# dnvtmf/SK_GS

Measured on AMD Instinct MI355X. Metric: train iters/sec (deform + rasterize fwd+bwd + L1/SSIM loss + Adam; ms/render fwd+bwd beside it), 100k Gaussians @800x800, higher is better.
Workload: dtype f32

## Files before the change

### include/skgs.h

```cpp
#ifndef SKGS_H_
#define SKGS_H_

#include <stddef.h>
#include <stdint.h>

#ifdef __cplusplus
extern "C" {
#endif

#define SKGS_VERSION 1
#define SKGS_TILE 16
#define SKGS_MAX_RENDER_EXTRA 4
#define SKGS_FUSED_LBS_MAX_BONES 60
#define SKGS_FUSED_LBS_MAX_K 8

typedef void* skgs_stream_t;

typedef struct skgs_knn_deform_job {
  int32_t M, K;
  const float* points;
  const float* joints;
  const float* sp_W;
  const float* bone_T;
  const float* bone_drot;
// ... 90 lines not shown
int skgs_rasterize_forward_stage2(const skgs_raster_inputs* in, const skgs_raster_buffers* buf, float* out_color,
    float* out_opacity, float* out_extra, skgs_stream_t stream);
int skgs_rasterize_forward(const skgs_raster_inputs* in, const skgs_raster_buffers* buf, int32_t* radii,
    float* out_color, float* out_opacity, float* out_extra, int32_t* host_num_rendered, skgs_stream_t stream);
int skgs_read_status(const skgs_raster_buffers* buf, skgs_status* host_status, skgs_stream_t stream);

typedef struct skgs_raster_grads {
  const float* dL_dout_color;
  const float* dL_dout_opacity;
  const float* dL_dout_extra;
  const float* grad_means2D_in;
  const float* grad_conic_in;
  const float* grad_opacity_in;
  float* dL_dmeans2D;
  float* dL_dconic;
  float* dL_dcolors;
  float* dL_dopacity;
  float* dL_dmeans3D;
  float* dL_dcov3D;
  float* dL_dsh;
  float* dL_dscales;
  float* dL_drotations;
  float* dL_dextras;
  float* dL_dsh_rest;
  float* workspace; size_t workspace_bytes;
  int32_t workspace_is_zero;
  float* dL_dsh_factors;
  float* stat_xyz_gradient_accum;
  float* stat_denom;
  float* stat_max_radii2D;
  float stat_grad_multiplier;
  const struct skgs_deform_backward_job* deform_backward_job;
  const struct skgs_sp_skinning_job* sp_skinning_job;
  const skgs_offset_deform_job* offset_job;
} skgs_raster_grads;
size_t skgs_backward_workspace_bytes(int32_t P);

int skgs_rasterize_backward(const skgs_raster_inputs* in, const skgs_raster_buffers* buf, const int32_t* radii,
    const float* out_opacity, const skgs_raster_grads* g, skgs_stream_t stream);

int skgs_rasterize_extra_forward(int32_t W, int32_t H, int32_t P, int32_t E, const float* extra,
    const skgs_raster_buffers* buf, float* pixel_extra, skgs_stream_t stream);
int skgs_rasterize_extra_backward(int32_t W, int32_t H, int32_t P, int32_t E, const float* extra,
    const float* out_opacity, const float* grad_pixel_extra, const skgs_raster_buffers* buf, float* grad_means2D,
    float* grad_conic, float* grad_opacity, float* dL_dextra, skgs_stream_t stream);
int skgs_topk_weights(int32_t topk, int32_t W, int32_t H, int32_t P, const skgs_raster_buffers* buf,
    int32_t* top_indices, float* top_weights, skgs_stream_t stream);
int skgs_render_census(int32_t W, int32_t H, const skgs_raster_buffers* buf, float* out_color, float* out_opacity,
    uint32_t* census, skgs_stream_t stream);
int skgs_mark_visible(int32_t P, const float* means3D, const float* viewmatrix, int32_t colmap, uint8_t* present,
    skgs_stream_t stream);

int skgs_sh_grad_from_factors(int32_t P, int32_t n_views, int32_t sh_degree, int32_t sh_coeffs, const float* factors,
    float* dL_dsh, float* dL_dsh_rest, skgs_stream_t stream);

typedef struct skgs_deform_inputs {
  int32_t P, K, M;
  const float* points;
  const float* weights;
  const int64_t* indices;
  const float* bone_T;
  const float* bone_drot;
  const float* bone_dscale;
  const float* xyz;
  const float* log_scale;
  const float* rot;
  const float* opacity_logit;
  const int32_t* live_count;
  int32_t largest;
} skgs_deform_inputs;
typedef struct skgs_deform_backward_job {
  const skgs_deform_inputs* in;
  float* g_bone_T;
  float* g_bone_drot;
  float* g_bone_dscale;
  float* g_xyz;
  float* g_log_scale;
  float* g_rot;
  float* g_opacity_logit;
  float* g_sp_W;
  float* g_logits;
  void* workspace;
  size_t workspace_bytes;
} skgs_deform_backward_job;
int skgs_lbs_deform_forward(const skgs_deform_inputs* in, float* means, float* scales, float* rotations,
    float* opacity, float* d_xyz, float* d_rot, float* d_scale, skgs_stream_t stream);
size_t skgs_lbs_deform_backward_workspace_bytes(int32_t P, int32_t M);
int skgs_lbs_deform_backward(const skgs_deform_inputs* in, const float* g_means, const float* g_scales,
    const float* g_rotations, const float* g_opacity, float* g_weights, float* g_bone_T, float* g_bone_drot,
    float* g_bone_dscale, float* g_xyz, float* g_log_scale, float* g_rot, float* g_opacity_logit, void* workspace,
    size_t workspace_bytes, skgs_stream_t stream);
int skgs_lbs_deform_backward_logits(const skgs_deform_inputs* in, const float* g_means, const float* g_scales,
    const float* g_rotations, const float* g_opacity, float* g_weights, float* g_bone_T, float* g_bone_drot,
    float* g_bone_dscale, float* g_xyz, float* g_log_scale, float* g_rot, float* g_opacity_logit, float* g_sp_W,
    float* g_logits, void* workspace, size_t workspace_bytes, skgs_stream_t stream);
int skgs_knn_bones(int32_t P, int32_t M, int32_t K, int32_t dim, const float* points, const float* joints,
    float* out_dist, int64_t* out_idx, skgs_stream_t stream);
int skgs_knn_dist_weights_forward(int32_t P, int32_t M, int32_t K, int32_t dim, const float* points, const float* joints,
    const float* kernel_radius, const float* kernel_weight, float temperature, int32_t raw_parameters, int64_t* out_idx,
    float* out_weights, float* out_dist, skgs_stream_t stream);
size_t skgs_knn_dist_weights_workspace_bytes(int32_t P, int32_t M, int32_t dim);
int skgs_knn_dist_weights_backward(int32_t P, int32_t M, int32_t K, int32_t dim, const float* points, const float* joints,
    const float* kernel_radius, const float* kernel_weight, float temperature, int32_t raw_parameters,
    int32_t accumulate_joints, const float* weights, const int64_t* indices, const float* nn_dist, const float* g_weights,
    float* g_points, float* g_joints, float* g_kernel_radius, float* g_kernel_weight, void* workspace, size_t workspace_bytes,
    skgs_stream_t stream);
int skgs_lbs_weights_forward(int32_t P, int32_t M, int32_t K, const float* sp_W, const int64_t* indices, float* weights,
    skgs_stream_t stream);
int skgs_lbs_weights_backward_compact(int32_t P, int32_t K, const float* weights, const float* g_weights, float* g_logits,
    skgs_stream_t stream);
int skgs_lbs_logits_scatter(int32_t P, int32_t M, int32_t K, const int64_t* indices, const float* g_logits, float* g_sp_W,
    skgs_stream_t stream);
int skgs_knn_lbs_weights(int32_t P, int32_t M, int32_t K, const float* points, const float* joints, const float* sp_W,
    int64_t* out_idx, float* out_weights, skgs_stream_t stream);
int skgs_lbs_weights_backward(int32_t P, int32_t M, int32_t K, const float* weights, const int64_t* indices,
    const float* g_weights, float* g_sp_W, skgs_stream_t stream);
int skgs_knn_lbs_deform_forward(int32_t P, int32_t M, int32_t K, const float* points, const float* joints, const float* sp_W,
    const float* bone_T, const float* bone_drot, const float* bone_dscale, const float* xyz, const float* log_scale,
    const float* rot, const float* opacity_logit, int64_t* out_idx, float* out_weights, float* means, float* scales,
    float* rotations, float* opacity, const int32_t* live_count ,
    skgs_stream_t stream);

int skgs_se3_blend_forward(int32_t P, int32_t K, int32_t M, const float* T, const int64_t* indices, const float* points,
    const float* weights, float* out, skgs_stream_t stream);
size_t skgs_se3_blend_backward_workspace_bytes(int32_t P, int32_t M);
int skgs_se3_blend_backward(int32_t P, int32_t K, int32_t M, const float* T, const int64_t* indices, const float* points,
    const float* weights, const float* g_out, float* g_T, float* g_weights, float* g_points, void* workspace,
    size_t workspace_bytes, skgs_stream_t stream);

size_t skgs_index_add_rows_workspace_bytes(int64_t R, int32_t C, int32_t M);
int skgs_index_add_rows(int64_t R, int32_t C, int32_t M, const int64_t* indices, const float* rows, float* out, void* workspace,
    size_t workspace_bytes, skgs_stream_t stream);

int skgs_lie_forward(int32_t group, int32_t op, int64_t B, const float* X, const float* Y, float* out, skgs_stream_t stream);
int skgs_lie_backward(int32_t group, int32_t op, int64_t B, const float* grad, const float* X, const float* Y, float* dX, float* dY,
    skgs_stream_t stream);

int skgs_bone_chain_forward(int32_t M, int32_t root, const int32_t* parents, const int32_t* level_nodes,
    const int32_t* level_start, int32_t num_levels, const float* sk_r_raw, const float* joints, const float* global_T,
    float* bone_T, float* chain_A, const int32_t* frame_index, skgs_stream_t stream);
int skgs_bone_chain_backward(int32_t M, int32_t root, const int32_t* parents, const int32_t* level_nodes,
    const int32_t* level_start, int32_t num_levels, const float* sk_r_raw, const float* joints, const float* global_T,
    const float* chain_A, const float* g_bone_T, float* g_sk_r_raw, float* g_joints, float* g_global_T,
    const int32_t* frame_index, skgs_stream_t stream);

size_t skgs_image_loss_workspace_bytes(int32_t C, int32_t H, int32_t W);
int skgs_image_loss_forward(int32_t C, int32_t H, int32_t W, const float* pred, const float* gt, const int32_t* gt_index,
    float lambda_l1, float lambda_ssim, float* loss3 , void* workspace,
    size_t workspace_bytes, skgs_stream_t stream);
int skgs_image_loss_backward(int32_t C, int32_t H, int32_t W, const float* pred, const float* gt, const int32_t* gt_index,
    float lambda_l1, float lambda_ssim, const float* grad_loss, const void* workspace, size_t workspace_bytes,
    float* dL_dpred, float* loss3, skgs_stream_t stream);
int skgs_image_loss_backward_terms(int32_t C, int32_t H, int32_t W, const float* pred, const float* gt,
    const int32_t* gt_index, const float* grad_l1, const float* grad_ssim, const void* workspace, size_t workspace_bytes,
    float* dL_dpred, skgs_stream_t stream);

int32_t skgs_weight_reg_partials(void);
int skgs_weight_sparsity(int64_t n, const float* weights, float eps, float* grad, float* partials, skgs_stream_t stream);
int skgs_weight_smooth(int32_t P, int32_t K, int32_t G, const float* weights, const int64_t* neighbours, const int32_t* inverse_offsets,
    const int32_t* inverse_sources, float* grad, float* partials, skgs_stream_t stream);

int32_t skgs_joint_loss_partials(int32_t M);
int skgs_joint_loss_forward(int32_t M, int32_t inverse_branch, const float* spT, const float* joint_pos, const float* cost_in, float momentum,
    float one_minus_momentum, float* cost_out, float* jd, float* partials, skgs_stream_t stream);
int skgs_joint_loss_reduce(int32_t M, int32_t edges, const int32_t* parent, const float* jd, const float* partials, float* out,
    skgs_stream_t stream);
size_t skgs_joint_loss_backward_workspace_bytes(int32_t M);
// ... 17 lines not shown
size_t skgs_adam_state_bytes(void);
int64_t skgs_adam_chunk_elems(void);
int skgs_adam_step(int32_t n_tensors, const void* tensors, int64_t total_chunks, double beta1, double beta2, double eps,
    float* step_state, float* zero_after ,
    int64_t zero_n, skgs_stream_t stream);
int skgs_adam_step_range(int32_t n_tensors, const void* tensors, int64_t chunk_begin, int64_t chunk_end, double beta1,
    double beta2, double eps, float* step_state, int32_t advance, float* zero_after, int64_t zero_n, skgs_stream_t stream);
int skgs_adam_logit_rows(int32_t P, int32_t M, int32_t K, const float* weights, const int64_t* indices, const float* g_weights,
    const void* tensor, uint32_t* tile_mask, double beta1, double beta2, double eps, const float* step_state, int32_t after_advance,
    skgs_stream_t stream);
int skgs_adam_masked_rows(int32_t P, int32_t M, int32_t K, const int64_t* indices, int32_t scan_gradient, const void* tensor,
    uint32_t* tile_mask, double beta1, double beta2, double eps, const float* step_state, int32_t after_advance, skgs_stream_t stream);
int skgs_adam_logit_mask_rebuild(int32_t P, int32_t M, const float* exp_avg, const float* exp_avg_sq, uint32_t* tile_mask,
    skgs_stream_t stream);
typedef struct skgs_view_advance {
  const void* table;
  const int32_t* order;
  int32_t* cursor;
  void* slot;
  int32_t n_order, words;
} skgs_view_advance;
int skgs_adam_step_tail(int32_t n_tensors, const void* tensors, int64_t chunk_begin, int64_t chunk_end, double beta1,
    double beta2, double eps, float* step_state, float* zero_after, int64_t zero_n, int64_t freq_chunk, int32_t freq_B,
    int32_t freq_D, int32_t freq_degree, const float* freq_grad_out, const float* freq_out, int32_t freq_ld_out,
    float* freq_grad_x, int32_t freq_accumulate, const skgs_view_advance* next_view, skgs_stream_t stream);

int skgs_freq_encode_forward(int32_t B, int32_t D, int32_t degree, const float* x, int32_t ld_x , float* out, int32_t ld_out, skgs_stream_t stream);
int skgs_freq_encode_backward(int32_t B, int32_t D, int32_t degree, const float* grad_out, const float* out, int32_t ld_out,
    float* grad_x, int32_t accumulate , skgs_stream_t stream);
int skgs_linear_forward(int32_t B, int32_t in1, int32_t in2, int32_t out, const float* X1, int32_t ldx1, const float* X2,
    int32_t ldx2, const float* W, const float* bias, float* Y, int32_t ldy, int32_t relu, skgs_stream_t stream);
int skgs_linear_backward(int32_t B, int32_t in1, int32_t in2, int32_t out, const float* X1, int32_t ldx1, const float* X2,
    int32_t ldx2, const float* W, const float* Y, const float* gY, int32_t ldy, int32_t relu, float* gW, float* gb,
    float* gX1, int32_t ldg1, float* gX2, int32_t ldg2, int32_t accumulate_gx, skgs_stream_t stream);

#define SKGS_MLP_MAX_LAYERS 12
typedef struct skgs_mlp_layer {
  const float* W;
  const float* bias;
  float* gW;
  float* gb;
  int32_t in_hidden, in_x0, out, relu;
} skgs_mlp_layer;
typedef struct skgs_mlp_desc {
  int32_t B;
  int32_t p_dim, p_degree, t_dim, t_degree;
  int32_t hidden, n_layers;
  skgs_mlp_layer layer[SKGS_MLP_MAX_LAYERS];
  int32_t n_heads, head_dim[4];
  float* head_out[4];
  const float* head_gout[4];
} skgs_mlp_desc;
size_t skgs_deform_mlp_workspace_bytes(const skgs_mlp_desc* d);
int skgs_deform_mlp_workspace_init(void* workspace, size_t workspace_bytes, skgs_stream_t stream);
int32_t skgs_deform_mlp_xcd_mode(int32_t mode);
int skgs_deform_mlp_forward(const skgs_mlp_desc* d, const float* points, const float* t, float* x0, float* acts, float* out,
    void* workspace, size_t workspace_bytes, skgs_stream_t stream);
int skgs_deform_mlp_backward(const skgs_mlp_desc* d, const float* points, const float* t, const float* x0, const float* acts,
    const float* g_out, float* g_x0, void* workspace, size_t workspace_bytes, skgs_stream_t stream);
typedef struct skgs_adam_range {
  int32_t n_tensors;
  const void* tensors;
  int64_t chunk_begin, chunk_end;
  double beta1, beta2, eps;
  const float* step_count;
  int32_t after_advance;
} skgs_adam_range;
int skgs_deform_mlp_backward_adam(const skgs_mlp_desc* d, const float* points, const float* t, const float* x0,
    const float* acts, const float* g_out, float* g_x0, void* workspace, size_t workspace_bytes, const skgs_adam_range* side,
    skgs_stream_t stream);
typedef struct skgs_bone_chain_desc {
  int32_t M, root, num_levels;
  const int32_t *parents, *level_nodes, *level_start;
  const float* joints;
  const float* global_T;
  const int32_t* frame_index;
  float* bone_T;
  float* chain_A;
  const float* sk_r_raw;
  const float* g_bone_T;
  float* g_joints;
  float* g_global_T;
  float* sk_cache;
} skgs_bone_chain_desc;
int skgs_skeleton_forward(const skgs_mlp_desc* d, const skgs_bone_chain_desc* bones, const float* points, const float* t,
    float* x0, float* acts, void* workspace, size_t workspace_bytes, const skgs_adam_range* side ,
    skgs_stream_t stream);
int skgs_skeleton_backward(const skgs_mlp_desc* d, const skgs_bone_chain_desc* bones, const float* points, const float* t,
    const float* x0, const float* acts, float* g_x0, void* workspace, size_t workspace_bytes, const skgs_adam_range* side,
    skgs_stream_t stream);
int skgs_deform_mlp_status(const void* workspace, uint32_t* host_words4, skgs_stream_t stream);

int skgs_sp_lbs_weights_forward(int32_t P, int32_t M, int32_t K, int32_t F, const float* points, const float* feature,
    const float* sp_points, const float* sp_feature, const float* sp_radius_raw, const float* sp_weight_raw, float temperature,
    const float* sp_W, const int32_t* sp_order , const int32_t* sp_rank , int64_t* out_idx,
    float* out_weights, float* out_dist, void* pairs , size_t pairs_bytes, int32_t params_activated,
    int32_t pairs_prepared ,
    skgs_stream_t stream);
size_t skgs_sp_lbs_weights_workspace_bytes(int32_t P, int32_t M, int32_t F);
int skgs_sp_lbs_weights_backward(int32_t P, int32_t M, int32_t K, int32_t F, const float* feature, const float* sp_feature,
    const float* sp_radius_raw, const float* sp_weight_raw, float temperature, const float* weights, const int64_t* indices,
    const float* nn_dist, const float* g_weights, float* g_feature, float* g_sp_feature, float* g_sp_radius, float* g_sp_weight,
    void* workspace, size_t workspace_bytes, int32_t params_activated, skgs_stream_t stream);

size_t skgs_sp_pairs_bytes(int32_t P, int32_t M, int32_t K);
size_t skgs_sp_skinning_backward_workspace_bytes(int32_t P, int32_t M, int32_t K);
typedef struct skgs_sp_skinning_job {
  const skgs_deform_inputs* in;
  int32_t F;
  const float *feature, *sp_feature, *sp_radius_raw, *sp_weight_raw;
  float temperature;
  int32_t logit_weighting;
  const float* nn_dist;
  float *g_weights, *g_xyz, *g_log_scale, *g_rot, *g_opacity_logit, *g_feature, *g_bone_T, *g_bone_drot, *g_bone_dscale, *g_sp_feature,
      *g_sp_radius, *g_sp_weight;
  void* pairs;
  size_t pairs_bytes;
  void* workspace;
  size_t workspace_bytes;
  const float* g_weights_extra;
  int32_t image_to_deform_off;
} skgs_sp_skinning_job;
int skgs_sp_skinning_backward(const skgs_deform_inputs* in, int32_t F, const float* feature, const float* sp_feature,
    const float* sp_radius_raw, const float* sp_weight_raw, float temperature, int32_t logit_weighting, const float* nn_dist,
    const float* g_means, const float* g_scales, const float* g_rotations, const float* g_opacity, float* g_weights, float* g_xyz,
    float* g_log_scale, float* g_rot, float* g_opacity_logit, float* g_feature, float* g_bone_T, float* g_bone_drot,
    float* g_bone_dscale, float* g_sp_feature, float* g_sp_radius, float* g_sp_weight, void* pairs, size_t pairs_bytes,
    void* workspace, size_t workspace_bytes, skgs_stream_t stream);
int skgs_sp_skinning_backward_job(const skgs_sp_skinning_job* job, const float* g_means, const float* g_scales, const float* g_rotations,
    const float* g_opacity, skgs_stream_t stream);

#define SKGS_SP_NET_LBS_C 1
#define SKGS_SP_NET_RAW_TIME_FLAG 2
#define SKGS_SP_NET_RAW_TIME SKGS_SP_NET_RAW_TIME_FLAG
#define SKGS_SP_NET_RAW_TIME_DEGREE(degree) (SKGS_SP_NET_RAW_TIME_FLAG | ((degree) << 8))
typedef struct skgs_sp_net {
  int32_t M, flags;
  const float* points;
  const float* time;
  const float *time_w1, *time_b1, *time_w2, *time_b2;
  const float* W[8];
  const float* b[8];
  const float *warp_w, *warp_b, *scaling_w, *scaling_b, *rotation_w, *rotation_b;
  const float *local_w, *local_b;
} skgs_sp_net;
size_t skgs_sp_net_saved_bytes(int32_t M);
size_t skgs_sp_net_workspace_bytes(int32_t M);
typedef struct skgs_sp_prepare {
  int32_t P, M, K, F;
  const float* sp_points;
  const float* sp_feature;
  const int32_t* sp_order;
  void* pairs;
  size_t pairs_bytes;
} skgs_sp_prepare;
int skgs_sp_net_forward(const skgs_sp_net* net, float* raw , float* bone_T, float* d_rot, float* d_scale,
    void* saved, size_t saved_bytes, const skgs_sp_prepare* prepare, skgs_stream_t stream);
int skgs_sp_net_backward(const skgs_sp_net* net, const skgs_sp_net* grads, const float* g_bone_T, const float* g_d_rot,
    const float* g_d_scale, const float* g_raw, const void* saved, size_t saved_bytes, void* workspace, size_t workspace_bytes,
    const skgs_adam_range* side, skgs_stream_t stream);

size_t skgs_sp_net_rows_saved_bytes(int32_t P);
size_t skgs_sp_net_rows_workspace_bytes(int32_t P);
int skgs_sp_net_rows_forward(const skgs_sp_net* net, float* raw, void* saved , size_t saved_bytes, skgs_stream_t stream);
int skgs_sp_net_rows_backward(const skgs_sp_net* net, const skgs_sp_net* grads, const float* g_raw, const void* saved,
    size_t saved_bytes, void* workspace, size_t workspace_bytes, skgs_stream_t stream);
// ... 42 lines not shown
```

### sk_gs_amd/_C.py

```python
from __future__ import annotations

import contextlib
import ctypes as C
import os
import threading
from typing import Optional, Tuple

import torch
from torch import Tensor

_HERE = os.path.dirname(os.path.abspath(__file__))
_LIB_PATH = os.environ.get('SKGS_HIP_LIB') or os.path.join(_HERE, 'libskgs_hip.so')
_lib = None
_lock = threading.Lock()


class SkgsError(RuntimeError):
    pass


class _KnnDeformJob(C.Structure):
    _fields_ = [('M', C.c_int32), ('K', C.c_int32)] + [(n, C.c_void_p) for n in (
        'points', 'joints', 'sp_W', 'bone_T', 'bone_drot', 'bone_dscale', 'xyz', 'log_scale', 'rot', 'opacity_logit', 'out_idx',
        'out_weights', 'means', 'scales', 'rotations', 'opacity')] + [('largest', C.c_int32)]


class _OffsetDeformJob(C.Structure):
    _fields_ = [('scale_mode', C.c_int32), ('d_xyz_stride', C.c_int32)] + [(n, C.c_void_p) for n in (
        'xyz', 'd_xyz', 'log_scale', 'rot', 'opacity_logit', 'scale_mean', 'means', 'scales', 'rotations', 'opacity', 'g_xyz', 'g_d_xyz',
        'g_log_scale', 'g_rot', 'g_opacity_logit', 'workspace')] + [('workspace_bytes', C.c_size_t)]


class _RasterInputs(C.Structure):
    _fields_ = [
        ('P', C.c_int32), ('sh_degree', C.c_int32), ('sh_coeffs', C.c_int32), ('E', C.c_int32),
        ('image_height', C.c_int32), ('image_width', C.c_int32),
        ('tanfovx', C.c_float), ('tanfovy', C.c_float), ('scale_modifier', C.c_float),
        ('prefiltered', C.c_int32), ('debug', C.c_int32), ('colmap', C.c_int32),
        ('viewmatrix', C.c_void_p), ('projmatrix', C.c_void_p), ('campos', C.c_void_p),
        ('means3D', C.c_void_p), ('opacity', C.c_void_p), ('sh', C.c_void_p), ('scales', C.c_void_p),
        ('rotations', C.c_void_p), ('extras', C.c_void_p), ('colors_precomp', C.c_void_p),
        ('cov3D_precomp', C.c_void_p), ('sh_rest', C.c_void_p), ('background', C.c_void_p),
        ('tile_bucket_capacity', C.c_int32), ('tanfov_device', C.c_void_p),
        ('host_status_words', C.c_int32), ('longest_list_hint', C.c_int32), ('live_count', C.c_void_p),
        ('deform_job', C.POINTER(_KnnDeformJob)), ('tiles_per_gaussian_hint', C.c_int32), ('offset_job', C.c_void_p),
    ]


class _RasterBuffers(C.Structure):
    _fields_ = [('geom', C.c_void_p), ('geom_bytes', C.c_size_t), ('binning', C.c_void_p),
                ('binning_bytes', C.c_size_t), ('img', C.c_void_p), ('img_bytes', C.c_size_t)]


class _Status(C.Structure):
    _fields_ = [('num_rendered', C.c_int32), ('overflow', C.c_int32), ('max_tile_count', C.c_int32),
                ('overflow_events', C.c_int32)]


class _RasterGrads(C.Structure):
    _fields_ = [
        ('dL_dout_color', C.c_void_p), ('dL_dout_opacity', C.c_void_p), ('dL_dout_extra', C.c_void_p),
        ('grad_means2D_in', C.c_void_p), ('grad_conic_in', C.c_void_p), ('grad_opacity_in', C.c_void_p),
        ('dL_dmeans2D', C.c_void_p), ('dL_dconic', C.c_void_p), ('dL_dcolors', C.c_void_p),
        ('dL_dopacity', C.c_void_p), ('dL_dmeans3D', C.c_void_p), ('dL_dcov3D', C.c_void_p), ('dL_dsh', C.c_void_p),
        ('dL_dscales', C.c_void_p), ('dL_drotations', C.c_void_p), ('dL_dextras', C.c_void_p),
        ('dL_dsh_rest', C.c_void_p), ('workspace', C.c_void_p), ('workspace_bytes', C.c_size_t),
        ('workspace_is_zero', C.c_int32), ('dL_dsh_factors', C.c_void_p),
        ('stat_xyz_gradient_accum', C.c_void_p), ('stat_denom', C.c_void_p), ('stat_max_radii2D', C.c_void_p),
        ('stat_grad_multiplier', C.c_float), ('deform_backward_job', C.c_void_p), ('sp_skinning_job', C.c_void_p),
        ('offset_job', C.c_void_p),
    ]


class _DeformInputs(C.Structure):
    _fields_ = [
        ('P', C.c_int32), ('K', C.c_int32), ('M', C.c_int32),
        ('points', C.c_void_p), ('weights', C.c_void_p), ('indices', C.c_void_p), ('bone_T', C.c_void_p),
        ('bone_drot', C.c_void_p), ('bone_dscale', C.c_void_p), ('xyz', C.c_void_p), ('log_scale', C.c_void_p),
        ('rot', C.c_void_p), ('opacity_logit', C.c_void_p), ('live_count', C.c_void_p), ('largest', C.c_int32),
    ]


class _DeformBackwardJob(C.Structure):
    _fields_ = [('in_', C.POINTER(_DeformInputs))] + [(n, C.c_void_p) for n in (
        'g_bone_T', 'g_bone_drot', 'g_bone_dscale', 'g_xyz', 'g_log_scale', 'g_rot', 'g_opacity_logit', 'g_sp_W', 'g_logits',
        'workspace')] + [('workspace_bytes', C.c_size_t)]


class _SpSkinningJob(C.Structure):
    _fields_ = ([('in_', C.POINTER(_DeformInputs)), ('F', C.c_int32)] +
                [(n, C.c_void_p) for n in ('feature', 'sp_feature', 'sp_radius_raw', 'sp_weight_raw')] +
                [('temperature', C.c_float), ('logit_weighting', C.c_int32), ('nn_dist', C.c_void_p)] +
                [(n, C.c_void_p) for n in ('g_weights', 'g_xyz', 'g_log_scale', 'g_rot', 'g_opacity_logit', 'g_feature', 'g_bone_T',
                                           'g_bone_drot', 'g_bone_dscale', 'g_sp_feature', 'g_sp_radius', 'g_sp_weight', 'pairs')] +
                [('pairs_bytes', C.c_size_t), ('workspace', C.c_void_p), ('workspace_bytes', C.c_size_t), ('g_weights_extra', C.c_void_p),
                 ('image_to_deform_off', C.c_int32)])


EXPORTED_SYMBOLS = [
    'skgs_geom_buffer_bytes', 'skgs_img_buffer_bytes', 'skgs_binning_buffer_bytes', 'skgs_binning_capacity',
    'skgs_rasterize_forward_stage1', 'skgs_rasterize_forward_stage2', 'skgs_rasterize_forward', 'skgs_read_status',
    'skgs_backward_workspace_bytes', 'skgs_rasterize_backward', 'skgs_rasterize_extra_forward',
    'skgs_rasterize_extra_backward', 'skgs_topk_weights', 'skgs_render_census', 'skgs_set_tile_order', 'skgs_knn_dist_weights_forward', 'skgs_knn_dist_weights_backward',
    'skgs_knn_dist_weights_workspace_bytes', 'skgs_mark_visible', 'skgs_lbs_deform_forward',
    'skgs_lbs_deform_backward', 'skgs_lbs_deform_backward_workspace_bytes', 'skgs_knn_bones',
    'skgs_lbs_weights_forward', 'skgs_lbs_weights_backward', 'skgs_last_error', 'skgs_version',
    'skgs_joint_loss_partials', 'skgs_joint_loss_forward', 'skgs_joint_loss_reduce', 'skgs_joint_loss_backward_workspace_bytes',
    'skgs_joint_loss_backward', 'skgs_point_knn_workspace_bytes', 'skgs_point_knn',
]


def lib_path() -> str:
    return _LIB_PATH


def load_library():
    global _lib
    if _lib is not None:
        return _lib
    with _lock:
        if _lib is not None:
            return _lib
        if not os.path.exists(_LIB_PATH):
            raise SkgsError(
                f'{_LIB_PATH} not found: the HIP extension is not built. Run `python -c "import __graft_entry__ as g; '
                f'g.build()"` or `make -C sk_gs_amd/csrc`. There is no CPU / PyTorch fallback for this path.')
        lib = C.CDLL(_LIB_PATH)
        for name in ('skgs_geom_buffer_bytes', 'skgs_img_buffer_bytes', 'skgs_binning_buffer_bytes',
                     'skgs_backward_workspace_bytes', 'skgs_lbs_deform_backward_workspace_bytes',
                     'skgs_image_loss_workspace_bytes', 'skgs_offset_deform_workspace_bytes'):
            getattr(lib, name).restype = C.c_size_t
        lib.skgs_binning_capacity.restype = C.c_int64
        lib.skgs_binning_capacity.argtypes = [C.c_size_t]
        lib.skgs_binning_buffer_bytes.argtypes = [C.c_int64]
        lib.skgs_last_error.restype = C.c_char_p
        if os.environ.get('SKGS_TILE_ORDER') is not None:
            lib.skgs_set_tile_order(C.c_int(int(os.environ['SKGS_TILE_ORDER'])))
        _lib = lib
    return _lib


_ops = None


def _torch_ops():
    global _ops
    if _ops is None:
        _ops = False
        if os.environ.get('SKGS_TORCH_OPS', '1') != '0' and not os.environ.get('SKGS_HIP_LIB'):
            load_library()
            try:
                from sk_gs_amd import _skgs_torch
                _ops = _skgs_torch
            except ImportError:
                pass
    return _ops or None


def _check(rc: int):
    if rc != 0:
        raise SkgsError(load_library().skgs_last_error().decode())


def _ptr(t: Optional[Tensor]):
    if t is None or t.numel() == 0:
        return None
    return t.data_ptr()


# ... 773 lines not shown
```

### sk_gs_amd/csrc/api.hip

```cpp
#include <stdarg.h>
#include <stdio.h>

#include <algorithm>

#include "skgs_common.h"

namespace skgs {
static thread_local char g_err[512] = "";
int set_error(const char* fmt, ...) {
  va_list ap;
  va_start(ap, fmt);
  vsnprintf(g_err, sizeof(g_err), fmt, ap);
  va_end(ap);
  return 1;
}

__global__ void fill_u32_kernel(uint32_t* __restrict__ p, uint32_t v, size_t n) {
  const size_t stride = (size_t) gridDim.x * blockDim.x;
  for (size_t i = (size_t) blockIdx.x * blockDim.x + threadIdx.x; i < n; i += stride) p[i] = v;
}
int fill_u32(void* p, uint32_t v, size_t n_words, hipStream_t s) {
  if (n_words == 0) return 0;
  const int blocks = (int) std::min<size_t>((n_words + 255) / 256, 2048);
  hipLaunchKernelGGL(fill_u32_kernel, dim3(blocks), dim3(256), 0, s, reinterpret_cast<uint32_t*>(p), v, n_words);
// ... 186 lines not shown
    if (launch_preprocess_forward(*in, g, im, radii, s)) return 1;
    if (launch_scatter_sort(*in, g, im, b, s)) return 1;
    return launch_render_forward(*in, g, im, b, out_color, out_opacity, out_extra, s);
  }
  if (skgs_rasterize_forward_stage1(in, buf, radii, host_num_rendered, stream)) return 1;
  return skgs_rasterize_forward_stage2(in, buf, out_color, out_opacity, out_extra, stream);
}

int skgs_read_status(const skgs_raster_buffers* buf, skgs_status* host_status, skgs_stream_t stream) {
  SKGS_REQUIRE(buf && buf->geom && host_status, "read_status: NULL argument");
  SKGS_CHECK_HIP(hipMemcpyAsync(host_status, buf->geom, sizeof(skgs_status), hipMemcpyDeviceToHost, (hipStream_t) stream));
  return 0;
}

static int check_deform(const skgs_deform_inputs* in);

int skgs_rasterize_backward(const skgs_raster_inputs* in, const skgs_raster_buffers* buf, const int32_t* radii,
    const float* out_opacity, const skgs_raster_grads* gr, skgs_stream_t stream) {
  if (check_inputs(in) || check_buffers(in, buf, true)) return 1;
  SKGS_REQUIRE(gr != nullptr, "grads struct is NULL");
  const skgs_offset_deform_job* oj = gr->offset_job;
  if (oj) {
    SKGS_REQUIRE(!gr->deform_backward_job && !gr->sp_skinning_job, "offset_job: not together with deform_backward_job / sp_skinning_job");
    if (offset_job_check(*in, *oj, true)) return 1;
  }
  if (in->P == 0) {
    if (const skgs_deform_backward_job* dj0 = gr->deform_backward_job) {
      SKGS_REQUIRE(dj0->in && dj0->g_bone_T && dj0->g_bone_drot && dj0->g_bone_dscale, "deform_backward_job: NULL argument");
      hipStream_t s0 = (hipStream_t) stream;
      if (fill_u32(dj0->g_bone_T, 0u, (size_t) dj0->in->M * 7, s0) || fill_u32(dj0->g_bone_drot, 0u, (size_t) dj0->in->M * 4, s0) ||
          fill_u32(dj0->g_bone_dscale, 0u, (size_t) dj0->in->M * 3, s0))
        return 1;
    }
    if (const skgs_sp_skinning_job* sj0 = gr->sp_skinning_job)
      return sp_skinning_check(*sj0) || (!sp_fix_job(*sj0) && launch_sp_skinning_rest(*sj0, (hipStream_t) stream));
    return 0;
  }
  SKGS_REQUIRE(radii && out_opacity, "radii / out_opacity are required");
  SKGS_REQUIRE(gr->dL_dout_color, "dL_dout_color is required");
  SKGS_REQUIRE(gr->dL_dmeans2D && ((gr->deform_backward_job || gr->sp_skinning_job || oj) ||
                                      (gr->dL_dcolors && gr->dL_dopacity && gr->dL_dmeans3D && gr->dL_dcov3D && gr->dL_dscales &&
                                          gr->dL_drotations)),
      "gradient outputs are required");
  SKGS_REQUIRE(!(in->sh && in->sh_coeffs > 0) || gr->dL_dsh || gr->dL_dsh_factors,
      "dL_dsh (or dL_dsh_factors) is required when sh is given");
  SKGS_REQUIRE(gr->dL_dsh_factors || (in->sh_rest != nullptr) == (gr->dL_dsh_rest != nullptr),
      "dL_dsh_rest goes with sh_rest (split SH storage)");
  SKGS_REQUIRE(!gr->dL_dsh_factors || (!gr->dL_dsh && !gr->dL_dsh_rest), "dL_dsh_factors replaces dL_dsh / dL_dsh_rest");
  SKGS_REQUIRE(gr->workspace && gr->workspace_bytes >= skgs_backward_workspace_bytes(in->P), "workspace too small");
  hipStream_t s = (hipStream_t) stream;
  GeomView g    = geom_view(buf->geom);
  ImgView im    = img_view(buf->img, in->image_width, in->image_height);
  BinView b     = bin_view(buf->binning, buf->binning_bytes);
  const skgs_deform_backward_job* dj = gr->deform_backward_job;
  if (dj) {
    SKGS_REQUIRE(dj->in != nullptr, "deform_backward_job: in is NULL");
    if (check_deform(dj->in)) return 1;
    SKGS_REQUIRE(dj->in->P == in->P && dj->in->live_count == in->live_count, "deform_backward_job: P / live_count differ from the rasterizer's");
    SKGS_REQUIRE(!dj->in->largest, "deform_backward_job: warp_method `largest` is served by the sp_skinning_job only");
    SKGS_REQUIRE(dj->in->M <= deform_backward_job_max_bones() && dj->in->K <= deform_backward_job_max_k(),
        "deform_backward_job: needs M <= %d, K <= %d (got %d, %d)", deform_backward_job_max_bones(), deform_backward_job_max_k(),
        dj->in->M, dj->in->K);
    SKGS_REQUIRE(dj->g_bone_T && dj->g_bone_drot && dj->g_bone_dscale, "deform_backward_job: bone gradient outputs are required");
    SKGS_REQUIRE(dj->g_xyz && dj->g_log_scale && dj->g_rot && dj->g_opacity_logit, "deform_backward_job: gradient outputs are required");
    SKGS_REQUIRE(dj->g_sp_W || dj->g_logits, "deform_backward_job: one of g_sp_W / g_logits is required");
    SKGS_REQUIRE(dj->workspace && dj->workspace_bytes >= deform_backward_workspace_bytes(in->P, dj->in->M),
        "deform_backward_job: workspace too small (skgs_lbs_deform_backward_workspace_bytes)");
    SKGS_REQUIRE(in->scales && in->rotations, "deform_backward_job: not with cov3D_precomp");
  }
  const skgs_sp_skinning_job* sj = gr->sp_skinning_job;
  if (sj) {
    SKGS_REQUIRE(!dj, "sp_skinning_job: not together with deform_backward_job");
    if (sp_skinning_check(*sj)) return 1;
    SKGS_REQUIRE(sj->in->P == in->P && in->live_count == nullptr, "sp_skinning_job: P differs from the rasterizer's / no row capacity");
    SKGS_REQUIRE(in->scales && in->rotations, "sp_skinning_job: not with cov3D_precomp");
  }
  if (!gr->workspace_is_zero && fill_u32(gr->workspace, 0u, (size_t) in->P * GRAD_ROW, s)) return 1;
  if (launch_render_backward(*in, g, im, b, out_opacity, gr->dL_dout_color, gr->dL_dout_opacity, gr->dL_dout_extra,
          gr->workspace, s))
    return 1;
  if (launch_preprocess_backward(*in, g, radii, *gr, s)) return 1;
  if (sj) return sp_fix_job(*sj) ? 0 : launch_sp_skinning_rest(*sj, s);
  if (oj) return launch_offset_scale_grad_finalize(in->P, *oj, s);
  return dj ? launch_deform_backward_finalize(*dj->in, dj->workspace, dj->g_bone_T, dj->g_bone_drot, dj->g_bone_dscale, s) : 0;
}

int skgs_rasterize_extra_forward(int32_t W, int32_t H, int32_t P, int32_t E, const float* extra,
    const skgs_raster_buffers* buf, float* pixel_extra, skgs_stream_t stream) {
  SKGS_REQUIRE(buf && buf->geom && buf->img, "buffers are required");
  SKGS_REQUIRE(E > 0 && extra && pixel_extra, "Error shape for extras");
  if (P == 0) return 0;
  GeomView g = geom_view(buf->geom);
  ImgView im = img_view(buf->img, W, H);
  BinView b  = bin_view(buf->binning, buf->binning_bytes);
  return launch_extra_forward(W, H, P, E, extra, g, im, b, pixel_extra, (hipStream_t) stream);
}

int skgs_rasterize_extra_backward(int32_t W, int32_t H, int32_t P, int32_t E, const float* extra, const float* out_opacity,
    const float* grad_pixel_extra, const skgs_raster_buffers* buf, float* grad_means2D, float* grad_conic,
    float* grad_opacity, float* dL_dextra, skgs_stream_t stream) {
  SKGS_REQUIRE(buf && buf->geom && buf->img, "buffers are required");
  SKGS_REQUIRE(E > 0 && extra && grad_pixel_extra && out_opacity, "Error shape for extras");
  SKGS_REQUIRE(grad_means2D && grad_conic && grad_opacity && dL_dextra, "gradient outputs are required");
  if (P == 0) return 0;
  hipStream_t s = (hipStream_t) stream;
  GeomView g = geom_view(buf->geom);
  ImgView im = img_view(buf->img, W, H);
  BinView b  = bin_view(buf->binning, buf->binning_bytes);
  if (fill_u32(dL_dextra, 0u, (size_t) P * E, s)) return 1;
  return launch_extra_backward(W, H, P, E, extra, out_opacity, grad_pixel_extra, g, im, b, grad_means2D, grad_conic,
      grad_opacity, dL_dextra, s);
}

int skgs_topk_weights(int32_t topk, int32_t W, int32_t H, int32_t P, const skgs_raster_buffers* buf, int32_t* top_indices,
    float* top_weights, skgs_stream_t stream) {
  SKGS_REQUIRE(buf && buf->geom && buf->img, "buffers are required");
  SKGS_REQUIRE(topk > 0 && top_indices && top_weights, "topk outputs are required");
  hipStream_t s = (hipStream_t) stream;
  if (P == 0) {
    if (fill_u32(top_indices, 0xffffffffu, (size_t) W * H * topk, s)) return 1;
    if (fill_u32(top_weights, 0u, (size_t) W * H * topk, s)) return 1;
    return 0;
  }
  GeomView g = geom_view(buf->geom);
  ImgView im = img_view(buf->img, W, H);
  BinView b  = bin_view(buf->binning, buf->binning_bytes);
  return launch_topk(topk, W, H, g, im, b, top_indices, top_weights, s);
}

int skgs_render_census(int32_t W, int32_t H, const skgs_raster_buffers* buf, float* out_color, float* out_opacity,
    uint32_t* census, skgs_stream_t stream) {
  SKGS_REQUIRE(buf && buf->geom && buf->img && buf->binning, "buffers of a finished forward are required");
  SKGS_REQUIRE(out_color && out_opacity && census, "census outputs are required");
  GeomView g = geom_view(buf->geom);
  ImgView im = img_view(buf->img, W, H);
  BinView b  = bin_view(buf->binning, buf->binning_bytes);
  return launch_render_census(W, H, g, im, b, out_color, out_opacity, census, (hipStream_t) stream);
}

int skgs_mark_visible(int32_t P, const float* means3D, const float* viewmatrix, int32_t colmap, uint8_t* present,
    skgs_stream_t stream) {
  SKGS_REQUIRE(P == 0 || (means3D && viewmatrix && present), "mark_visible: NULL argument");
  return launch_mark_visible(P, means3D, viewmatrix, colmap, present, (hipStream_t) stream);
}

static int check_deform(const skgs_deform_inputs* in) {
  SKGS_REQUIRE(in != nullptr, "deform inputs struct is NULL");
  SKGS_REQUIRE(in->P >= 0 && in->K >= 1 && in->M >= 1, "deform: need P >= 0, K >= 1, M >= 1");
  if (in->P == 0) return 0;
  SKGS_REQUIRE(in->points && in->weights && in->indices && in->bone_T && in->bone_drot && in->bone_dscale,
      "deform: points / weights / indices / bone tensors are required");
  SKGS_REQUIRE(in->log_scale && in->rot && in->opacity_logit, "deform: Gaussian parameter tensors are required");
  return 0;
}

int skgs_lbs_deform_forward(const skgs_deform_inputs* in, float* means, float* scales, float* rotations, float* opacity,
    float* d_xyz, float* d_rot, float* d_scale, skgs_stream_t stream) {
  if (check_deform(in)) return 1;
  SKGS_REQUIRE(in->P == 0 || (in->xyz && means && scales && rotations && opacity), "deform: outputs are required");
  return launch_deform_forward(*in, means, scales, rotations, opacity, d_xyz, d_rot, d_scale, (hipStream_t) stream);
}

size_t skgs_lbs_deform_backward_workspace_bytes(int32_t P, int32_t M) {
  return deform_backward_workspace_bytes(P < 0 ? 0 : P, M < 0 ? 0 : M);
}

int skgs_lbs_deform_backward(const skgs_deform_inputs* in, const float* g_means, const float* g_scales,
// ... 120 lines not shown
```

### sk_gs_amd/csrc/deform.hip

```cpp
#include <algorithm>

#include "skgs_common.h"
#include "deform_lane.h"

#pragma clang fp contract(off)

namespace skgs {
namespace {

constexpr int DEFORM_THREADS = 256;
constexpr int MAX_LDS_BONES  = 1024;

template <bool LDS_BONES>
__global__ void __launch_bounds__(DEFORM_THREADS) deform_forward_kernel(int P, int K, int M, const float* __restrict__ points,
    const float* __restrict__ weights, const int64_t* __restrict__ indices, const float* __restrict__ bone_T,
    const float* __restrict__ bone_drot, const float* __restrict__ bone_dscale, const float* __restrict__ xyz,
    const float* __restrict__ log_scale, const float* __restrict__ rot, const float* __restrict__ opacity_logit,
    float* __restrict__ means, float* __restrict__ scales, float* __restrict__ rotations, float* __restrict__ opacity,
    float* __restrict__ d_xyz, float* __restrict__ d_rot, float* __restrict__ d_scale, int largest) {
  extern __shared__ float s_bones[];
  if (LDS_BONES) {
    for (int j = threadIdx.x; j < M; j += DEFORM_THREADS) load_bone(bone_T, bone_drot, bone_dscale, j, s_bones + j * BONE_F);
    __syncthreads();
  }
  const int n = blockIdx.x * DEFORM_THREADS + threadIdx.x;
  if (n >= P) return;
  const float p[3] = {points[3 * n], points[3 * n + 1], points[3 * n + 2]};
  float sx[3] = {0, 0, 0}, sr[4] = {0, 0, 0, 0}, ss[3] = {0, 0, 0};
  const int kmax = largest ? argmax_slot(weights + (size_t) n * K, K) : -1;
  for (int k = 0; k < K; ++k) {
    const int j   = (int) indices[(size_t) n * K + k];
    const float w = weights[(size_t) n * K + k];
    float bl[BONE_F];
    const float* b;
    if (LDS_BONES) {
      b = s_bones + j * BONE_F;
    } else {
      load_bone(bone_T, bone_drot, bone_dscale, j, bl);
      b = bl;
    }
    float y[3];
    se3_act(b, p, y);
    const float wx = kmax < 0 ? w : (k == kmax ? 1.f : 0.f);
    sx[0] += y[0] * wx, sx[1] += y[1] * wx, sx[2] += y[2] * wx;
    sr[0] += b[7] * w, sr[1] += b[8] * w, sr[2] += b[9] * w, sr[3] += b[10] * w;
    ss[0] += b[11] * w, ss[1] += b[12] * w, ss[2] += b[13] * w;
  }
  float v[4];
#pragma unroll
  for (int c = 0; c < 3; ++c) {
    const float dx = sx[c] - p[c];
    if (d_xyz) d_xyz[3 * n + c] = dx;
    means[3 * n + c]  = xyz[3 * n + c] + dx;
    scales[3 * n + c] = expf(log_scale[3 * n + c]) + ss[c];
    if (d_scale) d_scale[3 * n + c] = ss[c];
  }
  const float4 r4 = reinterpret_cast<const float4*>(rot)[n];
  v[0] = r4.x + sr[0], v[1] = r4.y + sr[1], v[2] = r4.z + sr[2], v[3] = r4.w + sr[3];
  if (d_rot) reinterpret_cast<float4*>(d_rot)[n] = make_float4(sr[0], sr[1], sr[2], sr[3]);
  float nv = sqrtf(v[0] * v[0] + v[1] * v[1] + v[2] * v[2] + v[3] * v[3]);
  nv       = fmaxf(nv, 1e-12f);
  reinterpret_cast<float4*>(rotations)[n] = make_float4(v[0] / nv, v[1] / nv, v[2] / nv, v[3] / nv);
  opacity[n] = 1.0f / (1.0f + expf(-opacity_logit[n]));
}

template <bool LDS_BONES>
__global__ void __launch_bounds__(DEFORM_THREADS) deform_backward_kernel(int P, int K, int M, const float* __restrict__ points,
    const float* __restrict__ weights, const int64_t* __restrict__ indices, const float* __restrict__ bone_T,
    const float* __restrict__ bone_drot, const float* __restrict__ bone_dscale, const float* __restrict__ log_scale,
    const float* __restrict__ rot, const float* __restrict__ opacity_logit, const float* __restrict__ g_means,
    const float* __restrict__ g_scales, const float* __restrict__ g_rotations, const float* __restrict__ g_opacity,
    float* __restrict__ g_weights, float* __restrict__ g_bone_T, float* __restrict__ g_bone_drot,
    float* __restrict__ g_bone_dscale, float* __restrict__ g_xyz, float* __restrict__ g_log_scale,
    float* __restrict__ g_rot, float* __restrict__ g_opacity_logit, int ncopy, float* __restrict__ partials) {
  extern __shared__ float s_mem[];
  float* s_bones = s_mem;
  float* s_grad  = s_mem + (LDS_BONES ? M * BONE_F : 0);
  float* s_my = s_grad + (size_t) (threadIdx.x & (ncopy - 1)) * M * BONE_F;
  if (LDS_BONES) {
    for (int j = threadIdx.x; j < M; j += DEFORM_THREADS) load_bone(bone_T, bone_drot, bone_dscale, j, s_bones + j * BONE_F);
    for (int i = threadIdx.x; i < ncopy * M * BONE_F; i += DEFORM_THREADS) s_grad[i] = 0.f;
    __syncthreads();
  }
  for (int base = blockIdx.x * DEFORM_THREADS; base < P; base += gridDim.x * DEFORM_THREADS) {
    const bool live = base + (int) threadIdx.x < P;
    const int n     = live ? base + (int) threadIdx.x : P - 1;
// ... 93 lines not shown
          for (int c = 0; c < BONE_F; ++c) atomicAdd(&s_my[j * BONE_F + c], out[c]);
        }
      } else if (live) {
#pragma unroll
        for (int c = 0; c < 7; ++c) atomicAdd(&g_bone_T[7 * j + c], out[c]);
#pragma unroll
        for (int c = 0; c < 4; ++c) atomicAdd(&g_bone_drot[4 * j + c], out[7 + c]);
#pragma unroll
        for (int c = 0; c < 3; ++c) atomicAdd(&g_bone_dscale[3 * j + c], out[11 + c]);
      }
    };
#pragma unroll
    for (int k = 0; k < PREF_K; ++k)
      if (k < K) bone_body(k, jj[k], ww[k]);
    for (int k = PREF_K; k < K; ++k) bone_body(k, (int) indices[(size_t) n * K + k], weights[(size_t) n * K + k]);
  }
  if (LDS_BONES) {
    __syncthreads();
    for (int i = threadIdx.x; i < M * BONE_F; i += DEFORM_THREADS) {
      float val = 0.f;
      for (int cpy = 0; cpy < ncopy; ++cpy) val += s_grad[(size_t) cpy * M * BONE_F + i];
      if (partials) {
        partials[(size_t) blockIdx.x * M * BONE_F + i] = val;
      } else if (val != 0.f) {
        const int j = i / BONE_F, c = i % BONE_F;
        if (c < 7)
          atomicAdd(&g_bone_T[7 * j + c], val);
        else if (c < 11)
          atomicAdd(&g_bone_drot[4 * j + c - 7], val);
        else
          atomicAdd(&g_bone_dscale[3 * j + c - 11], val);
      }
    }
  }
}

__global__ void __launch_bounds__(256) deform_backward_wide_finalize_kernel(int M, int nblk, const float* __restrict__ partials,
    float* __restrict__ g_bone_T, float* __restrict__ g_bone_drot, float* __restrict__ g_bone_dscale) {
  const int i = blockIdx.x * 256 + threadIdx.x;
  if (i >= M * BONE_F) return;
  float sum = 0.f;
  for (int b0 = 0; b0 < nblk; b0 += 16) {
    float v[16];
#pragma unroll
    for (int u = 0; u < 16; ++u) v[u] = partials[(size_t) min(b0 + u, nblk - 1) * M * BONE_F + i];
#pragma unroll
    for (int u = 0; u < 16; ++u)
      if (b0 + u < nblk) sum += v[u];
  }
  const int j = i / BONE_F, c = i % BONE_F;
  if (c < 7)
    g_bone_T[7 * j + c] = sum;
  else if (c < 11)
    g_bone_drot[4 * j + c - 7] = sum;
  else
    g_bone_dscale[3 * j + c - 11] = sum;
}

__global__ void __launch_bounds__(DEFORM_BWD_THREADS) deform_backward_moments_kernel(int P, DeformBwdArgs a,
    const float* __restrict__ g_means, const float* __restrict__ g_scales, const float* __restrict__ g_rotations,
    const float* __restrict__ g_opacity, const int32_t* __restrict__ live_count ) {
  if (live_count) P = min(P, live_count[0]);
  if ((int) (blockIdx.x * DEFORM_BWD_THREADS) >= P) {
    deform_bwd_zero_partials(a);
    return;
  }
  extern __shared__ float s_mem[];
  const int n = blockIdx.x * DEFORM_BWD_THREADS + threadIdx.x;
  DeformBwdLane L;
  deform_bwd_prefetch(a, n, n < P, L);
  float g_dx[3] = {0, 0, 0}, g_ds[3] = {0, 0, 0}, go = 0.f;
  float4 gr4 = make_float4(0.f, 0.f, 0.f, 0.f);
  if (n < P) {
#pragma unroll
    for (int c = 0; c < 3; ++c) g_dx[c] = g_means[3 * n + c], g_ds[c] = g_scales[3 * n + c];
    gr4 = reinterpret_cast<const float4*>(g_rotations)[n], go = g_opacity[n];
  }
  deform_bwd_moments(a, P, s_mem, L, g_dx, g_ds, gr4, go);
}

__global__ void __launch_bounds__(256) deform_backward_finalize_kernel(int M, int nblk, const float* __restrict__ partials,
    const float* __restrict__ bone_T, float* __restrict__ g_bone_T, float* __restrict__ g_bone_drot,
    float* __restrict__ g_bone_dscale) {
  __shared__ float s_red[256][MOM_F + 1];
  const int b = blockIdx.x, t = threadIdx.x;
  float acc[MOM_F];
#pragma unroll
  for (int c = 0; c < MOM_F; ++c) acc[c] = 0.f;
  for (int w = t; w < nblk; w += 256) {
    const float* row = partials + ((size_t) w * M + b) * MOM_F;
#pragma unroll
    for (int c = 0; c < MOM_F; ++c) acc[c] += row[c];
  }
#pragma unroll
  for (int c = 0; c < MOM_F; ++c) s_red[t][c] = acc[c];
  __syncthreads();
  for (int d = 128; d > 0; d >>= 1) {
    if (t < d) {
#pragma unroll
      for (int c = 0; c < MOM_F; ++c) s_red[t][c] += s_red[t + d][c];
    }
    __syncthreads();
  }
  if (t != 0) return;
  float m[MOM_F];
  for (int i = 0; i < MOM_F; ++i) m[i] = s_red[0][i];
  const float q0 = bone_T[7 * b + 3], q1 = bone_T[7 * b + 4], q2 = bone_T[7 * b + 5], q3 = bone_T[7 * b + 6];
  const float qn = sqrtf(q0 * q0 + q1 * q1 + q2 * q2 + q3 * q3);
  const float vq[4] = {q0 / qn, q1 / qn, q2 / qn, q3 / qn};
  const float* S = m + 3;
#define SM(a, c) S[3 * (a) + (c)]
  const float pxg[3] = {SM(2, 1) - SM(1, 2), SM(0, 2) - SM(2, 0), SM(1, 0) - SM(0, 1)};
  const float tr     = SM(0, 0) + SM(1, 1) + SM(2, 2);
  float gqh[4];
  for (int i = 0; i < 3; ++i) {
    const float vdp_g = vq[0] * SM(i, 0) + vq[1] * SM(i, 1) + vq[2] * SM(i, 2);
    const float gdv_p = vq[0] * SM(0, i) + vq[1] * SM(1, i) + vq[2] * SM(2, i);
    gqh[i] = 2.0f * vq[3] * pxg[i] + 2.0f * (vdp_g + gdv_p - 2.0f * tr * vq[i]);
  }
  gqh[3] = 2.0f * ((vq[1] * SM(0, 2) - vq[2] * SM(0, 1)) + (vq[2] * SM(1, 0) - vq[0] * SM(1, 2)) +
                   (vq[0] * SM(2, 1) - vq[1] * SM(2, 0)));
#undef SM
  const float dotq = vq[0] * gqh[0] + vq[1] * gqh[1] + vq[2] * gqh[2] + vq[3] * gqh[3];
  g_bone_T[7 * b] = m[0], g_bone_T[7 * b + 1] = m[1], g_bone_T[7 * b + 2] = m[2];
  for (int i = 0; i < 4; ++i) g_bone_T[7 * b + 3 + i] = (gqh[i] - vq[i] * dotq) / qn;
  for (int i = 0; i < 4; ++i) g_bone_drot[4 * b + i] = m[12 + i];
  for (int i = 0; i < 3; ++i) g_bone_dscale[3 * b + i] = m[16 + i];
}

constexpr int KNN_MAXK = 16;
template <int KCAP>
__global__ void __launch_bounds__(256) knn_bones_kernel(int P, int M, int K, int dim, const float* __restrict__ points,
    const float* __restrict__ joints, float* __restrict__ out_dist, int64_t* __restrict__ out_idx, int lds_joints) {
  extern __shared__ float s_j[];
  if (lds_joints) {
    for (int i = threadIdx.x; i < M * dim; i += blockDim.x) s_j[i] = joints[i];
    __syncthreads();
  }
  const float* jt = lds_joints ? s_j : joints;
  const int n = blockIdx.x * blockDim.x + threadIdx.x;
  if (n >= P) return;
  float bd[KCAP];
  int bi[KCAP];
#pragma unroll
  for (int k = 0; k < KCAP; ++k) bd[k] = __builtin_inff(), bi[k] = -1;
  const float* pn = points + (size_t) n * dim;
  const float p0 = pn[0], p1 = dim > 1 ? pn[1] : 0.f, p2 = dim > 2 ? pn[2] : 0.f;
  for (int j = 0; j < M; ++j) {
    float d = 0.f;
    if (dim == 3) {
      const float d0 = p0 - jt[3 * j], d1 = p1 - jt[3 * j + 1], d2 = p2 - jt[3 * j + 2];
      d += d0 * d0;
      d += d1 * d1;
      d += d2 * d2;
    } else {
      for (int c = 0; c < dim; ++c) {
        const float df = pn[c] - jt[(size_t) j * dim + c];
        d += df * df;
      }
    }
    float cd = d;
    int ci   = j;
    topk_insert<KCAP>(bd, bi, cd, ci);
  }
#pragma unroll
  for (int k = 0; k < KCAP; ++k)
    if (k < K) {
      out_dist[(size_t) n * K + k] = bi[k] >= 0 ? bd[k] : 0.f;
      out_idx[(size_t) n * K + k]  = bi[k];
    }
}

__global__ void __launch_bounds__(256) lbs_weights_forward_kernel(int P, int M, int K, const float* __restrict__ sp_W,
    const int64_t* __restrict__ indices, float* __restrict__ weights) {
  const int p = blockIdx.x * 256 + threadIdx.x;
  if (p >= P) return;
  float l[KNN_MAXK];
  float mx = -INFINITY;
  for (int k = 0; k < K; ++k) {
    l[k] = sp_W[(size_t) p * M + (int) indices[(size_t) p * K + k]];
    mx   = fmaxf(mx, l[k]);
  }
  float sum = 0.f;
  for (int k = 0; k < K; ++k) {
    l[k] = expf(l[k] - mx);
    sum += l[k];
  }
  for (int k = 0; k < K; ++k) weights[(size_t) p * K + k] = l[k] / sum;
}

__global__ void __launch_bounds__(256) lbs_weights_backward_kernel(int P, int M, int K, const float* __restrict__ weights,
    const int64_t* __restrict__ indices, const float* __restrict__ g_weights, float* __restrict__ g_sp_W) {
  extern __shared__ float s_rows[];
  const int p0 = blockIdx.x * 256, p = p0 + threadIdx.x;
  float* row = s_rows + (size_t) threadIdx.x * M;
  for (int m = 0; m < M; ++m) row[m] = 0.f;
  if (p < P) {
    float dot = 0.f;
    for (int k = 0; k < K; ++k) dot += weights[(size_t) p * K + k] * g_weights[(size_t) p * K + k];
    for (int k = 0; k < K; ++k) {
      const float w = weights[(size_t) p * K + k];
      row[(int) indices[(size_t) p * K + k]] += w * (g_weights[(size_t) p * K + k] - dot);
    }
  }
  __syncthreads();
  const size_t n = (size_t) min(256, P - p0) * M;
  float* dst     = g_sp_W + (size_t) p0 * M;
  for (size_t i = threadIdx.x; i < n; i += 256) dst[i] = s_rows[i];
}

// ... 315 lines not shown
  if (in.M <= MAX_LDS_BONES)
    hipLaunchKernelGGL(deform_forward_kernel<true>, grid, block, (size_t) in.M * BONE_F * 4, s, in.P, in.K, in.M, in.points,
        in.weights, in.indices, in.bone_T, in.bone_drot, in.bone_dscale, in.xyz, in.log_scale, in.rot, in.opacity_logit,
        means, scales, rotations, opacity, d_xyz, d_rot, d_scale, in.largest ? 1 : 0);
  else
    hipLaunchKernelGGL(deform_forward_kernel<false>, grid, block, 0, s, in.P, in.K, in.M, in.points, in.weights,
        in.indices, in.bone_T, in.bone_drot, in.bone_dscale, in.xyz, in.log_scale, in.rot, in.opacity_logit, means, scales,
        rotations, opacity, d_xyz, d_rot, d_scale, in.largest ? 1 : 0);
  SKGS_CHECK_HIP(hipGetLastError());
  return 0;
}

constexpr int WIDE_MAX_BLOCKS = 512;
static int wide_blocks(int P) { return std::max(1, std::min((P + DEFORM_THREADS - 1) / DEFORM_THREADS, WIDE_MAX_BLOCKS)); }
size_t deform_backward_workspace_bytes(int P, int M) {
  if (M > MOM_MAX_BONES) return M <= MAX_LDS_BONES / 2 ? align256((size_t) wide_blocks(P) * M * BONE_F * 4) + 256 : 256;
  const size_t nblk = (size_t) (P + DEFORM_THREADS - 1) / DEFORM_THREADS;
  return align256(nblk * (size_t) M * MOM_F * 4) + 256;
}

int launch_deform_backward(const skgs_deform_inputs& in, const float* g_means, const float* g_scales,
    const float* g_rotations, const float* g_opacity, float* g_weights, float* g_bone_T, float* g_bone_drot,
    float* g_bone_dscale, float* g_xyz, float* g_log_scale, float* g_rot, float* g_opacity_logit, void* workspace,
    hipStream_t s, float* g_sp_W, float* g_logits) {
  if ((g_sp_W || g_logits) && (in.M > MOM_MAX_BONES || in.K > PREF_K))
    return set_error("deform backward with the logit gradient folded in needs M <= %d and K <= %d (got %d, %d)",
        MOM_MAX_BONES, PREF_K, in.M, in.K);
  if (in.P == 0) {
    if (fill_u32(g_bone_T, 0u, (size_t) in.M * 7, s) || fill_u32(g_bone_drot, 0u, (size_t) in.M * 4, s) ||
        fill_u32(g_bone_dscale, 0u, (size_t) in.M * 3, s))
      return 1;
    return 0;
  }
  dim3 grid((in.P + DEFORM_THREADS - 1) / DEFORM_THREADS), block(DEFORM_THREADS);
  if (in.M <= MOM_MAX_BONES) {
    const size_t lds = deform_bwd_lds_bytes(in.M);
    float* partials  = reinterpret_cast<float*>(workspace);
    DeformBwdArgs a{in.K, in.M, in.points, in.weights, in.indices, in.bone_T, in.bone_drot, in.bone_dscale, in.log_scale, in.rot,
        in.opacity_logit, g_weights, g_xyz, g_log_scale, g_rot, g_opacity_logit, partials, g_sp_W, g_logits};
    {
      ProfScope prof(K_DEFORM_BWD, s);
      hipLaunchKernelGGL(deform_backward_moments_kernel, grid, block, lds, s, in.P, a, g_means, g_scales, g_rotations, g_opacity,
          in.live_count);
    }
    SKGS_CHECK_HIP(hipGetLastError());
    hipLaunchKernelGGL(deform_backward_finalize_kernel, dim3(in.M), dim3(256), 0, s, in.M, (int) grid.x, partials, in.bone_T,
        g_bone_T, g_bone_drot, g_bone_dscale);
    SKGS_CHECK_HIP(hipGetLastError());
    return 0;
  }
  if (in.M <= MAX_LDS_BONES / 2) {
    const size_t table = (size_t) in.M * BONE_F * 4;
    int ncopy = 1;
    while (ncopy < 16 && table * (1 + 2 * ncopy) <= 56 * 1024) ncopy *= 2;
    const int nblk  = wide_blocks(in.P);
    float* partials = reinterpret_cast<float*>(workspace);
    {
      ProfScope prof(K_DEFORM_BWD, s);
      hipLaunchKernelGGL(deform_backward_kernel<true>, dim3(nblk), block, table * (1 + ncopy), s, in.P, in.K, in.M, in.points,
          in.weights, in.indices, in.bone_T, in.bone_drot, in.bone_dscale, in.log_scale, in.rot, in.opacity_logit, g_means,
          g_scales, g_rotations, g_opacity, g_weights, g_bone_T, g_bone_drot, g_bone_dscale, g_xyz, g_log_scale, g_rot,
          g_opacity_logit, ncopy, partials);
    }
    SKGS_CHECK_HIP(hipGetLastError());
    hipLaunchKernelGGL(deform_backward_wide_finalize_kernel, dim3((in.M * BONE_F + 255) / 256), dim3(256), 0, s, in.M, nblk,
        partials, g_bone_T, g_bone_drot, g_bone_dscale);
    SKGS_CHECK_HIP(hipGetLastError());
    return 0;
  }
  if (fill_u32(g_bone_T, 0u, (size_t) in.M * 7, s) || fill_u32(g_bone_drot, 0u, (size_t) in.M * 4, s) ||
      fill_u32(g_bone_dscale, 0u, (size_t) in.M * 3, s))
    return 1;
  ProfScope prof(K_DEFORM_BWD, s);
  hipLaunchKernelGGL(deform_backward_kernel<false>, grid, block, 0, s, in.P, in.K, in.M, in.points, in.weights,
      in.indices, in.bone_T, in.bone_drot, in.bone_dscale, in.log_scale, in.rot, in.opacity_logit, g_means, g_scales,
      g_rotations, g_opacity, g_weights, g_bone_T, g_bone_drot, g_bone_dscale, g_xyz, g_log_scale, g_rot,
      g_opacity_logit, 1, (float*) nullptr);
  SKGS_CHECK_HIP(hipGetLastError());
  return 0;
}

int launch_deform_backward_finalize(const skgs_deform_inputs& in, void* workspace, float* g_bone_T, float* g_bone_drot,
    float* g_bone_dscale, hipStream_t s) {
  const int nblk = (in.P + DEFORM_BWD_THREADS - 1) / DEFORM_BWD_THREADS;
  hipLaunchKernelGGL(deform_backward_finalize_kernel, dim3(in.M), dim3(256), 0, s, in.M, nblk, reinterpret_cast<float*>(workspace),
      in.bone_T, g_bone_T, g_bone_drot, g_bone_dscale);
  SKGS_CHECK_HIP(hipGetLastError());
  return 0;
}
int deform_backward_job_max_bones() { return MOM_MAX_BONES; }
int deform_backward_job_max_k() { return PREF_K; }

int launch_knn_bones(int P, int M, int K, int dim, const float* points, const float* joints, float* out_dist,
    int64_t* out_idx, hipStream_t s) {
  if (P == 0) return 0;
  if (K > KNN_MAXK || K < 1) return set_error("knn_bones: K must be in [1,%d] (got %d)", KNN_MAXK, K);
  const size_t lds = (size_t) M * dim * 4;
  const int use_lds = lds <= 48 * 1024;
  ProfScope prof(K_KNN, s);
#define SKGS_KNN(KCAP_)                                                                                                  \
  hipLaunchKernelGGL(knn_bones_kernel<KCAP_>, dim3((P + 255) / 256), dim3(256), use_lds ? lds : 0, s, P, M, K, dim, points, \
      joints, out_dist, out_idx, use_lds)
  if (K <= 4)
    SKGS_KNN(4);
  else if (K <= 8)
    SKGS_KNN(8);
  else
    SKGS_KNN(KNN_MAXK);
#undef SKGS_KNN
  SKGS_CHECK_HIP(hipGetLastError());
  return 0;
}

int launch_lbs_weights_forward(int P, int M, int K, const float* sp_W, const int64_t* indices, float* weights, hipStream_t s) {
  if (P == 0) return 0;
  if (K > KNN_MAXK || K < 1) return set_error("lbs_weights: K must be in [1,%d] (got %d)", KNN_MAXK, K);
  hipLaunchKernelGGL(lbs_weights_forward_kernel, dim3((P + 255) / 256), dim3(256), 0, s, P, M, K, sp_W, indices, weights);
  SKGS_CHECK_HIP(hipGetLastError());
  return 0;
}

int launch_lbs_weights_backward(int P, int M, int K, const float* weights, const int64_t* indices, const float* g_weights,
    float* g_sp_W, hipStream_t s) {
  if (P == 0 || M == 0) return 0;
  if (M > SKGS_FUSED_LBS_MAX_BONES) {
    const long long n = (long long) P * ((M + 3) / 4);
    hipLaunchKernelGGL(lbs_logits_dense_wide_kernel<true>, dim3((unsigned) ((n + 255) / 256)), dim3(256), 0, s, P, M, K, weights,
        indices, g_weights, g_sp_W);
    SKGS_CHECK_HIP(hipGetLastError());
    return 0;
  }
  hipLaunchKernelGGL(lbs_weights_backward_kernel, dim3((P + 255) / 256), dim3(256), (size_t) M * 256 * 4, s, P, M, K, weights,
      indices, g_weights, g_sp_W);
  SKGS_CHECK_HIP(hipGetLastError());
  return 0;
}

int launch_knn_lbs_weights(int P, int M, int K, const float* points, const float* joints, const float* sp_W, int64_t* out_idx,
    float* out_weights, hipStream_t s) {
  if (P == 0) return 0;
  if (K > KNN_MAXK || K < 1 || K > M) return set_error("knn_lbs_weights: K must be in [1,min(%d,M)] (got %d)", KNN_MAXK, K);
  const size_t lds = ((size_t) ((M * 3 + 3) & ~3) + ((256 * K + 3) & ~3)) * 4 + (size_t) 256 * K * 8;
  if (lds > 60 * 1024) return set_error("knn_lbs_weights: M = %d too large for the LDS joint table", M);
  ProfScope prof(K_KNN, s);
#define SKGS_KNNW(KCAP_)                                                                                            \
  hipLaunchKernelGGL(knn_weights_kernel<KCAP_>, dim3((P + 255) / 256), dim3(256), lds, s, P, M, K, points, joints, sp_W, \
      out_idx, out_weights)
  if (K <= 4)
    SKGS_KNNW(4);
  else if (K <= 5)
    SKGS_KNNW(5);
  else if (K <= 8)
    SKGS_KNNW(8);
  else
    SKGS_KNNW(KNN_MAXK);
#undef SKGS_KNNW
  SKGS_CHECK_HIP(hipGetLastError());
  return 0;
}

int launch_knn_dist_weights_forward(int P, int M, int K, int dim, const float* points, const float* joints, const float* radius,
    const float* kweight, float temperature, int activate, int64_t* out_idx, float* out_weights, float* out_dist, hipStream_t s) {
  if (P == 0) return 0;
  if (K > KNN_MAXK || K < 1 || K > M) return set_error("knn_dist_weights: K must be in [1,min(%d,M)] (got %d)", KNN_MAXK, K);
  if (dim < 1 || dim > 16) return set_error("knn_dist_weights: dim must be in [1,16] (got %d)", dim);
  const size_t lds = (size_t) M * dim * 4;
  const int use_lds = lds <= 48 * 1024;
  ProfScope prof(K_KNN, s);
#define SKGS_KNND(KCAP_)                                                                                                     \
  hipLaunchKernelGGL(knn_dist_weights_kernel<KCAP_>, dim3((P + 255) / 256), dim3(256), use_lds ? lds : 0, s, P, M, K, dim, points, \
      joints, radius, kweight, temperature, out_idx, out_weights, out_dist, use_lds, activate)
  if (K <= 4)
// ... 89 lines not shown
```

### sk_gs_amd/csrc/mlp_fused.hip

```cpp
#include <algorithm>
#include <cstdlib>

#include "adam_update.h"
#include "bone_chain.inl"
#include "skgs_common.h"

namespace skgs {
namespace {

constexpr int MAXL = SKGS_MLP_MAX_LAYERS;
constexpr unsigned SENTINEL = 0xffffffffu;
constexpr int H = 256, INP = 128, KL = 10;
constexpr int NT = 512, NW = NT / 64, NC = 8;
constexpr int G_NET = H / NC;
constexpr int HP = H + 4;

using gu32 = __attribute__((address_space(1))) unsigned int;
typedef float f4 __attribute__((ext_vector_type(4)));

struct FusedLayer {
  const float* W;
  const float* bias;
  float* gW;
  float* gb;
  int in_h, in_x, out, relu;
};
struct FusedArgs {
  int B, p_dim, p_deg, t_dim, t_deg, IN, n_layers, lds_floats;
  const float* points;
  const float* t;
  float* x0;
  float* acts;
  float* out;
  const float* g_out;
  float* g_x0;
  unsigned* hdr;
  float* exch;
  int n_heads, head_dim[4];
  float* head_out[4];
  const float* head_gout[4];
  const float* W[KL];
  const float* bias[KL];
  float* gW[KL];
  float* gb[KL];
  unsigned xmask, relu_mask;
  int out_last;
  const AdamTensor* adam_tensors;
  int adam_n;
  long long adam_c0, adam_c1;
  double adam_beta1, adam_beta2;
  float adam_eps;
  const AdamState* adam_step;
  int adam_after_advance;
  int has_chain;
  chain::ChainArgs chain;
  float* sk_cache;
  int xcd_mode;
  int side_delay;
  unsigned* census;
};

__device__ __forceinline__ FusedLayer get_layer(const FusedArgs& a, int l) {
  return FusedLayer{a.W[l], a.bias[l], a.gW[l], a.gb[l], l ? H : 0, ((a.xmask >> l) & 1u) ? a.IN : 0,
      l == a.n_layers - 1 ? a.out_last : H, (int) ((a.relu_mask >> l) & 1u)};
}

__device__ __host__ __forceinline__ int pad32(int x) { return (x + 31) & ~31; }

__device__ __forceinline__ float* head_elem(const FusedArgs& a, float* const* heads, float* single, int row, int col, int out) {
  if (a.n_heads == 0) return single + (size_t) row * out + col;
  int j = 0, off = 0;
  while (j < a.n_heads - 1 && col >= off + a.head_dim[j]) off += a.head_dim[j++];
  return heads[j] + (size_t) row * a.head_dim[j] + (col - off);
}

__device__ __forceinline__ float row_sum_to_lane15(float v) {
  v += dpp_mov<0x111, 0xf, 0xf, true>(v);
  v += dpp_mov<0x112, 0xf, 0xf, true>(v);
  v += dpp_mov<0x114, 0xf, 0xf, true>(v);
  v += dpp_mov<0x118, 0xf, 0xf, true>(v);
  return v;
}


__device__ __forceinline__ void stamp(const FusedArgs& a, const unsigned* s_misc, int& si, unsigned long long t_entry = 0) {
  if (s_misc[2] && blockIdx.x == 0 && threadIdx.x == 0 && si < 20) {
    if (t_entry) a.hdr[16 + 46] = (unsigned) t_entry;
    a.hdr[16 + 2 * si]     = (unsigned) __builtin_amdgcn_s_memrealtime();
    a.hdr[16 + 2 * si + 1] = (unsigned) __builtin_amdgcn_s_memtime();
    ++si;
  }
}

__device__ __forceinline__ const float* head_elem_sel(const FusedArgs& a, const float* const* heads, const float* single, int row, int col,
    int out) {
  if (a.n_heads == 0) return single + (size_t) row * out + col;
  const int d0 = a.head_dim[0], d1 = a.head_dim[1], d2 = a.head_dim[2], d3 = a.head_dim[3];
  const float *h0 = heads[0], *h1 = heads[1], *h2 = heads[2], *h3 = heads[3];
  const int n = a.n_heads;
  const bool in0 = n == 1 || col < d0, in1 = n == 2 || col < d0 + d1, in2 = n == 3 || col < d0 + d1 + d2;
  const float* base = in0 ? h0 : in1 ? h1 : in2 ? h2 : h3;
  const int dim     = in0 ? d0 : in1 ? d1 : in2 ? d2 : d3;
  const int off     = in0 ? 0 : in1 ? d0 : in2 ? d0 + d1 : d0 + d1 + d2;
  return base + (size_t) row * dim + (col - off);
}

__device__ __forceinline__ bool stamps_on_all(const FusedArgs& a) { return a.hdr[2] != 0; }

__device__ __forceinline__ float not_sentinel(float v) { return f2u(v) == SENTINEL ? u2f(0x7fc00000u) : v; }

__device__ __forceinline__ void store16_sc1(float* p, float4 v) {
  const f4 q = {v.x, v.y, v.z, v.w};
  asm volatile("global_store_dwordx4 %0, %1, off sc1\n\ts_nop 1" ::"v"(p), "v"(q) : "memory");
}

__device__ __forceinline__ void store16_plain(float* p, float4 v) {
  const f4 q = {v.x, v.y, v.z, v.w};
  asm volatile("global_store_dwordx4 %0, %1, off\n\ts_nop 1" ::"v"(p), "v"(q) : "memory");
}
__device__ __forceinline__ void store16_exch(float* p, float4 v, bool plain) {
  if (plain) store16_plain(p, v);
  else store16_sc1(p, v);
}

template <int U>
__device__ __forceinline__ bool gather_slabs(const float* img, float* s_dst, int B, int Bp, int pitch, int n_units, const unsigned* census,
    unsigned& census_word) {
  constexpr int Q = NC / 4;
  const unsigned* cptr = census + 4 * (threadIdx.x & (G_NET - 1));
  f4 cv;
  const float* ptr[U];
  int dst[U];
  bool live[U];
#pragma unroll
  for (int j = 0; j < U; ++j) {
    int u   = j * NT + (int) threadIdx.x;
    live[j] = u < n_units;
    if (!live[j]) u = 0;
    const int g = u / (B * Q), rem = u - g * (B * Q), row = rem / Q, part = rem - row * Q;
    ptr[j] = img + ((size_t) g * Bp + row) * NC + 4 * part;
    dst[j] = row * pitch + g * NC + 4 * part;
  }
  f4 v[U];
  const unsigned long long t0 = __builtin_amdgcn_s_memrealtime();
  bool good = true;
  unsigned polls = 0;
  for (;;) {
    if constexpr (U == 4) {
      asm volatile(
          "global_load_dwordx4 %0, %5, off sc1\n\tglobal_load_dwordx4 %1, %6, off sc1\n\t"
          "global_load_dwordx4 %2, %7, off sc1\n\tglobal_load_dwordx4 %3, %8, off sc1\n\t"
          "global_load_dwordx4 %4, %9, off sc1\n\ts_waitcnt vmcnt(0)"
          : "=&v"(v[0]), "=&v"(v[1]), "=&v"(v[2]), "=&v"(v[3]), "=&v"(cv)
          : "v"(ptr[0]), "v"(ptr[1]), "v"(ptr[2]), "v"(ptr[3]), "v"(cptr)
          : "memory");
    } else {
      static_assert(U == 4 || U == 8, "gather_slabs: 4 or 8 units per thread");
      asm volatile(
          "global_load_dwordx4 %0, %9, off sc1\n\tglobal_load_dwordx4 %1, %10, off sc1\n\t"
          "global_load_dwordx4 %2, %11, off sc1\n\tglobal_load_dwordx4 %3, %12, off sc1\n\t"
          "global_load_dwordx4 %4, %13, off sc1\n\tglobal_load_dwordx4 %5, %14, off sc1\n\t"
          "global_load_dwordx4 %6, %15, off sc1\n\tglobal_load_dwordx4 %7, %16, off sc1\n\t"
          "global_load_dwordx4 %8, %17, off sc1\n\ts_waitcnt vmcnt(0)"
          : "=&v"(v[0]), "=&v"(v[1]), "=&v"(v[2]), "=&v"(v[3]), "=&v"(v[4 % U]), "=&v"(v[5 % U]), "=&v"(v[6 % U]), "=&v"(v[7 % U]), "=&v"(cv)
          : "v"(ptr[0]), "v"(ptr[1]), "v"(ptr[2]), "v"(ptr[3]), "v"(ptr[4 % U]), "v"(ptr[5 % U]), "v"(ptr[6 % U]), "v"(ptr[7 % U]), "v"(cptr)
          : "memory");
    }
    bool ok = f2u(cv.x) != SENTINEL;
#pragma unroll
// ... 44 lines not shown
    acc[rd][1] = __builtin_amdgcn_mfma_f32_4x4x1f32(xv.y, wv.y, acc[rd][1], 0, 0, 0);
    acc[rd][0] = __builtin_amdgcn_mfma_f32_4x4x1f32(xv.z, wv.z, acc[rd][0], 0, 0, 0);
    acc[rd][1] = __builtin_amdgcn_mfma_f32_4x4x1f32(xv.w, wv.w, acc[rd][1], 0, 0, 0);
  }
}
template <int ROUNDS, int NK4 = 0>
__device__ __forceinline__ void mfma_dot(f4 (&acc)[ROUNDS][2], const float* __restrict__ s_src, int pitch, const int (&rowc)[ROUNDS],
    const float* __restrict__ s_w, int wpitch, int colw, int k0, int nk4 = NK4) {
  const float* ws = s_w + colw * wpitch + k0;
  const float* xs = s_src + k0;
  if constexpr (NK4 > 0) {
#pragma unroll
    for (int q = 0; q < NK4; ++q) mfma_step<ROUNDS>(acc, xs + 4 * q, pitch, rowc, ws + 4 * q);
  } else {
#pragma unroll 1
    for (int q = 0; q < nk4; ++q) mfma_step<ROUNDS>(acc, xs + 4 * q, pitch, rowc, ws + 4 * q);
  }
}
template <int ROUNDS>
__device__ __forceinline__ void zero_acc(f4 (&acc)[ROUNDS][2]) {
#pragma unroll
  for (int rd = 0; rd < ROUNDS; ++rd) acc[rd][0] = acc[rd][1] = f4{0.f, 0.f, 0.f, 0.f};
}
template <int Bp>
__device__ __forceinline__ void load_act_column(float (&av)[Bp], const float* __restrict__ ap, int B) {
#pragma unroll
  for (int b4 = 0; b4 < Bp; b4 += 4) {
    if (b4 < B) {
#pragma unroll
      for (int u = 0; u < 4; ++u) av[b4 + u] = ap[min(b4 + u, B - 1) * H];
    }
  }
}
template <int ROUNDS>
__device__ __forceinline__ void write_partials(float* s_part, const f4 (&acc)[ROUNDS][2], const LaneMap& m, int wave, int Bp,
    int n_rg) {
#pragma unroll
  for (int rd = 0; rd < ROUNDS; ++rd) {
    const int rg = 8 * rd + m.rgl;
    if (rg < n_rg) {
      const f4 v = acc[rd][0] + acc[rd][1];
      float* d   = s_part + ((size_t) (wave * Bp + 4 * rg)) * NC + m.colw;
      d[0] = v[0], d[NC] = v[1], d[2 * NC] = v[2], d[3 * NC] = v[3];
    }
  }
}
__device__ __forceinline__ float4 sum_partials(const float* s_part, int Bp, int row, int part) {
  float4 y = *reinterpret_cast<const float4*>(s_part + (size_t) row * NC + 4 * part);
#pragma unroll
  for (int w = 1; w < NW; ++w) {
    const float4 p = *reinterpret_cast<const float4*>(s_part + ((size_t) (w * Bp + row)) * NC + 4 * part);
    y.x += p.x, y.y += p.y, y.z += p.z, y.w += p.w;
  }
  return y;
}

__device__ __forceinline__ void repoison(float* img_other, int nX, int G, int Bp, int g, unsigned* census_other) {
  const int slab4 = Bp * NC / 4;
  const float4 s  = make_float4(u2f(SENTINEL), u2f(SENTINEL), u2f(SENTINEL), u2f(SENTINEL));
  if (threadIdx.x == 0) reinterpret_cast<float4*>(census_other)[g] = s;
  for (int i = threadIdx.x; i < nX * slab4; i += NT) {
    const int l = i / slab4, q = i - l * slab4;
    reinterpret_cast<float4*>(img_other + ((size_t) l * G + g) * Bp * NC)[q] = s;
  }
}

inline int num_cus() {
  static int cached[64] = {0};
  int dev = 0;
  if (hipGetDevice(&dev) != hipSuccess || dev < 0 || dev >= 64) return 256;
  if (cached[dev] == 0) {
    int n = 0;
    if (hipDeviceGetAttribute(&n, hipDeviceAttributeMultiprocessorCount, dev) != hipSuccess || n <= 0) n = 256;
    cached[dev] = n;
  }
  return cached[dev];
}
struct Role {
  bool net;
  int g, wg, n_side;
};
__device__ __forceinline__ Role role_of(const FusedArgs& a) {
  const int b = (int) blockIdx.x, n_side = (int) gridDim.x - G_NET;
  if (!a.xcd_mode) return Role{b < G_NET, b, b - G_NET, n_side};
  const bool low = b < 8 * G_NET;
  const bool net = low && (b & 7) == 0;
  const int before = low ? (b >> 3) + 1 : G_NET;
  return Role{net, b >> 3, b - before, n_side};
}
__device__ __forceinline__ void adam_side_job(const FusedArgs& a, int wg, int n_side) {
  if (!a.adam_tensors || a.adam_c1 <= a.adam_c0) return;
  for (int i = 0; i < a.side_delay; ++i) __builtin_amdgcn_s_sleep(32);
  const int half = threadIdx.x >> 8, t256 = threadIdx.x & 255, lane = threadIdx.x & 63;
  const AdamCoef k = adam_coefficients(a.adam_beta1, a.adam_beta2, a.adam_eps, a.adam_step, a.adam_after_advance != 0);
  const AdamTensorLanes desc = adam_load_descriptors(a.adam_tensors, a.adam_n, lane);
  const int64_t first0 = lane < a.adam_n ? a.adam_tensors[lane].chunk0 : INT64_MAX;
  const int64_t n_chunks = a.adam_c1 - a.adam_c0;
  const int64_t begin = a.adam_c0 + n_chunks * wg / n_side, end = a.adam_c0 + n_chunks * (wg + 1) / n_side;
#if SKGS_SIDE_CHUNKS == 1
  for (int64_t chunk = begin + half; chunk < end; chunk += 2) {
    const int ti0 = adam_owner(a.adam_tensors, a.adam_n, first0, lane, chunk);
    const AdamTensor T0 = ti0 < 64 ? adam_descriptor_of(desc, ti0) : a.adam_tensors[ti0];
    adam_update_chunk(T0, (chunk - T0.chunk0) * ADAM_CHUNK, t256, k);
  }
  return;
#endif
  for (int64_t chunk = begin + 2 * half; chunk < end; chunk += 4) {
    const int ti0 = adam_owner(a.adam_tensors, a.adam_n, first0, lane, chunk);
    const AdamTensor T0 = ti0 < 64 ? adam_descriptor_of(desc, ti0) : a.adam_tensors[ti0];
    if (chunk + 1 < end) {
      const int ti1 = adam_owner(a.adam_tensors, a.adam_n, first0, lane, chunk + 1);
      const AdamTensor T1 = ti1 < 64 ? adam_descriptor_of(desc, ti1) : a.adam_tensors[ti1];
      adam_update_chunk2(T0, (chunk - T0.chunk0) * ADAM_CHUNK, T1, (chunk + 1 - T1.chunk0) * ADAM_CHUNK, t256, k);
    } else {
      adam_update_chunk(T0, (chunk - T0.chunk0) * ADAM_CHUNK, t256, k);
    }
  }
}

template <int PASSES>
__global__ void __launch_bounds__(NT) fused_mlp_forward_kernel(const FusedArgs a) {
  constexpr int Bp = 16 * PASSES, ROUNDS = (4 * PASSES + 7) / 8;
  constexpr int U = (Bp * 64 + NT - 1) / NT <= 4 ? 4 : 8;
  constexpr int EQ = (Bp * INP + NT - 1) / NT;
  static_assert((Bp * 64 + NT - 1) / NT <= 8, "gather_slabs covers at most 8 units per thread");
  extern __shared__ __attribute__((aligned(16))) float smem[];
  const Role role = role_of(a);
  if (!role.net) {
    adam_side_job(a, role.wg, role.n_side);
    return;
  }
  const unsigned long long t_entry = __builtin_amdgcn_s_memrealtime();
  const int tid = threadIdx.x, wave = tid >> 6;
  const int G = G_NET, g = role.g, col0 = g * NC;
  const int B = a.B, nL = a.n_layers, nX = nL - 1, IN = a.IN;
  const int XW = pad32(IN), XP = XW + 4;
  float* s_x0   = smem;
  float* s_act  = s_x0 + Bp * XP;
  float* s_part = s_act + Bp * HP;
  float* s_raw  = s_part + NW * Bp * NC;
  float* s_w    = s_raw + Bp * 4;
  unsigned* s_misc = reinterpret_cast<unsigned*>(smem + a.lds_floats - 4);
  float* s_bias    = smem + a.lds_floats - 4 - KL * NC;
  const LaneMap lm = lane_map();
  int rowc[ROUNDS];
#pragma unroll
  for (int rd = 0; rd < ROUNDS; ++rd) rowc[rd] = (8 * rd + lm.rgl < 4 * PASSES) ? 4 * (8 * rd + lm.rgl) + lm.j : lm.j;

  unsigned cnt = 0, stamps_on = 0;
  if (tid == 0) {
    const gu32* h = reinterpret_cast<const gu32*>((unsigned long long) a.hdr);
    cnt       = __hip_atomic_load(h, __ATOMIC_RELAXED, __HIP_MEMORY_SCOPE_AGENT);
    stamps_on = __hip_atomic_load(h + 2, __ATOMIC_RELAXED, __HIP_MEMORY_SCOPE_AGENT);
  }
  chain::Prefetch cpf;
  int frame_pf = 0;
  if (a.sk_cache && a.chain.frame_index && col0 < a.out_last) frame_pf = a.chain.frame_index[0];
  cpf.valid = false;
  if (a.has_chain && g == 0) cpf = chain::prefetch(a.chain, false, false);
  const int pe = a.p_dim * (1 + 2 * a.p_deg);
  const int ec = tid & (INP - 1), eb0 = tid >> 7;
  const bool e_live = ec < IN;
  const bool e_pt   = ec < pe;
  const int e_cc = e_pt ? ec : ec - pe, e_D = e_pt ? a.p_dim : a.t_dim;
  const int e_col = e_cc / e_D - 1, e_d = e_cc - (e_col + 1) * e_D;
  const float e_phase = (float) (e_col & 1) * (3.141592653589793f / 2);
  float xin[EQ];
#pragma unroll
  for (int q = 0; q < EQ; ++q) {
    const int b = eb0 + q * (NT / INP);
    xin[q] = 0.f;
    if (e_live && b < B) xin[q] = e_pt ? a.points[(size_t) b * a.p_dim + e_d] : a.t[e_d];
  }
  float bv[KL];
  float4 vh[KL], vx[KL];
  const int ch = tid >> 6, kh = 4 * (tid & 63);
  const int cx = tid >> 5, kx = 4 * (tid & 31);
  {
    const float* wp[KL];
    const float* bp[KL];
#pragma unroll
    for (int l = 0; l < KL; ++l) wp[l] = a.W[l], bp[l] = a.bias[l];
#pragma unroll
    for (int l = 0; l < KL; ++l) asm volatile("" : "+s"(wp[l]), "+s"(bp[l]));
#pragma unroll
    for (int l = 0; l < KL; ++l) {
      bv[l] = 0.f;
      vh[l] = vx[l] = make_float4(0.f, 0.f, 0.f, 0.f);
      if (l < nL) {
        FusedLayer L = get_layer(a, l);
        L.W = wp[l], L.bias = bp[l];
        const int K = L.in_h + L.in_x;
        if (tid < NC && L.bias && col0 + tid < L.out) bv[l] = L.bias[col0 + tid];
        if (l > 0 && col0 + ch < L.out) vh[l] = *reinterpret_cast<const float4*>(L.W + (size_t) (col0 + ch) * K + kh);
        if (L.in_x && tid < NT / 2 && col0 + cx < L.out && kx < L.in_x)
          vx[l] = *reinterpret_cast<const float4*>(L.W + (size_t) (col0 + cx) * K + L.in_h + kx);
      }
    }
  }
#pragma unroll
// ... 36 lines not shown
    if (l > 0) {
      const bool ok = gather_slabs<U>(img + (size_t) (l - 1) * G * Bp * NC, s_act, B, Bp, HP, B * H / 4, census, census_word);
      if (!ok) s_misc[1] = 1;
      __syncthreads();
      if (s_misc[1]) break;
      if (l == 1) plain = (a.xcd_mode == 1 || a.xcd_mode == 3) && census_one_xcd(census_word);
      stamp(a, s_misc, si);
    }
    if (last && col0 >= L.out) break;
    f4 acc[ROUNDS][2];
    zero_acc<ROUNDS>(acc);
    if (l > 0) mfma_dot<ROUNDS, H / NW / 4>(acc, s_act, HP, rowc, s_w + woff, WP, lm.colw, (H / NW) * wave);
    if (L.in_x) mfma_dot<ROUNDS>(acc, s_x0, XP, rowc, s_w + woff + hp, WP, lm.colw, (XW / NW) * wave, XW / NW / 4);
    write_partials<ROUNDS>(s_part, acc, lm, wave, Bp, 4 * PASSES);
    __syncthreads();
    if (tid < Bp * 2) {
      const int row = tid >> 1, part = tid & 1;
      float4 y = sum_partials(s_part, Bp, row, part);
      const float4 bz = *reinterpret_cast<const float4*>(s_bias + l * NC + 4 * part);
      y.x += bz.x, y.y += bz.y, y.z += bz.z, y.w += bz.w;
      if (L.relu) y.x = fmaxf(y.x, 0.f), y.y = fmaxf(y.y, 0.f), y.z = fmaxf(y.z, 0.f), y.w = fmaxf(y.w, 0.f);
      y.x = not_sentinel(y.x), y.y = not_sentinel(y.y), y.z = not_sentinel(y.z), y.w = not_sentinel(y.w);
      if (row < B) {
        if (last) {
          const int c = col0 + 4 * part;
          if (c == 0) *reinterpret_cast<float4*>(s_raw + 4 * row) = y;
          if (c < L.out) *const_cast<float*>(head_elem_sel(a, a.head_out, a.out, row, c, L.out)) = y.x;
          if (c + 1 < L.out) *const_cast<float*>(head_elem_sel(a, a.head_out, a.out, row, c + 1, L.out)) = y.y;
          if (c + 2 < L.out) *const_cast<float*>(head_elem_sel(a, a.head_out, a.out, row, c + 2, L.out)) = y.z;
          if (c + 3 < L.out) *const_cast<float*>(head_elem_sel(a, a.head_out, a.out, row, c + 3, L.out)) = y.w;
          if (a.sk_cache) {
            const int frame = frame_pf;
            float* cr = a.sk_cache + ((size_t) frame * B + row) * L.out;
            if (c == 0) {
              const chain::Q4 q = chain::qnormalize({y.x, y.y, y.z, y.w + 1.0f});
              cr[0] = q.x, cr[1] = q.y, cr[2] = q.z, cr[3] = q.w;
            } else {
              if (c < L.out) cr[c] = y.x;
              if (c + 1 < L.out) cr[c + 1] = y.y;
              if (c + 2 < L.out) cr[c + 2] = y.z;
              if (c + 3 < L.out) cr[c + 3] = y.w;
            }
          }
        } else {
          store16_exch(img + ((size_t) l * G + g) * Bp * NC + 4 * tid, y, plain);
          *reinterpret_cast<float4*>(a.acts + ((size_t) l * B + row) * H + col0 + 4 * part) = y;
        }
      }
    }
    woff += NC * WP;
    if (l == 0) {
      int woffs = w_after0;
#pragma unroll
      for (int l2 = 1; l2 < KL; ++l2)
        if (l2 < nL) woffs += store_layer(l2, woffs);
    }
    stamp(a, s_misc, si);
  }
  if (a.has_chain && g == 0 && !s_misc[1]) {
    __syncthreads();
    chain::ChainArgs c = a.chain;
    c.sk_r_raw = s_raw;
    chain::forward_body(s_part, c, cpf);
  }
  if (a.x0 && g == G - 1)
    for (int i = tid; i < B * IN; i += NT) a.x0[i] = s_x0[(i / IN) * XP + (i % IN)];
  if (g == 0 && tid == 0) {
    gu32* h = reinterpret_cast<gu32*>((unsigned long long) a.hdr);
    if (s_misc[1]) __hip_atomic_fetch_add(h + 1, 1u, __ATOMIC_RELAXED, __HIP_MEMORY_SCOPE_AGENT);
    if (plain) __hip_atomic_fetch_add(h + 4, 1u, __ATOMIC_RELAXED, __HIP_MEMORY_SCOPE_AGENT);
    __hip_atomic_fetch_or(h + 6, 1u << (xcc_id() & 7u), __ATOMIC_RELAXED, __HIP_MEMORY_SCOPE_AGENT);
    __hip_atomic_store(h, count + 1, __ATOMIC_RELAXED, __HIP_MEMORY_SCOPE_AGENT);
  }
}

template <int PASSES>
__global__ void __launch_bounds__(NT) fused_mlp_backward_kernel(const FusedArgs a) {
  constexpr int Bp = 16 * PASSES, ROUNDS = (4 * PASSES + 7) / 8;
  constexpr int U = (Bp * 64 + NT - 1) / NT <= 4 ? 4 : 8;
  static_assert((Bp * 64 + NT - 1) / NT <= 8, "gather_slabs covers at most 8 units per thread");
  extern __shared__ __attribute__((aligned(16))) float smem[];
  const Role role = role_of(a);
  if (!role.net) {
    adam_side_job(a, role.wg, role.n_side);
    return;
  }
  const int tid = threadIdx.x, wave = tid >> 6;
  const int G = G_NET, g = role.g, col0 = g * NC;
  const int B = a.B, nL = a.n_layers, IN = a.IN, nX = nL - 1;
  const bool want_gx = a.g_x0 != nullptr && col0 < IN;
  float* s_gz   = smem;
  float* s_x0   = s_gz;
  float* s_own  = s_gz + Bp * HP;
  float* s_part = s_own + nL * Bp * NC;
  float* s_graw = s_part + NW * Bp * NC;
  float* s_wT   = s_graw + Bp * 4;
  int t_total = 0;
  for (int l = 1; l < nL; ++l) t_total += NC * (pad32(get_layer(a, l).out) + 4);
  int x_total = 0;
  if (want_gx)
    for (int l = 0; l < nL; ++l)
      if (get_layer(a, l).in_x) x_total += NC * (pad32(get_layer(a, l).out) + 4);
  unsigned* s_misc = reinterpret_cast<unsigned*>(smem + a.lds_floats - 4);
  float** s_ptr = reinterpret_cast<float**>(smem + a.lds_floats - 4 - 4 * KL);
  static_assert(4 * (KL - 1) <= 64, "the ReLU masks of a thread's unit: four bits per layer in one 64-bit word");
  unsigned long long relu_bits = 0;
  const LaneMap lm = lane_map();
  int rowc[ROUNDS];
#pragma unroll
  for (int rd = 0; rd < ROUNDS; ++rd) rowc[rd] = (8 * rd + lm.rgl < 4 * PASSES) ? 4 * (8 * rd + lm.rgl) + lm.j : lm.j;

  const unsigned long long t_entry = __builtin_amdgcn_s_memrealtime();
  unsigned cnt = 0, stamps_on = 0;
  if (tid == 0) {
    const gu32* h = reinterpret_cast<const gu32*>((unsigned long long) a.hdr);
    cnt       = __hip_atomic_load(h + 3, __ATOMIC_RELAXED, __HIP_MEMORY_SCOPE_AGENT);
    stamps_on = __hip_atomic_load(h + 2, __ATOMIC_RELAXED, __HIP_MEMORY_SCOPE_AGENT);
  }
  auto pstamp = [&](int slot, unsigned long long t) {
    if (stamps_on && blockIdx.x == 0 && tid == 0) {
      a.hdr[16 + 2 * slot]     = (unsigned) (t ? t : __builtin_amdgcn_s_memrealtime());
      a.hdr[16 + 2 * slot + 1] = (unsigned) __builtin_amdgcn_s_memtime();
    }
  };
  chain::Prefetch cpf;
  cpf.valid = false;
  if (a.has_chain) cpf = chain::prefetch(a.chain, true, true);
  pstamp(18, t_entry);
  const int mrow = tid >> 1, mpart = tid & 1;
  const bool mlive = tid < Bp * 2 && mrow < B;
  float4 am[KL], vt[KL], vx[KL];
  constexpr int XQ = Bp * INP / NT;
  float xv[XQ];
  if (a.x0) {
#pragma unroll
    for (int q = 0; q < XQ; ++q) {
      const int i = tid + q * NT, b = i / INP, c = i - b * INP;
      xv[q] = a.x0[(size_t) min(b, B - 1) * IN + min(c, IN - 1)];
    }
  }
  const int wo = tid >> 1, wc4 = 4 * (tid & 1);
  {
    const float* wp[KL];
    float* gwp[KL];
    float* gbp[KL];
#pragma unroll
    for (int l = 0; l < KL; ++l) wp[l] = a.W[l], gwp[l] = a.gW[l], gbp[l] = a.gb[l];
#pragma unroll
    for (int l = 0; l < KL; ++l) asm volatile("" : "+s"(wp[l]), "+s"(gwp[l]), "+s"(gbp[l]));
    if (tid == 0) {
#pragma unroll
      for (int l = 0; l < KL; ++l) s_ptr[2 * l] = gwp[l], s_ptr[2 * l + 1] = gbp[l];
    }
#pragma unroll
    for (int l = 0; l < KL; ++l) {
      am[l] = make_float4(1.f, 1.f, 1.f, 1.f);
      vt[l] = vx[l] = make_float4(0.f, 0.f, 0.f, 0.f);
      if (l < nL) {
        FusedLayer L = get_layer(a, l);
        L.W = wp[l];
        const int K = L.in_h + L.in_x;
        if (l < nL - 1 && L.relu && mlive)
          am[l] = *reinterpret_cast<const float4*>(a.acts + ((size_t) l * B + mrow) * H + col0 + 4 * mpart);
        if (wo < L.out) {
          if (l >= 1) vt[l] = *reinterpret_cast<const float4*>(L.W + (size_t) wo * K + col0 + wc4);
          if (want_gx && L.in_x && col0 + wc4 < L.in_x) vx[l] = *reinterpret_cast<const float4*>(L.W + (size_t) wo * K + L.in_h + col0 + wc4);
        }
      }
    }
  }
  const int oL_pf = get_layer(a, nL - 1).out;
  constexpr int GZQ = Bp * 64 / NT;
  float hgz[GZQ], hown = 0.f;
  {
    const int c = tid & 63;
#pragma unroll
    for (int q = 0; q < GZQ; ++q) {
      const int b = (tid >> 6) + q * (NT / 64);
      hgz[q] = 0.f;
      if (b < B && c < oL_pf && !(a.has_chain && c < 4))
        hgz[q] = *head_elem_sel(a, a.head_gout, a.g_out, b, c, oL_pf);
    }
    const int bo = tid / NC, co = col0 + tid % NC;
    if (tid < Bp * NC && bo < B && co < oL_pf && !(a.has_chain && co < 4))
      hown = *head_elem_sel(a, a.head_gout, a.g_out, bo, co, oL_pf);
  }
  if (stamps_on_all(a)) {
    asm volatile("s_waitcnt vmcnt(0)" ::: "memory");
    pstamp(22, 0);
  }
  if (a.has_chain) {
    chain::backward_stage(s_part, a.chain, cpf);
    pstamp(19, 0);
    chain::backward_levels(s_part, a.chain, s_graw, g == 0);
    __syncthreads();
  }
  pstamp(21, 0);
  {
    int toff = 0, xoff = t_total;
#pragma unroll
    for (int l = 0; l < KL; ++l) {
      if (l < nL) {
        if (l < nL - 1)
          relu_bits |= (unsigned long long) ((am[l].x > 0.f ? 1u : 0u) | (am[l].y > 0.f ? 2u : 0u) | (am[l].z > 0.f ? 4u : 0u) | (am[l].w > 0.f ? 8u : 0u))
                       << (4 * l);
        const int op = pad32(get_layer(a, l).out), OP = op + 4;
        if (wo < op) {
          if (l >= 1) {
            float* d = s_wT + toff + wc4 * OP + wo;
            d[0] = vt[l].x, d[OP] = vt[l].y, d[2 * OP] = vt[l].z, d[3 * OP] = vt[l].w;
          }
          if (want_gx && get_layer(a, l).in_x) {
            float* d = s_wT + xoff + wc4 * OP + wo;
            d[0] = vx[l].x, d[OP] = vx[l].y, d[2 * OP] = vx[l].z, d[3 * OP] = vx[l].w;
          }
        }
        if (l >= 1) toff += NC * OP;
        if (want_gx && get_layer(a, l).in_x) xoff += NC * OP;
      }
    }
  }
  pstamp(20, 0);
  {
    const int oL = oL_pf;
    const int c = tid & 63;
#pragma unroll
    for (int q = 0; q < GZQ; ++q) {
      const int b = (tid >> 6) + q * (NT / 64);
      float v = hgz[q];
      if (a.has_chain && c < 4 && b < B) v = s_graw[4 * b + c];
      s_gz[b * HP + c] = (b < B && c < oL) ? v : 0.f;
    }
    if (tid < Bp * NC) {
      const int b = tid / NC, cc = col0 + tid % NC;
      float v = hown;
      if (a.has_chain && cc < 4 && b < B) v = s_graw[4 * b + cc];
      s_own[(nL - 1) * Bp * NC + tid] = (b < B && cc < oL) ? v : 0.f;
    }
  }
  if (tid == 0) s_misc[0] = cnt, s_misc[1] = 0, s_misc[2] = stamps_on;
  __syncthreads();
  const unsigned count = s_misc[0];
  const size_t img_floats = (size_t) nX * G * Bp * NC;
  float* img = a.exch + (count & 1u) * img_floats;
  repoison(a.exch + ((count & 1u) ^ 1u) * img_floats, nX, G, Bp, g, a.census + ((count & 1u) ^ 1u) * (G_NET * 4));
  census_publish(a, count & 1u, g);
  const unsigned* census = a.census + (count & 1u) * (G_NET * 4);
  bool plain = false;
  unsigned census_word = 0;
  int si = 12;
  stamp(a, s_misc, si);

  const int kcol = (H / NW) * wave + 4 * lm.rgl + lm.j;
  f4 gw = {0.f, 0.f, 0.f, 0.f};
  float* gw_dst = nullptr;
  int gw_ld = 0, gw_rows = 0;
  f4 accx[ROUNDS][2];
  zero_acc<ROUNDS>(accx);

  int tcur = t_total, xcur = t_total + x_total;
#pragma unroll 1
  for (int l = nL - 1; l >= 1; --l) {
    {
      const int L_out = l == nL - 1 ? a.out_last : H, L_in_x = ((a.xmask >> l) & 1u) ? a.IN : 0, L_in_h = H;
      float* const L_gW = s_ptr[2 * l];
      const int op = pad32(L_out), OP = op + 4;
      const bool publish = l - 1 >= 1 || a.g_x0 != nullptr;
      const bool do_x = want_gx && L_in_x;
      tcur -= NC * OP;
      if (do_x) xcur -= NC * OP;
      if (gw_dst) {
#pragma unroll
        for (int i = 0; i < 4; ++i)
          if (i < gw_rows) gw_dst[(size_t) i * gw_ld] = gw[i];
        gw_dst = nullptr;
      }
      const bool wg_rows = col0 < L_out;
      float av[Bp];
      if (wg_rows) load_act_column<Bp>(av, a.acts + (size_t) (l - 1) * B * H + kcol, B);
      f4 acc[ROUNDS][2];
      zero_acc<ROUNDS>(acc);
      if (op == H) {
        mfma_dot<ROUNDS, H / NW / 4>(acc, s_gz, HP, rowc, s_wT + tcur, OP, lm.colw, (H / NW) * wave);
        if (do_x) mfma_dot<ROUNDS, H / NW / 4>(accx, s_gz, HP, rowc, s_wT + xcur, OP, lm.colw, (H / NW) * wave);
      } else {
        mfma_dot<ROUNDS>(acc, s_gz, HP, rowc, s_wT + tcur, OP, lm.colw, (op / NW) * wave, op / NW / 4);
        if (do_x) mfma_dot<ROUNDS>(accx, s_gz, HP, rowc, s_wT + xcur, OP, lm.colw, (op / NW) * wave, op / NW / 4);
      }
      write_partials<ROUNDS>(s_part, acc, lm, wave, Bp, 4 * PASSES);
      __syncthreads();
      if (tid < Bp * 2) {
        float4 y = sum_partials(s_part, Bp, mrow, mpart);
        const unsigned m = (unsigned) (relu_bits >> (4 * (l - 1)));
        y.x = (mlive && (m & 1u)) ? not_sentinel(y.x) : 0.f, y.y = (mlive && (m & 2u)) ? not_sentinel(y.y) : 0.f;
        y.z = (mlive && (m & 4u)) ? not_sentinel(y.z) : 0.f, y.w = (mlive && (m & 8u)) ? not_sentinel(y.w) : 0.f;
        if (publish && mlive) store16_exch(img + ((size_t) (l - 1) * G + g) * Bp * NC + 4 * tid, y, plain);
        *reinterpret_cast<float4*>(s_own + (l - 1) * Bp * NC + 4 * tid) = y;
      }
      if (wg_rows) {
        const float* own = s_own + l * Bp * NC + lm.colw;
        gw = f4{0.f, 0.f, 0.f, 0.f};
#pragma unroll
        for (int b4 = 0; b4 < Bp; b4 += 4) {
          if (b4 < B) {
#pragma unroll
            for (int u = 0; u < 4; ++u) gw = __builtin_amdgcn_mfma_f32_4x4x1f32(own[(b4 + u) * NC], av[b4 + u], gw, 0, 0, 0);
          }
        }
        gw_dst = L_gW + (size_t) (col0 + 4 * lm.cg) * (L_in_h + L_in_x) + kcol;
        gw_ld = L_in_h + L_in_x, gw_rows = L_out - (col0 + 4 * lm.cg);
      }
      if (publish) {
        const bool ok = gather_slabs<U>(img + (size_t) (l - 1) * G * Bp * NC, s_gz, B, Bp, HP, B * H / 4, census, census_word);
        if (!ok) s_misc[1] = 1;
      }
      __syncthreads();
      if (s_misc[1]) break;
      if (publish && l == nL - 1) plain = (a.xcd_mode == 1 || a.xcd_mode == 3) && census_one_xcd(census_word);
    }
  }
  if (gw_dst) {
#pragma unroll
    for (int i = 0; i < 4; ++i)
      if (i < gw_rows) gw_dst[(size_t) i * gw_ld] = gw[i];
  }
  stamp(a, s_misc, si);
  if (want_gx && !s_misc[1]) {
    mfma_dot<ROUNDS, H / NW / 4>(accx, s_gz, HP, rowc, s_wT + t_total, H + 4, lm.colw, (H / NW) * wave);
    write_partials<ROUNDS>(s_part, accx, lm, wave, Bp, 4 * PASSES);
    __syncthreads();
    if (tid < Bp * 2 && mrow < B) {
      const float4 y = sum_partials(s_part, Bp, mrow, mpart);
      const int c = col0 + 4 * mpart;
      float* d = a.g_x0 + (size_t) mrow * IN + c;
      if (c < IN) d[0] = y.x;
      if (c + 1 < IN) d[1] = y.y;
      if (c + 2 < IN) d[2] = y.z;
      if (c + 3 < IN) d[3] = y.w;
    }
  }
  stamp(a, s_misc, si);
  if (!s_misc[1]) {
    __syncthreads();
    if (a.x0) {
#pragma unroll
      for (int q = 0; q < XQ; ++q) {
        const int i = tid + q * NT, b = i / INP, c = i - b * INP;
        s_x0[i] = (b < B && c < IN) ? xv[q] : 0.f;
      }
    } else {
      const int pe = a.p_dim * (1 + 2 * a.p_deg);
      for (int i = tid; i < Bp * INP; i += NT) {
        const int b = i / INP, c = i - b * INP;
        float v = 0.f;
        if (b < B && c < IN) {
          const int cc = c < pe ? c : c - pe, D = c < pe ? a.p_dim : a.t_dim;
          v = c < pe ? a.points[(size_t) b * a.p_dim + cc % D] : a.t[cc % D];
          if (cc >= D) {
            const int col = cc / D - 1;
            v = sinf(scalbnf(v, col / 2) + (float) (col % 2) * (3.141592653589793f / 2));
          }
        }
        s_x0[i] = v;
      }
    }
    __syncthreads();
    for (int l = nL - 1; l >= 0; --l) {
      struct { int out, in_x, in_h; float* gW; } L = {l == nL - 1 ? a.out_last : H, ((a.xmask >> l) & 1u) ? a.IN : 0, l ? H : 0, s_ptr[2 * l]};
      if (col0 >= L.out || !L.in_x) continue;
      const int K = L.in_h + L.in_x;
      const float* own = s_own + l * Bp * NC;
      for (int i = tid; i < L.in_x * (NC / 4); i += NT) {
        const int kx = i % L.in_x, q = i / L.in_x, k = L.in_h + kx;
        float gacc[4] = {0.f, 0.f, 0.f, 0.f};
#pragma unroll 4
        for (int b = 0; b < B; ++b) {
          const float av = s_x0[b * INP + kx];
          const float4 o = *reinterpret_cast<const float4*>(own + b * NC + 4 * q);
          gacc[0] += o.x * av, gacc[1] += o.y * av, gacc[2] += o.z * av, gacc[3] += o.w * av;
        }
#pragma unroll
        for (int c = 0; c < 4; ++c)
          if (col0 + 4 * q + c < L.out) L.gW[(size_t) (col0 + 4 * q + c) * K + k] = gacc[c];
      }
    }
    for (int i = tid; i < nL * NC; i += NT) {
      const int l = i / NC, c = i - l * NC;
      struct { int out; float* gb; } L = {l == nL - 1 ? a.out_last : H, s_ptr[2 * l + 1]};
      if (L.gb && col0 + c < L.out) {
        const float* own = s_own + l * Bp * NC + c;
        float sum = 0.f;
#pragma unroll 4
        for (int b = 0; b < B; ++b) sum += own[b * NC];
        L.gb[col0 + c] = sum;
      }
    }
  }
  stamp(a, s_misc, si);
  if (g == 0 && tid == 0) {
    gu32* h = reinterpret_cast<gu32*>((unsigned long long) a.hdr);
    if (s_misc[1]) __hip_atomic_fetch_add(h + 1, 1u, __ATOMIC_RELAXED, __HIP_MEMORY_SCOPE_AGENT);
    if (plain) __hip_atomic_fetch_add(h + 5, 1u, __ATOMIC_RELAXED, __HIP_MEMORY_SCOPE_AGENT);
    __hip_atomic_fetch_or(h + 7, 1u << (xcc_id() & 7u), __ATOMIC_RELAXED, __HIP_MEMORY_SCOPE_AGENT);
    __hip_atomic_store(h + 3, count + 1, __ATOMIC_RELAXED, __HIP_MEMORY_SCOPE_AGENT);
  }
}

constexpr int HDR_BYTES = 256;
constexpr int CENSUS_BYTES = 2 * G_NET * 16;

struct Plan {
  int Bp, passes, IN, INP, G, NC;
  size_t exch_bytes;
};
int make_plan(const skgs_mlp_desc* d, Plan* p) {
  SKGS_REQUIRE(d, "deform_mlp: NULL descriptor");
  SKGS_REQUIRE(d->B >= 1 && d->B <= 48, "deform_mlp: the fused kernels handle 1..48 rows (B = %d): use the per-layer path", d->B);
  SKGS_REQUIRE(d->hidden == H, "deform_mlp: the fused kernels are built for hidden width %d (got %d): use the per-layer path", H, d->hidden);
  SKGS_REQUIRE(d->n_layers >= 2 && d->n_layers <= KL, "deform_mlp: 2..%d layers (heads included)", KL);
  SKGS_REQUIRE(d->p_dim >= 1 && d->t_dim >= 0 && d->p_degree >= 0 && d->t_degree >= 0, "deform_mlp: bad encoder sizes");
  p->IN  = d->p_dim * (1 + 2 * d->p_degree) + d->t_dim * (1 + 2 * d->t_degree);
  p->INP = (p->IN + 63) & ~63;
  SKGS_REQUIRE(p->IN <= INP && p->IN % 4 == 0, "deform_mlp: encoded input must be a multiple of 4 and <= %d wide (%d)", INP, p->IN);
  for (int l = 0; l < d->n_layers; ++l) {
    const skgs_mlp_layer& L = d->layer[l];
    SKGS_REQUIRE(L.W && (reinterpret_cast<uintptr_t>(L.W) & 15) == 0, "deform_mlp: layer %d: weights missing or not 16-byte aligned", l);
    SKGS_REQUIRE(L.in_hidden == (l == 0 ? 0 : d->hidden), "deform_mlp: layer %d: in_hidden must be %d", l, l == 0 ? 0 : d->hidden);
    SKGS_REQUIRE(L.in_x0 == 0 || L.in_x0 == p->IN, "deform_mlp: layer %d: in_x0 must be 0 or the encoded width %d", l, p->IN);
    SKGS_REQUIRE(l > 0 || L.in_x0 == p->IN, "deform_mlp: the first layer reads the encoded input");
    SKGS_REQUIRE(l == d->n_layers - 1 ? (L.out >= 1 && L.out <= d->hidden) : L.out == d->hidden,
        "deform_mlp: layer %d: out = %d", l, L.out);
  }
  SKGS_REQUIRE(d->n_heads >= 0 && d->n_heads <= 4, "deform_mlp: 0..4 heads");
  if (d->n_heads) {
    int sum = 0;
    for (int j = 0; j < d->n_heads; ++j) sum += d->head_dim[j];
    SKGS_REQUIRE(sum == d->layer[d->n_layers - 1].out, "deform_mlp: the head widths must add up to the last layer's out");
  }
  p->passes = (d->B + 15) / 16;
  p->Bp     = p->passes * 16;
  p->NC     = NC;
  p->G      = d->hidden / NC;
  p->exch_bytes = (size_t) 2 * (d->n_layers - 1) * p->Bp * d->hidden * 4 + CENSUS_BYTES;
  return 0;
}

void fill_args(const skgs_mlp_desc* d, const Plan& p, FusedArgs* a) {
  a->B = d->B, a->p_dim = d->p_dim, a->p_deg = d->p_degree, a->t_dim = d->t_dim, a->t_deg = d->t_degree;
  a->IN = p.IN, a->n_layers = d->n_layers;
  a->xmask = a->relu_mask = 0;
  for (int l = 0; l < d->n_layers; ++l) {
    const skgs_mlp_layer& L = d->layer[l];
    a->W[l] = L.W, a->bias[l] = L.bias, a->gW[l] = L.gW, a->gb[l] = L.gb;
    if (L.in_x0) a->xmask |= 1u << l;
    if (L.relu) a->relu_mask |= 1u << l;
  }
  a->out_last = d->layer[d->n_layers - 1].out;
  a->n_heads = d->n_heads;
  for (int j = 0; j < 4; ++j) a->head_dim[j] = d->head_dim[j], a->head_out[j] = d->head_out[j], a->head_gout[j] = d->head_gout[j];
}

int fill_chain(const skgs_mlp_desc* d, const Plan& p, const skgs_bone_chain_desc* b, FusedArgs* a) {
  SKGS_REQUIRE(d->n_heads >= 1 && d->head_dim[0] == 4, "skeleton: the network's first head must be the [M,4] raw joint rotations");
  SKGS_REQUIRE(b->M == d->B, "skeleton: %d bones but %d network rows", b->M, d->B);
  SKGS_REQUIRE(b->root >= 0 && b->root < b->M && b->num_levels >= 1, "skeleton: bad skeleton sizes");
  SKGS_REQUIRE(b->parents && b->level_nodes && b->level_start && b->joints, "skeleton: NULL topology / joints");
  a->has_chain = 1;
  chain::ChainArgs& c = a->chain;
  c.M = b->M, c.root = b->root, c.num_levels = b->num_levels, c.parents = b->parents, c.level_nodes = b->level_nodes;
  c.level_start = b->level_start, c.joints = b->joints, c.global_T = b->global_T, c.frame_index = b->frame_index;
  c.bone_T = b->bone_T, c.chain_A = b->chain_A;
  c.global_T_row = reinterpret_cast<float*>(a->hdr + 8);
  a->sk_cache = b->sk_cache;
  return 0;
}
int fill_side(const skgs_adam_range* side, FusedArgs* a) {
  if (!side || side->n_tensors <= 0) return 0;
  SKGS_REQUIRE(side->tensors && side->step_count && side->chunk_begin >= 0 && side->chunk_end >= side->chunk_begin,
      "deform_mlp: bad side range");
  a->adam_tensors = reinterpret_cast<const AdamTensor*>(side->tensors), a->adam_n = side->n_tensors;
  a->adam_c0 = side->chunk_begin, a->adam_c1 = side->chunk_end;
  a->adam_beta1 = side->beta1, a->adam_beta2 = side->beta2, a->adam_eps = (float) side->eps;
  a->adam_step  = reinterpret_cast<const AdamState*>(side->step_count);
  a->adam_after_advance = side->after_advance ? 1 : 0;
  return 0;
}
int forward_impl(const skgs_mlp_desc* d, const skgs_bone_chain_desc* bones, const float* points, const float* t, float* x0,
    float* acts, float* out, void* workspace, size_t workspace_bytes, const skgs_adam_range* side, skgs_stream_t stream);
int backward_impl(const skgs_mlp_desc* d, const skgs_bone_chain_desc* bones, const float* points, const float* t,
    const float* x0, const float* acts, const float* g_out, float* g_x0, void* workspace, size_t workspace_bytes,
    const skgs_adam_range* side, skgs_stream_t stream);

int g_xcd_mode = -1;
inline int xcd_mode_wanted() {
  if (g_xcd_mode < 0) {
    const char* e = getenv("SKGS_MLP_XCD");
    const char* shared = getenv("SKGS_SHARE_GPU");
    g_xcd_mode = e ? std::max(0, std::min(3, atoi(e))) : ((shared && atoi(shared) != 0) ? 0 : 1);
  }
  return g_xcd_mode;
}
template <typename KernelT>
int launch(KernelT k, const Plan& p, const FusedArgs& a, size_t lds, hipStream_t s, int prof_id) {
  ProfScope prof(prof_id, s);
  if (lds > 64 * 1024)
    SKGS_CHECK_HIP(hipFuncSetAttribute(reinterpret_cast<const void*>(k), hipFuncAttributeMaxDynamicSharedMemorySize, 160 * 1024));
  int side = 0;
  if (a.adam_tensors && a.adam_c1 > a.adam_c0)
    side = (int) std::max<long long>(1, std::min<long long>((a.adam_c1 - a.adam_c0 + 1) / 2, num_cus() - p.G));
  FusedArgs b = a;
  int grid = p.G + side;
  {
    static const int delay = [] { const char* e = getenv("SKGS_SIDE_DELAY"); return e ? std::max(0, atoi(e)) : 0; }();
    b.side_delay = delay;
  }
  b.xcd_mode = xcd_mode_wanted();
  if (b.xcd_mode) {
    if (num_cus() != 256 || p.G != G_NET || (side > 0 && grid < 8 * p.G - 7)) b.xcd_mode = 0;
    else grid = std::max(grid, 8 * p.G - 7);
  }
  hipLaunchKernelGGL(k, dim3(grid), dim3(NT), lds, s, b);
  SKGS_CHECK_HIP(hipGetLastError());
  return 0;
}
#define SKGS_MLP_DISPATCH(KERNEL, PROF_ID)                                                    \
  if (p.passes == 1) return launch(KERNEL<1>, p, a, lds, (hipStream_t) stream, PROF_ID);      \
  if (p.passes == 2) return launch(KERNEL<2>, p, a, lds, (hipStream_t) stream, PROF_ID);      \
  return launch(KERNEL<3>, p, a, lds, (hipStream_t) stream, PROF_ID);

__global__ void init_workspace_kernel(uint32_t* w, size_t n_words) {
  const size_t stride = (size_t) gridDim.x * blockDim.x;
  for (size_t i = (size_t) blockIdx.x * blockDim.x + threadIdx.x; i < n_words; i += stride)
    w[i] = i < HDR_BYTES / 4 ? 0u : SENTINEL;
}

}
}

using namespace skgs;

extern "C" {

int32_t skgs_deform_mlp_xcd_mode(int32_t mode) {
  const int before = xcd_mode_wanted();
  if (mode >= 0) g_xcd_mode = std::min(3, (int) mode);
  return before;
}

size_t skgs_deform_mlp_workspace_bytes(const skgs_mlp_desc* d) {
  Plan p;
  if (make_plan(d, &p)) return 0;
  return HDR_BYTES + 2 * p.exch_bytes;
}

int skgs_deform_mlp_workspace_init(void* workspace, size_t workspace_bytes, skgs_stream_t stream) {
  SKGS_REQUIRE(workspace && workspace_bytes >= HDR_BYTES && (reinterpret_cast<uintptr_t>(workspace) & 255) == 0,
      "deform_mlp_workspace_init: NULL, short or unaligned workspace");
  const size_t n = workspace_bytes / 4;
  hipLaunchKernelGGL(init_workspace_kernel, dim3((unsigned) std::min<size_t>((n + 255) / 256, 1024)), dim3(256), 0,
      (hipStream_t) stream, reinterpret_cast<uint32_t*>(workspace), n);
  SKGS_CHECK_HIP(hipGetLastError());
  return 0;
}

int skgs_deform_mlp_forward(const skgs_mlp_desc* d, const float* points, const float* t, float* x0, float* acts, float* out,
    void* workspace, size_t workspace_bytes, skgs_stream_t stream) {
  return forward_impl(d, nullptr, points, t, x0, acts, out, workspace, workspace_bytes, nullptr, stream);
}

int skgs_skeleton_forward(const skgs_mlp_desc* d, const skgs_bone_chain_desc* bones, const float* points, const float* t,
    float* x0, float* acts, void* workspace, size_t workspace_bytes, const skgs_adam_range* side, skgs_stream_t stream) {
  SKGS_REQUIRE(bones, "skeleton_forward: NULL bone chain");
  return forward_impl(d, bones, points, t, x0, acts, nullptr, workspace, workspace_bytes, side, stream);
}

}

namespace skgs {
namespace {
int forward_impl(const skgs_mlp_desc* d, const skgs_bone_chain_desc* bones, const float* points, const float* t, float* x0,
    float* acts, float* out, void* workspace, size_t workspace_bytes, const skgs_adam_range* side, skgs_stream_t stream) {
  Plan p;
  if (make_plan(d, &p)) return 1;
  SKGS_REQUIRE(points && (t || d->t_dim == 0) && acts && workspace, "deform_mlp_forward: NULL argument");
  for (int j = 0; j < d->n_heads; ++j) SKGS_REQUIRE(d->head_out[j], "deform_mlp_forward: head_out[%d] is NULL", j);
  SKGS_REQUIRE(out || d->n_heads, "deform_mlp_forward: no output tensor");
  SKGS_REQUIRE(workspace_bytes >= HDR_BYTES + 2 * p.exch_bytes, "deform_mlp_forward: workspace too small");
  SKGS_REQUIRE((reinterpret_cast<uintptr_t>(acts) & 15) == 0 && (reinterpret_cast<uintptr_t>(workspace) & 255) == 0,
      "deform_mlp_forward: acts must be 16-byte, the workspace 256-byte aligned");
  FusedArgs a{};
  fill_args(d, p, &a);
  a.points = points, a.t = t, a.x0 = x0, a.acts = acts, a.out = out;
  a.hdr  = reinterpret_cast<unsigned*>(workspace);
  a.exch = reinterpret_cast<float*>(reinterpret_cast<char*>(workspace) + HDR_BYTES);
  a.census = reinterpret_cast<unsigned*>(reinterpret_cast<char*>(a.exch) + p.exch_bytes - CENSUS_BYTES);
  if (bones) {
    if (fill_chain(d, p, bones, &a)) return 1;
    SKGS_REQUIRE(bones->bone_T, "skeleton_forward: bone_T is NULL");
    SKGS_REQUIRE(chain::forward_scratch_floats(bones->M, bones->num_levels) <= (size_t) NW * p.Bp * NC,
        "skeleton_forward: %d tree levels do not fit the scratch", bones->num_levels);
  }
  if (fill_side(side, &a)) return 1;
  const int XW = pad32(p.IN);
  size_t fl = (size_t) p.Bp * (XW + 4) + (size_t) p.Bp * HP + (size_t) NW * p.Bp * NC + (size_t) p.Bp * 4 + (size_t) KL * NC + 4;
  for (int l = 0; l < d->n_layers; ++l) fl += (size_t) NC * ((l ? H : 0) + (d->layer[l].in_x0 ? XW : 0) + 4);
  a.lds_floats = (int) fl;
  const size_t lds = fl * 4;
  SKGS_REQUIRE(lds <= 160 * 1024, "deform_mlp_forward: %zu bytes of LDS needed", lds);
  SKGS_MLP_DISPATCH(fused_mlp_forward_kernel, K_SKELETON_FWD)
}
}
}

extern "C" {

int skgs_deform_mlp_backward(const skgs_mlp_desc* d, const float* points, const float* t, const float* x0, const float* acts,
    const float* g_out, float* g_x0, void* workspace, size_t workspace_bytes, skgs_stream_t stream) {
  return backward_impl(d, nullptr, points, t, x0, acts, g_out, g_x0, workspace, workspace_bytes, nullptr, stream);
}

int skgs_deform_mlp_backward_adam(const skgs_mlp_desc* d, const float* points, const float* t, const float* x0,
    const float* acts, const float* g_out, float* g_x0, void* workspace, size_t workspace_bytes, const skgs_adam_range* side,
    skgs_stream_t stream) {
  return backward_impl(d, nullptr, points, t, x0, acts, g_out, g_x0, workspace, workspace_bytes, side, stream);
}

int skgs_skeleton_backward(const skgs_mlp_desc* d, const skgs_bone_chain_desc* bones, const float* points, const float* t,
    const float* x0, const float* acts, float* g_x0, void* workspace, size_t workspace_bytes, const skgs_adam_range* side,
    skgs_stream_t stream) {
  SKGS_REQUIRE(bones, "skeleton_backward: NULL bone chain");
  return backward_impl(d, bones, points, t, x0, acts, nullptr, g_x0, workspace, workspace_bytes, side, stream);
}

}

namespace skgs {
namespace {
int backward_impl(const skgs_mlp_desc* d, const skgs_bone_chain_desc* bones, const float* points, const float* t,
    const float* x0, const float* acts, const float* g_out, float* g_x0, void* workspace, size_t workspace_bytes,
    const skgs_adam_range* side, skgs_stream_t stream) {
  Plan p;
  if (make_plan(d, &p)) return 1;
  SKGS_REQUIRE(points && (t || d->t_dim == 0) && acts && workspace, "deform_mlp_backward: NULL argument");
  for (int j = bones ? 1 : 0; j < d->n_heads; ++j)
    SKGS_REQUIRE(d->head_gout[j], "deform_mlp_backward: head_gout[%d] is NULL", j);
  SKGS_REQUIRE(g_out || d->n_heads, "deform_mlp_backward: no incoming gradient");
  SKGS_REQUIRE(workspace_bytes >= HDR_BYTES + 2 * p.exch_bytes, "deform_mlp_backward: workspace too small");
  SKGS_REQUIRE((reinterpret_cast<uintptr_t>(acts) & 15) == 0 && (reinterpret_cast<uintptr_t>(workspace) & 255) == 0,
      "deform_mlp_backward: acts must be 16-byte, the workspace 256-byte aligned");
  for (int l = 0; l < d->n_layers; ++l) SKGS_REQUIRE(d->layer[l].gW, "deform_mlp_backward: layer %d has no gW", l);
  SKGS_REQUIRE(!g_x0 || p.IN <= d->hidden, "deform_mlp_backward: the input gradient needs hidden >= encoded width (%d < %d)",
      d->hidden, p.IN);
  FusedArgs a{};
  fill_args(d, p, &a);
  a.points = points, a.t = t, a.x0 = const_cast<float*>(x0), a.acts = const_cast<float*>(acts), a.g_out = g_out, a.g_x0 = g_x0;
  a.hdr = reinterpret_cast<unsigned*>(workspace);
  if (bones) {
    if (fill_chain(d, p, bones, &a)) return 1;
    SKGS_REQUIRE(bones->sk_r_raw && bones->chain_A && bones->g_bone_T, "skeleton_backward: sk_r_raw / chain_A / g_bone_T is NULL");
    SKGS_REQUIRE(chain::backward_scratch_floats(bones->M, bones->num_levels) <= (size_t) NW * p.Bp * NC,
        "skeleton_backward: %d tree levels do not fit the scratch", bones->num_levels);
    a.chain.sk_r_raw = bones->sk_r_raw, a.chain.g_bone_T = bones->g_bone_T, a.chain.g_joints = bones->g_joints;
    a.chain.g_global_T = bones->g_global_T, a.chain.g_sk_r_raw = const_cast<float*>(d->head_gout[0]);
  }
  if (fill_side(side, &a)) return 1;
  a.hdr  = reinterpret_cast<unsigned*>(workspace);
  a.exch = reinterpret_cast<float*>(reinterpret_cast<char*>(workspace) + HDR_BYTES + p.exch_bytes);
  a.census = reinterpret_cast<unsigned*>(reinterpret_cast<char*>(a.exch) + p.exch_bytes - CENSUS_BYTES);
  size_t fl = (size_t) p.Bp * HP + (size_t) (d->n_layers + NW) * p.Bp * NC + (size_t) p.Bp * 4 + 4;
  fl += (size_t) 4 * KL;
  for (int l = 1; l < d->n_layers; ++l) fl += (size_t) NC * (pad32(d->layer[l].out) + 4);
  if (g_x0)
    for (int l = 0; l < d->n_layers; ++l)
      if (d->layer[l].in_x0) fl += (size_t) NC * (pad32(d->layer[l].out) + 4);
  a.lds_floats = (int) fl;
  const size_t lds = fl * 4;
  SKGS_REQUIRE(lds <= 160 * 1024, "deform_mlp_backward: %zu bytes of LDS needed", lds);
  SKGS_MLP_DISPATCH(fused_mlp_backward_kernel, K_SKELETON_BWD)
}
}
}

extern "C" {

int skgs_deform_mlp_status(const void* workspace, uint32_t* host_words4, skgs_stream_t stream) {
  SKGS_REQUIRE(workspace && host_words4, "deform_mlp_status: NULL argument");
  SKGS_CHECK_HIP(hipMemcpyAsync(host_words4, workspace, 16, hipMemcpyDeviceToHost, (hipStream_t) stream));
  return 0;
}

}
```

### sk_gs_amd/csrc/skgs_common.h

```cpp
#pragma once
#include <hip/hip_runtime.h>
#include <algorithm>
#include <stdint.h>

#include "../../include/skgs.h"

namespace skgs {

constexpr int TILE      = SKGS_TILE;
constexpr int WAVE      = 64;
constexpr int REC_F4    = 3;
constexpr int GRAD_ROW  = 16;

struct GeomHeader {
  int32_t num_rendered;
  int32_t overflow;
  int32_t max_tile_count;
  int32_t overflow_events;
  int32_t P;
  int32_t big_tiles;
  int32_t pad[58];
};
static_assert(sizeof(GeomHeader) == 256, "header");

// ... 287 lines not shown
};
#if defined(__HIPCC__)
__device__ __forceinline__ void sp_prepare_element(const SpPrepareJob& j, int i) {
  constexpr int ROW = 12;
  if (i < j.n_clear && i != 2) j.header_and_counts[i] = 0u;
  if (i >= j.M * ROW) return;
  const int r = i / ROW, c = i - r * ROW;
  const int id = j.sp_order ? j.sp_order[r] : r;
  float v = 0.f;
  if (c < 3)
    v = j.sp_points[3 * id + c];
  else if (c < 3 + j.F)
    v = j.sp_feature[(size_t) id * j.F + c - 3];
  else if (c == ROW - 1)
    v = __builtin_bit_cast(float, id);
  j.table[i] = v;
}
#endif
inline size_t sp_pairs_capacity(int P, int M, int K) {
  const size_t mean = ((size_t) P * K + M - 1) / M;
  return std::min<size_t>((size_t) std::max(P, 1), std::max<size_t>(4096, 16 * mean));
}
inline SpPairsView sp_pairs_view(void* base, int P, int M, int K) {
  SpPairsView v;
  v.header = reinterpret_cast<uint32_t*>(base);
  v.counts = reinterpret_cast<uint32_t*>(reinterpret_cast<char*>(base) + 256);
  v.lists  = reinterpret_cast<uint32_t*>(reinterpret_cast<char*>(base) + 256 + align256((size_t) M * 4));
  v.cap    = (int) sp_pairs_capacity(P, M, K);
  v.table  = reinterpret_cast<float*>(v.lists + (size_t) M * v.cap);
  return v;
}
size_t sp_pairs_bytes(int P, int M, int K);

int fill_u32(void* p, uint32_t v, size_t n_words, hipStream_t s);

int launch_preprocess_forward(const skgs_raster_inputs& in, GeomView g, ImgView im, int32_t* radii, hipStream_t s);
int launch_preprocess_backward(const skgs_raster_inputs& in, GeomView g, const int32_t* radii,
    const skgs_raster_grads& gr, hipStream_t s);
int launch_sh_grad_from_factors(int P, int n_views, int D, int M, const float* factors, float* dL_dsh, float* dL_dsh_rest,
    hipStream_t s);
int launch_mark_visible(int P, const float* means, const float* view, int colmap, uint8_t* present, hipStream_t s);
size_t offset_deform_workspace_bytes(int P);
int offset_job_check(const skgs_raster_inputs& in, const skgs_offset_deform_job& j, bool backward);
int launch_offset_scale_grad_finalize(int P, const skgs_offset_deform_job& j, hipStream_t s);
int launch_scan_tiles(GeomView g, ImgView im, int64_t P, hipStream_t s);
int launch_scatter_sort(const skgs_raster_inputs& in, GeomView g, ImgView im, BinView b, hipStream_t s);
bool gradacc_rows_hold_moments();
int launch_render_forward(const skgs_raster_inputs& in, GeomView g, ImgView im, BinView b, float* out_color,
    float* out_opacity, float* out_extra, hipStream_t s);
int launch_render_census(int W, int H, GeomView g, ImgView im, BinView b, float* out_color, float* out_opacity,
    uint32_t* census, hipStream_t s);
int launch_render_backward(const skgs_raster_inputs& in, GeomView g, ImgView im, BinView b, const float* out_opacity,
    const float* dL_dcolor, const float* dL_dopacity, const float* dL_dextra, float* gradacc, hipStream_t s);
int launch_extra_forward(int W, int H, int P, int E, const float* extra, GeomView g, ImgView im, BinView b,
    float* pixel_extra, hipStream_t s);
int launch_extra_backward(int W, int H, int P, int E, const float* extra, const float* out_opacity,
    const float* grad_pixel_extra, GeomView g, ImgView im, BinView b, float* grad_means2D, float* grad_conic,
    float* grad_opacity, float* dL_dextra, hipStream_t s);
int launch_topk(int topk, int W, int H, GeomView g, ImgView im, BinView b, int32_t* top_idx, float* top_w,
    hipStream_t s);
int launch_deform_forward(const skgs_deform_inputs& in, float* means, float* scales, float* rotations, float* opacity,
    float* d_xyz, float* d_rot, float* d_scale, hipStream_t s);
size_t deform_backward_workspace_bytes(int P, int M);
int launch_deform_backward(const skgs_deform_inputs& in, const float* g_means, const float* g_scales,
    const float* g_rotations, const float* g_opacity, float* g_weights, float* g_bone_T, float* g_bone_drot,
    float* g_bone_dscale, float* g_xyz, float* g_log_scale, float* g_rot, float* g_opacity_logit, void* workspace,
    hipStream_t s, float* g_sp_W = nullptr, float* g_logits = nullptr);
int launch_knn_bones(int P, int M, int K, int dim, const float* points, const float* joints, float* out_dist,
    int64_t* out_idx, hipStream_t s);
int launch_knn_dist_weights_forward(int P, int M, int K, int dim, const float* points, const float* joints, const float* radius,
    const float* kweight, float temperature, int activate, int64_t* out_idx, float* out_weights, float* out_dist, hipStream_t s);
size_t knn_dist_weights_workspace_bytes(int P, int M, int dim);
int launch_knn_dist_weights_backward(int P, int M, int K, int dim, const float* points, const float* joints, const float* radius,
    const float* kweight, float temperature, int activate, int accumulate_joints, const float* weights, const int64_t* indices,
    const float* nn_dist, const float* g_weights, float* g_points, float* g_joints, float* g_radius, float* g_kweight,
    void* workspace, size_t workspace_bytes, hipStream_t s);
int launch_knn_lbs_weights(int P, int M, int K, const float* points, const float* joints, const float* sp_W, int64_t* out_idx,
    float* out_weights, hipStream_t s);
int sp_skinning_check(const skgs_sp_skinning_job& j);
int launch_sp_skinning_rest(const skgs_sp_skinning_job& j, hipStream_t s);
inline bool sp_fix_job(const skgs_sp_skinning_job& j) { return j.image_to_deform_off != 0 && j.g_weights_extra == nullptr; }
int launch_deform_backward_finalize(const skgs_deform_inputs& in, void* workspace, float* g_bone_T, float* g_bone_drot,
    float* g_bone_dscale, hipStream_t s);
int deform_backward_job_max_bones();
int deform_backward_job_max_k();
int launch_knn_deform_forward(int P, int M, int K, const float* points, const float* joints, const float* sp_W,
    const float* bone_T, const float* bone_drot, const float* bone_dscale, const float* xyz, const float* log_scale,
    const float* rot, const float* opacity_logit, int64_t* out_idx, float* out_weights, float* means, float* scales,
    float* rotations, float* opacity, const int32_t* live_count, hipStream_t s);
int launch_lbs_weights_backward_compact(int P, int K, const float* weights, const float* g_weights, float* g_logits,
    hipStream_t s);
int launch_lbs_logits_scatter(int P, int M, int K, const int64_t* indices, const float* g_logits, float* g_sp_W,
    hipStream_t s);
int launch_lbs_weights_forward(int P, int M, int K, const float* sp_W, const int64_t* indices, float* weights, hipStream_t s);
int launch_lbs_weights_backward(int P, int M, int K, const float* weights, const int64_t* indices, const float* g_weights,
    float* g_sp_W, hipStream_t s);
}
```

### sk_gs_amd/deform_net.py

```python
import ctypes as C
import weakref
from typing import List, Optional, Sequence, Tuple

import torch
from torch import Tensor, nn
import torch.nn.functional as F

from sk_gs_amd import _C


def freq_encode_torch(x: Tensor, degree: int) -> Tensor:
    outs = [x]
    for f in range(degree):
        outs.append(torch.sin(x * (2.0 ** f)))
        outs.append(torch.sin(x * (2.0 ** f) + torch.pi / 2))
    return torch.cat(outs, dim=-1)


class _MLPWithSkips(nn.Module):

    def __init__(self, in_channels: int, dim_hidden: int, out_channels: Sequence[int], num_layers: int, skips: Sequence[int]):
        super().__init__()
        self.in_channels, self.dim_hidden, self.num_layers = in_channels, dim_hidden, num_layers
        self.out_channels, self.skips = tuple(out_channels), tuple(skips)
# ... 92 lines not shown
    def forward_hidden(self, x0: Tensor, acts: Tensor):
        net, lib = self.mlp.dynamic_net, self.lib
        B, IN, H = x0.shape[0], net.in_channels, net.dim_hidden
        dims = net.layer_dims()
        prev, ldp = x0.data_ptr(), IN
        for i, layer in enumerate(net.net):
            in1, in2 = dims[i]
            _lin_fwd(lib, B, in1, in2, H, prev, ldp, x0.data_ptr() if in2 else None, IN, layer.weight.data_ptr(),
                     layer.bias.data_ptr(), acts[i].data_ptr(), H, 1)
            prev, ldp = acts[i].data_ptr(), H

    def forward(self, x0: Tensor, acts: Tensor, out: Tensor):
        net, lib = self.mlp.dynamic_net, self.lib
        self.forward_hidden(x0, acts)
        in1, in2 = net.layer_dims()[-1]
        _lin_fwd(lib, x0.shape[0], in1, in2, out.shape[1], acts[-1].data_ptr(), net.dim_hidden,
                 x0.data_ptr() if in2 else None, net.in_channels, net.last_weight.data_ptr(), net.last_bias.data_ptr(),
                 out.data_ptr(), out.shape[1], 0)

    def backward_hidden(self, x0: Tensor, acts: Tensor, grads: List[Tensor], g_act: Tensor, g_x0: Optional[Tensor] = None,
                        g_x0_started: bool = False):
        net, lib = self.mlp.dynamic_net, self.lib
        B, IN, H, L = x0.shape[0], net.in_channels, net.dim_hidden, net.num_layers
        dims = net.layer_dims()
        x0p = x0.data_ptr()
        gx0p = None if g_x0 is None else g_x0.data_ptr()
        started = g_x0_started
        cur = 0
        for i in range(L - 1, -1, -1):
            in1, in2 = dims[i]
            layer = net.net[i]
            x1, ld1 = (acts[i - 1].data_ptr(), H) if i > 0 else (x0p, IN)
            if i > 0:
                gx1, ldg1, gx2 = g_act[1 - cur].data_ptr(), H, (gx0p if in2 else None)
                acc = 2 if (gx2 is not None and started) else 0
                started = started or gx2 is not None
            else:
                gx1, ldg1, gx2 = gx0p, IN, None
                acc = 1 if (gx1 is not None and started) else 0
            _lin_bwd(lib, B, in1, in2, H, x1, ld1, x0p if in2 else None, IN, layer.weight.data_ptr(), acts[i].data_ptr(),
                     g_act[cur].data_ptr(), H, 1, grads[2 * i].data_ptr(), grads[2 * i + 1].data_ptr(), gx1, ldg1, gx2, IN,
                     acc)
            cur = 1 - cur

    def backward(self, x0: Tensor, acts: Tensor, out: Tensor, g_out: Tensor, grads: List[Tensor], g_act: Tensor,
                 g_x0: Optional[Tensor] = None):
        net, lib = self.mlp.dynamic_net, self.lib
        B, IN, H, L = x0.shape[0], net.in_channels, net.dim_hidden, net.num_layers
        in1, in2 = net.layer_dims()[-1]
        gx2 = g_x0.data_ptr() if (g_x0 is not None and in2) else None
        _lin_bwd(lib, B, in1, in2, out.shape[1], acts[L - 1].data_ptr(), H, x0.data_ptr() if in2 else None, IN,
                 net.last_weight.data_ptr(), None, g_out.data_ptr(), out.shape[1], 0, grads[-2].data_ptr(),
                 grads[-1].data_ptr(), g_act[0].data_ptr(), H, gx2, IN, 0)
        self.backward_hidden(x0, acts, grads[:-2], g_act, g_x0, g_x0_started=gx2 is not None)

    def input_grad(self, g_x0: Tensor, x0: Tensor, g_points: Tensor, accumulate: bool = False):
        m = self.mlp
        _C._check(self.lib.skgs_freq_encode_backward(
            C.c_int32(x0.shape[0]), C.c_int32(m.p_in), C.c_int32(m.p_degree), C.c_void_p(g_x0.data_ptr()),
            C.c_void_p(x0.data_ptr()), C.c_int32(x0.shape[1]), C.c_void_p(g_points.data_ptr()), C.c_int32(int(accumulate)),
            _C._stream()))


class _MlpLayer(C.Structure):
    _fields_ = [('W', C.c_void_p), ('bias', C.c_void_p), ('gW', C.c_void_p), ('gb', C.c_void_p),
                ('in_hidden', C.c_int32), ('in_x0', C.c_int32), ('out', C.c_int32), ('relu', C.c_int32)]


MLP_MAX_LAYERS = 12


class _MlpDesc(C.Structure):
    _fields_ = [('B', C.c_int32), ('p_dim', C.c_int32), ('p_degree', C.c_int32), ('t_dim', C.c_int32),
                ('t_degree', C.c_int32), ('hidden', C.c_int32), ('n_layers', C.c_int32),
                ('layer', _MlpLayer * MLP_MAX_LAYERS), ('n_heads', C.c_int32), ('head_dim', C.c_int32 * 4),
                ('head_out', C.c_void_p * 4), ('head_gout', C.c_void_p * 4)]


class BoneChainDesc(C.Structure):
    _fields_ = [('M', C.c_int32), ('root', C.c_int32), ('num_levels', C.c_int32),
                ('parents', C.c_void_p), ('level_nodes', C.c_void_p), ('level_start', C.c_void_p),
                ('joints', C.c_void_p), ('global_T', C.c_void_p), ('frame_index', C.c_void_p),
                ('bone_T', C.c_void_p), ('chain_A', C.c_void_p), ('sk_r_raw', C.c_void_p), ('g_bone_T', C.c_void_p),
                ('g_joints', C.c_void_p), ('g_global_T', C.c_void_p), ('sk_cache', C.c_void_p)]


def fused_supported(mlp: 'DeformMLP', B: int) -> bool:
    net = mlp.dynamic_net
    return (1 <= B <= 48 and net.dim_hidden == 256 and net.in_channels <= 128 and net.in_channels % 4 == 0
            and net.num_layers + 1 <= 10 and sum(net.out_channels) <= net.dim_hidden)


class FusedDeformMLP:

    def __init__(self, mlp: DeformMLP, B: int):
        if not fused_supported(mlp, B):
            raise _C.SkgsError(f'fused deform MLP: unsupported shape (rows {B}, hidden {mlp.dynamic_net.dim_hidden}, '
                               f'input {mlp.dynamic_net.in_channels}); use DeformMLPRunner')
        self.mlp, self.lib, self.B = mlp, _C.load_library(), int(B)
        net = mlp.dynamic_net
        dev = net.last_weight.device
        if dev.type != 'cuda':
            raise _C.SkgsError('fused deform MLP needs the network on a HIP device; sk_gs_amd has no CPU path')
        f32 = dict(dtype=torch.float32, device=dev)
        self.x0 = torch.empty((B, net.in_channels), **f32)
        self.acts = torch.empty((net.num_layers, B, net.dim_hidden), **f32)
        self.out = torch.empty((B, sum(net.out_channels)), **f32)
        self.lib.skgs_deform_mlp_workspace_bytes.restype = C.c_size_t
        d = self._desc(None)
        nbytes = self.lib.skgs_deform_mlp_workspace_bytes(C.byref(d))
        if nbytes == 0:
            _C._check(1)
        self.workspace = torch.empty((nbytes,), dtype=torch.uint8, device=dev)
        _C._check(self.lib.skgs_deform_mlp_workspace_init(C.c_void_p(self.workspace.data_ptr()), C.c_size_t(nbytes),
                                                          _C._stream()))

    def _desc(self, grads: Optional[Sequence[Tensor]], head_out: Optional[Sequence[Tensor]] = None,
              head_gout: Optional[Sequence[Tensor]] = None) -> _MlpDesc:
        m, net = self.mlp, self.mlp.dynamic_net
        flat = getattr(self, '_flat_params', None)
        if flat is None:
            flat = self._flat_params = [p for l in net.net for p in (l.weight, l.bias)] + [net.last_weight, net.last_bias]
        key = tuple(p.data_ptr() for p in flat)
        d = getattr(self, '_desc_cache', None)
        if d is None or self._desc_key != key:
            d = _MlpDesc()
            d.B, d.p_dim, d.p_degree, d.t_dim, d.t_degree = self.B, m.p_in, m.p_degree, m.t_in, m.t_degree
            d.hidden, d.n_layers = net.dim_hidden, net.num_layers + 1
            dims = net.layer_dims()
            for i, (in1, in2) in enumerate(dims):
                w, b = flat[2 * i], flat[2 * i + 1]
                assert w.is_contiguous() and b.is_contiguous() and w.dtype == torch.float32
                L = d.layer[i]
                L.W, L.bias = w.data_ptr(), b.data_ptr()
                L.in_hidden, L.in_x0 = (0, in1) if i == 0 else (in1, in2)
                L.out, L.relu = w.shape[0], int(i < net.num_layers)
            self._desc_cache, self._desc_key = d, key
        if grads is not None:
            for i in range(d.n_layers):
                gw, gb, w, b = grads[2 * i], grads[2 * i + 1], flat[2 * i], flat[2 * i + 1]
                assert gw.is_contiguous() and gb.is_contiguous() and gw.shape == w.shape and gb.shape == b.shape
                d.layer[i].gW, d.layer[i].gb = gw.data_ptr(), gb.data_ptr()
        heads = head_out if head_out is not None else head_gout
        d.n_heads = 0
        if heads is not None:
            assert len(heads) == len(net.out_channels) <= 4
            d.n_heads = len(heads)
            for j, (h, oc) in enumerate(zip(heads, net.out_channels)):
                assert h.is_cuda and h.is_contiguous() and h.dtype == torch.float32 and tuple(h.shape) == (self.B, oc)
                d.head_dim[j] = oc
                (d.head_out if head_out is not None else d.head_gout)[j] = h.data_ptr()
                (d.head_gout if head_out is not None else d.head_out)[j] = None
        return d

    def forward(self, points: Tensor, t: Tensor, head_out: Optional[Sequence[Tensor]] = None,
                out: Optional[Tensor] = None, bones: Optional[BoneChainDesc] = None, side_adam=None) -> Tensor:
        assert points.is_cuda and points.is_contiguous() and points.dtype == torch.float32 and points.shape[0] == self.B
        assert t.is_cuda and t.dtype == torch.float32 and t.numel() == self.mlp.t_in
        out = self.out if out is None else out
        assert out.is_cuda and out.is_contiguous() and out.shape == self.out.shape and out.dtype == torch.float32
        d = self._desc(None, head_out=head_out)
        if bones is not None:
            assert head_out is not None
            _C._check(self.lib.skgs_skeleton_forward(
                C.byref(d), C.byref(bones), C.c_void_p(points.data_ptr()), C.c_void_p(t.data_ptr()),
                C.c_void_p(self.x0.data_ptr()), C.c_void_p(self.acts.data_ptr()), C.c_void_p(self.workspace.data_ptr()),
                C.c_size_t(self.workspace.numel()), None if side_adam is None else C.byref(side_adam), _C._stream()))
# ... 188 lines not shown
```

### sk_gs_amd/fused_step.py

```python
import ctypes as C
import os
from typing import Optional

import torch
from torch import Tensor

from sk_gs_amd import _C
from sk_gs_amd.model import SkinnedGaussians
from sk_gs_amd.renderer.gaussian_render import GaussianRasterizationSettings


def _p(t: Optional[Tensor]) -> C.c_void_p:
    return C.c_void_p(None if t is None else t.data_ptr())


class FusedViewStep:

    def __init__(self, model: SkinnedGaussians, W: int, H: int, capacity: int, lambda_dssim: float = 0.2,
                 background: Optional[Tensor] = None, grad_scale: float = 1.0, densify_stats: bool = False,
                 spw_logit_grad: Optional[Tensor] = None, tables_zeroed_by_optimizer: bool = False,
                 tile_bucket: int = 0, sh_factors: Optional[Tensor] = None, fused_deform_net: bool = True,
                 view_table=None):
        assert not model.static, 'FusedViewStep covers the skinned stage (M >= 1)'
        self.model, self.W, self.H = model, int(W), int(H)
        self.lambda_l1, self.lambda_ssim = 1.0 - lambda_dssim, lambda_dssim
        lib = self.lib = _C.load_library()
        dev = model._xyz.device
        if not model._xyz.is_cuda:
            raise _C.SkgsError('FusedViewStep needs the model on a HIP device; sk_gs_amd has no CPU path')
        cap = getattr(model, 'capacity', None)
        P, M, K = (cap.P_cap if cap is not None else model.P), model.M, model.K
        self.P, self.M, self.K = P, M, K
        self._live = cap.live if cap is not None else None
        assert cap is None or (sh_factors is None and spw_logit_grad is None), \
            'row capacity: one-rank step (the factor / compact-logit exchanges are sized by the live count)'
        lib.skgs_fused_lbs_max_bones.restype = C.c_int
        self.max_fused_bones = int(lib.skgs_fused_lbs_max_bones())
        self.wide = M > self.max_fused_bones or K > 8
        self.deform_in_preprocess = os.environ.get('SKGS_SEPARATE_DEFORM', '0') != '1'
        self.deform_backward_in_preprocess = os.environ.get('SKGS_SEPARATE_DEFORM_BACKWARD', '0') != '1'
        self._rows_backward_done = False
        self.lbs_method = getattr(model, 'lbs_method', 'W')
        assert self.lbs_method == 'W' or (cap is None and spw_logit_grad is None), \
            'the distance-based LBS weightings run without a row capacity / compact-logit exchange'
        if K > 16 or K > M:
            raise _C.SkgsError(f'FusedViewStep: K = {K} neighbours: the KNN kernels keep at most 16 (and K <= M = {M})')
        self.sh_factors = sh_factors
        assert sh_factors is None or (sh_factors.is_cuda and sh_factors.dtype == torch.float32 and
                                      sh_factors.is_contiguous() and sh_factors.numel() == P * 6)
        f32 = dict(dtype=torch.float32, device=dev)
        u8 = dict(dtype=torch.uint8, device=dev)
        self.background = None if background is None else background.to(**f32).contiguous()
        self.grad_scale = None if grad_scale == 1.0 else torch.full((1,), float(grad_scale), **f32)
        self._grad_scale_value = float(grad_scale)
        from sk_gs_amd.capacity import cap_store
        for p in model.parameters():
            if p.grad is None:
                store = cap_store(p)
                if store is None:
                    p.grad = torch.zeros_like(p)
                else:
                    p.grad, p._grad_slot = torch.zeros_like(store)[:p.shape[0]], store.numel()
            assert cap_store(p) is None or getattr(p, '_grad_slot', 0) >= cap_store(p).numel(), \
                'row capacity: build the gradient buffers AFTER model.enable_capacity()'
            assert p.is_contiguous() and p.grad.is_contiguous() and p.dtype == torch.float32
        self.bone_T, self.chain_A = torch.empty((M, 7), **f32), torch.empty((M, 7), **f32)
        self.indices = torch.empty((P, K), dtype=torch.int64, device=dev)
        self.weights = torch.empty((P, K), **f32)
        self.means, self.scales = torch.empty((P, 3), **f32), torch.empty((P, 3), **f32)
        self.rotations, self.opacity = torch.empty((P, 4), **f32), torch.empty((P, 1), **f32)
        self.image, self.out_opacity = torch.empty((3, H, W), **f32), torch.empty((H, W), **f32)
        self.radii = torch.empty((P,), dtype=torch.int32, device=dev)
        self.geom = torch.empty((lib.skgs_geom_buffer_bytes(C.c_int32(P)),), **u8)
        self.geom[:256].zero_()
        self.img = torch.empty((lib.skgs_img_buffer_bytes(C.c_int32(W), C.c_int32(H)),), **u8)
        self.tile_bucket = int(tile_bucket)
        if self.tile_bucket > 0:
            capacity = ((W + 15) // 16) * ((H + 15) // 16) * self.tile_bucket
        self.binning = torch.empty((lib.skgs_binning_buffer_bytes(C.c_int64(int(capacity))),), **u8)
        self.loss3 = torch.zeros(3, **f32)
        self.loss_ws = torch.empty((lib.skgs_image_loss_workspace_bytes(C.c_int32(3), C.c_int32(H), C.c_int32(W)),), **u8)
        self.dL_dimage = torch.empty((3, H, W), **f32)
        self.grad_means2D = torch.empty((P, 3), **f32)
        self.g_colors, self.g_cov3D = torch.empty((P, 3), **f32), torch.empty((P, 6), **f32)
        self.g_means, self.g_scales = torch.empty((P, 3), **f32), torch.empty((P, 3), **f32)
        self.g_rotations, self.g_opacity = torch.empty((P, 4), **f32), torch.empty((P, 1), **f32)
        self.g_weights = torch.empty((P, K), **f32)
        self.g_bone_T = torch.empty((M, 7), **f32)
        if self.lbs_method != 'W':
            self.nn_dist = torch.empty((P, K), **f32)
            lib.skgs_knn_dist_weights_workspace_bytes.restype = C.c_size_t
            self.dist_ws = torch.empty((max(int(lib.skgs_knn_dist_weights_workspace_bytes(C.c_int32(P), C.c_int32(M), C.c_int32(3))),
                                            16),), **u8)
        self.deform_ws = torch.empty((lib.skgs_lbs_deform_backward_workspace_bytes(C.c_int32(P), C.c_int32(M)),), **u8)
        self.bwd_ws = torch.zeros((lib.skgs_backward_workspace_bytes(C.c_int32(P)),), **u8)
        self.tables_zeroed_by_optimizer = bool(tables_zeroed_by_optimizer)
        self.side_optimizer = None
        self.keep_raster_grads = bool(os.environ.get('SKGS_KEEP_RASTER_GRADS'))
        self.skeleton_ahead = False
        self.defer_input_grad = False
        self._arm_tail = None
        self.spw_logit_grad = spw_logit_grad
        assert spw_logit_grad is None or (spw_logit_grad.numel() == P * K and spw_logit_grad.is_contiguous())
        self.densify_stats = bool(densify_stats)
        self._acc_store, self._den_store = torch.zeros((P, 1), **f32), torch.zeros((P, 1), **f32)
        self._rad_store = torch.zeros((P,), **f32)
        self.deform_net = model.sk_deform_net
        self._mlp_fused = None
        if self.deform_net is not None:
            from sk_gs_amd.deform_net import DeformMLPRunner, FusedDeformMLP, fused_supported
            net = self.deform_net.dynamic_net
            self._mlp_fused = FusedDeformMLP(self.deform_net, M) if (fused_deform_net and fused_supported(self.deform_net, M)) else None
            self._mlp = DeformMLPRunner(self.deform_net)
            if self._mlp_fused is None:
                self._x0 = torch.empty((M, net.in_channels), **f32)
                self._acts = torch.empty((net.num_layers, M, net.dim_hidden), **f32)
                self._g_act = torch.empty((2, M, net.dim_hidden), **f32)
            self._sk_r_raw, self._d_rot, self._d_scale = (torch.empty((M, 4), **f32), torch.empty((M, 4), **f32),
                                                          torch.empty((M, 3), **f32))
            self._g_heads = [torch.empty((M, 4), **f32), torch.empty((M, 4), **f32), torch.empty((M, 3), **f32)]
            self._g_x0 = torch.empty((M, net.in_channels), **f32) if getattr(model, 'learn_joints', False) else None
        self.view_table = view_table
        if view_table is not None:
            assert self.deform_net is not None, 'the view slot drives the deform network\'s time input: tables mode keeps one graph per view'
# ... 155 lines not shown
                                         _p(m.sp_W), _p(self.indices), _p(self.weights), st))
            chk(lib.skgs_lbs_deform_forward(C.byref(d), _p(self.means), _p(self.scales), _p(self.rotations), _p(self.opacity),
                                            None, None, None, st))
            a = self._raster_inputs(rs)
            chk(lib.skgs_rasterize_forward(C.byref(a), C.byref(self._bufs), _p(self.radii), _p(self.image),
                                           _p(self.out_opacity), None, None, st))
            return a, d
        if self.deform_in_preprocess and K <= 8:
            j = _C._KnnDeformJob()
            j.M, j.K = M, K
            j.points, j.joints, j.sp_W, j.bone_T = d.points, m.joints.data_ptr(), m.sp_W.data_ptr(), d.bone_T
            j.bone_drot, j.bone_dscale, j.xyz, j.log_scale = d.bone_drot, d.bone_dscale, d.xyz, d.log_scale
            j.rot, j.opacity_logit, j.out_idx, j.out_weights = d.rot, d.opacity_logit, self.indices.data_ptr(), self.weights.data_ptr()
            j.means, j.scales = self.means.data_ptr(), self.scales.data_ptr()
            j.rotations, j.opacity = self.rotations.data_ptr(), self.opacity.data_ptr()
            a = self._raster_inputs(rs)
            a.deform_job = C.pointer(j)
            chk(lib.skgs_rasterize_forward(C.byref(a), C.byref(self._bufs), _p(self.radii), _p(self.image),
                                           _p(self.out_opacity), None, None, st))
            a.deform_job = None
            return a, d
        chk(lib.skgs_knn_lbs_deform_forward(
            C.c_int32(P), C.c_int32(M), C.c_int32(K), C.c_void_p(d.points), _p(m.joints), _p(m.sp_W), C.c_void_p(d.bone_T),
            C.c_void_p(d.bone_drot), C.c_void_p(d.bone_dscale), C.c_void_p(d.xyz), C.c_void_p(d.log_scale), C.c_void_p(d.rot),
            C.c_void_p(d.opacity_logit), _p(self.indices), _p(self.weights), _p(self.means), _p(self.scales),
            _p(self.rotations), _p(self.opacity), _p(self._live), st))
        a = self._raster_inputs(rs)
        chk(lib.skgs_rasterize_forward(C.byref(a), C.byref(self._bufs), _p(self.radii), _p(self.image),
                                       _p(self.out_opacity), None, None, st))
        return a, d

    @torch.no_grad()
    def forward_backward(self, rs: Optional[GaussianRasterizationSettings] = None, time_id: Optional[int] = None,
                         target: Optional[Tensor] = None):
        self.backward_raster(rs, time_id, target)
        self.backward_skinning(time_id)

    @torch.no_grad()
    def backward_raster(self, rs: Optional[GaussianRasterizationSettings] = None, time_id: Optional[int] = None,
                        target: Optional[Tensor] = None):
        lib, m, st, chk = self.lib, self.model, _C._stream(), _C._check
        P, M, K, W, H = self.P, self.M, self.K, self.W, self.H
        if rs is None:
            from sk_gs_amd import view_slot as vsl
            assert target is None and self.view_table.targets is not None
            target, gt_index = self.view_table.targets, C.c_void_p(self.view_table.ptr(vsl.W_TARGET))
        else:
            gt_index = None
        assert target.is_cuda and target.dtype == torch.float32 and target.is_contiguous()
        self._zero_table_grads()
        a, d = self.forward(rs, time_id)
        chk(lib.skgs_image_loss_forward(C.c_int32(3), C.c_int32(H), C.c_int32(W), _p(self.image), _p(target), gt_index,
                                        C.c_float(self.lambda_l1), C.c_float(self.lambda_ssim), None,
                                        _p(self.loss_ws), C.c_size_t(self.loss_ws.numel()), st))
        self._loss_backward_and_raster(a, d, target, gt_index, time_id, self.grad_scale)

    def _loss_backward_and_raster(self, a, d, target, gt_index, time_id, grad_loss: Tensor):
        lib, m, st, chk = self.lib, self.model, _C._stream(), _C._check
        W, H = self.W, self.H
        chk(lib.skgs_image_loss_backward(C.c_int32(3), C.c_int32(H), C.c_int32(W), _p(self.image), _p(target), gt_index,
                                         C.c_float(self.lambda_l1), C.c_float(self.lambda_ssim), _p(grad_loss),
                                         _p(self.loss_ws), C.c_size_t(self.loss_ws.numel()), _p(self.dL_dimage),
                                         _p(self.loss3), st))
        self._raster_backward(a, d, time_id)

    def _raster_backward(self, a, d, time_id):
        lib, m, st, chk = self.lib, self.model, _C._stream(), _C._check
        g = _C._RasterGrads()
        g.dL_dout_color = self.dL_dimage.data_ptr()
        g.dL_dmeans2D, g.dL_dcolors, g.dL_dopacity = (self.grad_means2D.data_ptr(), self.g_colors.data_ptr(),
                                                      self.g_opacity.data_ptr())
        g.dL_dmeans3D, g.dL_dcov3D = self.g_means.data_ptr(), self.g_cov3D.data_ptr()
        if self.sh_factors is None:
            g.dL_dsh, g.dL_dsh_rest = m._features_dc.grad.data_ptr(), m._features_rest.grad.data_ptr()
        else:
            g.dL_dsh_factors = self.sh_factors.data_ptr()
        g.dL_dscales, g.dL_drotations = self.g_scales.data_ptr(), self.g_rotations.data_ptr()
        g.workspace, g.workspace_bytes = self.bwd_ws.data_ptr(), self.bwd_ws.numel()
        g.workspace_is_zero = 1
        if self.densify_stats:
            g.stat_xyz_gradient_accum, g.stat_denom = self._acc_store.data_ptr(), self._den_store.data_ptr()
            g.stat_max_radii2D, g.stat_grad_multiplier = self._rad_store.data_ptr(), 1.0 / self._grad_scale_value
        self._rows_backward_done = False
        job = self._attach_backward_job(g, d, time_id)
        if job is not None and self._rows_backward_done and not self.keep_raster_grads:
            g.dL_dcolors = g.dL_dopacity = g.dL_dmeans3D = g.dL_dcov3D = g.dL_dscales = g.dL_drotations = None
        chk(lib.skgs_rasterize_backward(C.byref(a), C.byref(self._bufs), _p(self.radii), _p(self.out_opacity),
                                        C.byref(g), st))

    def _attach_backward_job(self, g, d, time_id):
        m = self.model
        if not (self.deform_backward_in_preprocess and self.lbs_method == 'W' and not self.wide and self.M <= 64 and self.K <= 8):
            return None
        if self.deform_net is None:
            g_drot, g_dscale = m.sk_d_rot.grad[time_id], m.sk_d_scale.grad[time_id]
        else:
            _, g_drot, g_dscale = self._g_heads
        dense = self.spw_logit_grad is None
        j = _C._DeformBackwardJob()
        j.in_ = C.pointer(d)
        j.g_bone_T, j.g_bone_drot, j.g_bone_dscale = self.g_bone_T.data_ptr(), g_drot.data_ptr(), g_dscale.data_ptr()
        j.g_xyz, j.g_log_scale = m._xyz.grad.data_ptr(), m._scaling.grad.data_ptr()
        j.g_rot, j.g_opacity_logit = m._rotation.grad.data_ptr(), m._opacity.grad.data_ptr()
        j.g_sp_W = m.sp_W.grad.data_ptr() if dense else None
        j.g_logits = None if dense else self.spw_logit_grad.data_ptr()
        j.workspace, j.workspace_bytes = self.deform_ws.data_ptr(), self.deform_ws.numel()
        g.deform_backward_job = C.cast(C.pointer(j), C.c_void_p)
        self._rows_backward_done = True
        return j

    @torch.no_grad()
    def forward_loss(self, rs: Optional[GaussianRasterizationSettings] = None, time_id: Optional[int] = None,
                     target: Optional[Tensor] = None) -> Tensor:
        lib, st, chk = self.lib, _C._stream(), _C._check
        if rs is None:
            from sk_gs_amd import view_slot as vsl
            assert target is None and self.view_table.targets is not None
            target, gt_index = self.view_table.targets, C.c_void_p(self.view_table.ptr(vsl.W_TARGET))
        else:
            gt_index = None
        assert target.is_cuda and target.dtype == torch.float32 and target.is_contiguous()
        self._zero_table_grads()
        a, d = self.forward(rs, time_id)
        chk(lib.skgs_image_loss_forward(C.c_int32(3), C.c_int32(self.H), C.c_int32(self.W), _p(self.image), _p(target), gt_index,
                                        C.c_float(self.lambda_l1), C.c_float(self.lambda_ssim), _p(self.loss3),
                                        _p(self.loss_ws), C.c_size_t(self.loss_ws.numel()), st))
        self._pending = (a, d, target, gt_index, time_id)
        return self.loss3[0]

    @torch.no_grad()
    def backward_pending(self, grad_loss: Optional[Tensor] = None):
        a, d, target, gt_index, time_id = self._pending
        self._pending = None
        seed = self.grad_scale
        if grad_loss is not None:
            seed = grad_loss.detach().reshape(1).to(torch.float32)
            if self.grad_scale is not None:
                seed = seed * self.grad_scale
            seed = seed.contiguous()
        self._loss_backward_and_raster(a, d, target, gt_index, time_id, seed)
        self.backward_skinning(time_id)

    def loss(self, rs: Optional[GaussianRasterizationSettings] = None, time_id: Optional[int] = None,
             target: Optional[Tensor] = None) -> Tensor:
        params = [p for p in self.model.parameters() if p.requires_grad]
        return _FusedViewLoss.apply(self, rs, time_id, target, *params)

    @torch.no_grad()
    def sh_grads_from_factors(self, all_factors: Tensor, sh_degree: int):
        m = self.model
        n_views = all_factors.numel() // (self.P * 6)
        assert all_factors.is_contiguous() and all_factors.numel() == n_views * self.P * 6
        _C._check(self.lib.skgs_sh_grad_from_factors(
            C.c_int32(self.P), C.c_int32(n_views), C.c_int32(sh_degree), C.c_int32(1 + m._features_rest.shape[1]),
            _p(all_factors), _p(m._features_dc.grad), _p(m._features_rest.grad), _C._stream()))

    @torch.no_grad()
    def backward_skinning(self, time_id: Optional[int] = None, part: Optional[str] = None):
        lib, m, st, chk = self.lib, self.model, _C._stream(), _C._check
        assert part in (None, 'rows', 'skeleton')
        if part is not None:
            assert self.lbs_method == 'W' and not self.wide and self._mlp_fused is not None, \
                'backward_skinning(part=...): the one-launch skinning backward and the fused skeleton stage'
        if part == 'skeleton':
            self._time_id = time_id
            self._deform_net_backward()
            return
        t = self._topo
        P, M, K = self.P, self.M, self.K
        d = self._deform_inputs(time_id)
        self._time_id = time_id
        gT, g_gT, fidx = self._frame(time_id)
        if self.deform_net is None:
            sk_r_raw, g_raw = m.sk_r[time_id], m.sk_r.grad[time_id]
            g_drot, g_dscale = m.sk_d_rot.grad[time_id], m.sk_d_scale.grad[time_id]
        else:
            sk_r_raw, (g_raw, g_drot, g_dscale) = self._sk_r_raw, self._g_heads
        if self.lbs_method != 'W':
            chk(lib.skgs_lbs_deform_backward(
                C.byref(d), _p(self.g_means), _p(self.g_scales), _p(self.g_rotations), _p(self.g_opacity),
                _p(self.g_weights), _p(self.g_bone_T), _p(g_drot), _p(g_dscale),
                _p(m._xyz.grad), _p(m._scaling.grad), _p(m._rotation.grad), _p(m._opacity.grad), _p(self.deform_ws),
                C.c_size_t(self.deform_ws.numel()), st))
        elif self._rows_backward_done:
            if part == 'rows':
                return
        elif not self.wide:
            dense = self.spw_logit_grad is None
            chk(lib.skgs_lbs_deform_backward_logits(
                C.byref(d), _p(self.g_means), _p(self.g_scales), _p(self.g_rotations), _p(self.g_opacity),
                None, _p(self.g_bone_T), _p(g_drot), _p(g_dscale),
# ... 24 lines not shown
                _p(m._sp_weight), C.c_float(m.lbs_temperature), C.c_int32(1), C.c_int32(1), _p(self.weights), _p(self.indices),
                _p(self.nn_dist), _p(self.g_weights), None, _p(m.joints.grad) if learn else None,
                None if m._sp_radius is None else _p(m._sp_radius.grad), None if m._sp_weight is None else _p(m._sp_weight.grad),
                _p(self.dist_ws), C.c_size_t(self.dist_ws.numel()), st))

    def _lbs_logits_backward(self):
        lib, m, st, chk = self.lib, self.model, _C._stream(), _C._check
        P, M, K = self.P, self.M, self.K
        if self.spw_logit_grad is None:
            chk(lib.skgs_lbs_weights_backward(C.c_int32(P), C.c_int32(M), C.c_int32(K), _p(self.weights),
                                              _p(self.indices), _p(self.g_weights), _p(m.sp_W.grad), st))
        else:
            chk(lib.skgs_lbs_weights_backward_compact(C.c_int32(P), C.c_int32(K), _p(self.weights), _p(self.g_weights),
                                                      _p(self.spw_logit_grad), st))

    def _time_tensor(self, time_id: Optional[int]) -> Tensor:
        if time_id is not None:
            return self.model.frame_times[time_id]
        from sk_gs_amd import view_slot as vsl
        return self.view_table.slot[vsl.W_TIME:vsl.W_TIME + 1]

    def input_grad_job(self):
        if self._g_x0 is None or self._mlp_fused is None:
            return None
        mlp = self.deform_net
        return (self.M, mlp.p_in, mlp.p_degree, self._g_x0, self._mlp_fused.x0, self._mlp_fused.x0.shape[1],
                self.model.joints.grad, True)

    def _bones_desc(self, time_id: Optional[int]):
        from sk_gs_amd.deform_net import BoneChainDesc
        m, t = self.model, self._topo
        gT, g_gT, fidx = self._frame(time_id)
        b = BoneChainDesc()
        b.M, b.root, b.num_levels = self.M, t['root'], t['num_levels']
        b.parents, b.level_nodes, b.level_start = t['parents'].data_ptr(), t['level_nodes'].data_ptr(), t['level_start'].data_ptr()
        b.joints, b.global_T = m.joints.data_ptr(), gT
        b.frame_index = fidx.value if isinstance(fidx, C.c_void_p) else fidx
        b.bone_T, b.chain_A = self.bone_T.data_ptr(), self.chain_A.data_ptr()
        b.sk_r_raw, b.g_bone_T = self._sk_r_raw.data_ptr(), self.g_bone_T.data_ptr()
        b.g_joints = m.joints.grad.data_ptr() if (getattr(m, 'learn_joints', False) and m.joints.grad is not None) else None
        b.g_global_T = g_gT
        cache = getattr(m, 'sk_cache', None)
        if cache is not None and cache.is_cuda and cache.shape[1] == self.M:
            b.sk_cache = cache.data_ptr() if time_id is None else cache[time_id].data_ptr()
        else:
            b.sk_cache = None
        return b

    def _joint_rotations(self, time_id: Optional[int]) -> Tensor:
        m = self.model
        if self.deform_net is None:
            return m.sk_r[time_id]
        tt = self._time_tensor(time_id)
        if self._mlp_fused is not None:
            if not self.skeleton_ahead:
                self.skeleton_forward(time_id)
            return self._sk_r_raw
        from sk_gs_amd.deform_net import _lin_fwd
        net, run = self.deform_net.dynamic_net, self._mlp
        run.encode(m.joints, tt, self._x0)
        run.forward_hidden(self._x0, self._acts)
        M, H, IN = self.M, net.dim_hidden, net.in_channels
        in1, in2 = net.layer_dims()[-1]
        o = 0
        for buf, oc in zip((self._sk_r_raw, self._d_rot, self._d_scale), net.out_channels):
            _lin_fwd(self.lib, M, in1, in2, oc, self._acts[-1].data_ptr(), H, self._x0.data_ptr() if in2 else None, IN,
                     net.last_weight[o:].data_ptr(), net.last_bias[o:].data_ptr(), buf.data_ptr(), oc, 0)
            o += oc
        return self._sk_r_raw

    def skeleton_forward(self, time_id: Optional[int] = None, side_adam=None):
        assert self._mlp_fused is not None
        self._mlp_fused.forward(self.model.joints, self._time_tensor(time_id),
                                head_out=(self._sk_r_raw, self._d_rot, self._d_scale), bones=self._bones_desc(time_id),
                                side_adam=side_adam)

    def _deform_net_backward(self):
        if self._mlp_fused is not None:
            net = self.deform_net.dynamic_net
            grads = [g for l in net.net for g in (l.weight.grad, l.bias.grad)] + [net.last_weight.grad, net.last_bias.grad]
            side = None
            if self.side_optimizer is not None:
                side = self.side_optimizer[0].side_range(*self.side_optimizer[1:])
            self._mlp_fused.backward(self.model.joints, self._time_tensor(self._time_id), self._g_heads, grads, self._g_x0,
                                     side_adam=side, bones=self._bones_desc(self._time_id))
            if self._g_x0 is not None and not self.defer_input_grad:
                self._mlp.input_grad(self._g_x0, self._mlp_fused.x0, self.model.joints.grad, accumulate=True)
            return
        from sk_gs_amd.deform_net import _lin_bwd
        net, run = self.deform_net.dynamic_net, self._mlp
        M, H, IN = self.M, net.dim_hidden, net.in_channels
        in1, in2 = net.layer_dims()[-1]
        o = 0
        for j, (g_head, oc) in enumerate(zip(self._g_heads, net.out_channels)):
            _lin_bwd(self.lib, M, in1, in2, oc, self._acts[-1].data_ptr(), H, self._x0.data_ptr() if in2 else None, IN,
                     net.last_weight[o:].data_ptr(), None, g_head.data_ptr(), oc, 0, net.last_weight.grad[o:].data_ptr(),
                     net.last_bias.grad[o:].data_ptr(), self._g_act[0].data_ptr(), H, None, IN, 1 if j > 0 else 0)
            o += oc
        grads = [g for l in net.net for g in (l.weight.grad, l.bias.grad)]
        run.backward_hidden(self._x0, self._acts, grads, self._g_act, self._g_x0)
        if self._g_x0 is not None:
            run.input_grad(self._g_x0, self._x0, self.model.joints.grad, accumulate=True)

    @torch.no_grad()
    def scatter_spw_grad(self):
        _C._check(self.lib.skgs_lbs_logits_scatter(C.c_int32(self.P), C.c_int32(self.M), C.c_int32(self.K),
                                                   _p(self.indices), _p(self.spw_logit_grad), _p(self.model.sp_W.grad),
                                                   _C._stream()))

    @torch.no_grad()
    def add_densification_stats(self):
        _C._check(self.lib.skgs_densify_stats(C.c_int32(self.P), _p(self.radii), _p(self.grad_means2D),
                                             C.c_float(1.0 / self._grad_scale_value), _p(self._acc_store),
                                             _p(self._den_store), _p(self._rad_store), _C._stream()))

    @torch.no_grad()
    def grow_capacity(self, factor: float = 2.0):
        lib = self.lib
        if self.tile_bucket > 0:
            self.tile_bucket = ((int(self.tile_bucket * factor) + 63) // 64) * 64
            capacity = ((self.W + 15) // 16) * ((self.H + 15) // 16) * self.tile_bucket
        else:
            capacity = int(int(lib.skgs_binning_capacity(C.c_size_t(self.binning.numel()))) * factor) + 1024
        self.binning = torch.empty((lib.skgs_binning_buffer_bytes(C.c_int64(int(capacity))),), dtype=torch.uint8,
                                   device=self.binning.device)
        self.geom[:256].zero_()
        self._bufs = _C._buffers(self.geom, self.binning, self.img)
        return capacity

    def status(self) -> dict:
        st = _C.read_status(self.geom)
        if self.deform_net is not None and self._mlp_fused is not None:
            m = self._mlp_fused.status()
            st['mlp_failed'] = m['failed']
            st['mlp_one_xcd'] = dict(forward=[m['one_xcd_forward'], m['forward']], backward=[m['one_xcd_backward'], m['backward']],
                                     xcds=[m['xcds_forward'], m['xcds_backward']])
        return st


class _FusedViewLoss(torch.autograd.Function):

    @staticmethod
    def forward(ctx, step, rs, time_id, target, *params):
        ctx.step = step
        return step.forward_loss(rs, time_id, target).clone()

    @staticmethod
    @torch.autograd.function.once_differentiable
    def backward(ctx, g):
        ctx.step.backward_pending(g)
        arm = getattr(ctx.step, '_arm_tail', None)
        if arm is not None:
            ctx.step._arm_tail = None
            arm[0]._pending_tail = arm[1]
        return (None,) * (4 + len([p for p in ctx.step.model.parameters() if p.requires_grad]))
```

Baseline: 3066.

## Fold deform-backward bone finalize into fused skeleton MLP backward kernel

The per-bone reduction of deform-backward partials moves out of its own kernel launch and into side workgroups of the fused skeleton MLP backward kernel. Those workgroups publish their results through a flag and record handshake that the net workgroups poll before reading the bone gradients. The Adam side work is rebalanced so the finalize workgroups take fewer chunks. This removes one kernel launch and its serialization, at the cost of cross-workgroup spin-waiting, which could stall if the finalize workgroups are not co-resident.

```diff
diff --git a/include/skgs.h b/include/skgs.h
--- a/include/skgs.h
+++ b/include/skgs.h
@@ -196,7 +196,9 @@
   float* g_logits;
   void* workspace;
   size_t workspace_bytes;
+  int32_t defer_finalize;
 } skgs_deform_backward_job;
+int skgs_deform_backward_job_finalize(const skgs_deform_backward_job* job, skgs_stream_t stream);
 int skgs_lbs_deform_forward(const skgs_deform_inputs* in, float* means, float* scales, float* rotations,
     float* opacity, float* d_xyz, float* d_rot, float* d_scale, skgs_stream_t stream);
 size_t skgs_lbs_deform_backward_workspace_bytes(int32_t P, int32_t M);
@@ -380,6 +382,7 @@
   float* g_joints;
   float* g_global_T;
   float* sk_cache;
+  const struct skgs_deform_backward_job* finalize_job;
 } skgs_bone_chain_desc;
 int skgs_skeleton_forward(const skgs_mlp_desc* d, const skgs_bone_chain_desc* bones, const float* points, const float* t,
     float* x0, float* acts, void* workspace, size_t workspace_bytes, const skgs_adam_range* side ,
diff --git a/sk_gs_amd/_C.py b/sk_gs_amd/_C.py
--- a/sk_gs_amd/_C.py
+++ b/sk_gs_amd/_C.py
@@ -84,7 +84,7 @@
 class _DeformBackwardJob(C.Structure):
     _fields_ = [('in_', C.POINTER(_DeformInputs))] + [(n, C.c_void_p) for n in (
         'g_bone_T', 'g_bone_drot', 'g_bone_dscale', 'g_xyz', 'g_log_scale', 'g_rot', 'g_opacity_logit', 'g_sp_W', 'g_logits',
-        'workspace')] + [('workspace_bytes', C.c_size_t)]
+        'workspace')] + [('workspace_bytes', C.c_size_t), ('defer_finalize', C.c_int32)]
 
 
 class _SpSkinningJob(C.Structure):
diff --git a/sk_gs_amd/csrc/api.hip b/sk_gs_amd/csrc/api.hip
--- a/sk_gs_amd/csrc/api.hip
+++ b/sk_gs_amd/csrc/api.hip
@@ -292,7 +292,15 @@
   if (launch_preprocess_backward(*in, g, radii, *gr, s)) return 1;
   if (sj) return sp_fix_job(*sj) ? 0 : launch_sp_skinning_rest(*sj, s);
   if (oj) return launch_offset_scale_grad_finalize(in->P, *oj, s);
-  return dj ? launch_deform_backward_finalize(*dj->in, dj->workspace, dj->g_bone_T, dj->g_bone_drot, dj->g_bone_dscale, s) : 0;
+  if (!dj || dj->defer_finalize) return 0;
+  return launch_deform_backward_finalize(*dj->in, dj->workspace, dj->g_bone_T, dj->g_bone_drot, dj->g_bone_dscale, s);
+}
+
+int skgs_deform_backward_job_finalize(const skgs_deform_backward_job* dj, skgs_stream_t stream) {
+  SKGS_REQUIRE(dj && dj->in && dj->workspace && dj->g_bone_T && dj->g_bone_drot && dj->g_bone_dscale, "deform_backward_job_finalize: NULL argument");
+  SKGS_REQUIRE(dj->in->M >= 1 && dj->in->M <= deform_backward_job_max_bones() && dj->in->bone_T, "deform_backward_job_finalize: bad bones");
+  SKGS_REQUIRE(dj->workspace_bytes >= deform_backward_workspace_bytes(dj->in->P, dj->in->M), "deform_backward_job_finalize: workspace too small");
+  return launch_deform_backward_finalize(*dj->in, dj->workspace, dj->g_bone_T, dj->g_bone_drot, dj->g_bone_dscale, (hipStream_t) stream);
 }
 
 int skgs_rasterize_extra_forward(int32_t W, int32_t H, int32_t P, int32_t E, const float* extra,
diff --git a/sk_gs_amd/csrc/deform.hip b/sk_gs_amd/csrc/deform.hip
--- a/sk_gs_amd/csrc/deform.hip
+++ b/sk_gs_amd/csrc/deform.hip
@@ -2,6 +2,7 @@
 
 #include "skgs_common.h"
 #include "deform_lane.h"
+#include "deform_finalize.h"
 
 #pragma clang fp contract(off)
 
@@ -261,50 +262,9 @@
 __global__ void __launch_bounds__(256) deform_backward_finalize_kernel(int M, int nblk, const float* __restrict__ partials,
     const float* __restrict__ bone_T, float* __restrict__ g_bone_T, float* __restrict__ g_bone_drot,
     float* __restrict__ g_bone_dscale) {
-  __shared__ float s_red[256][MOM_F + 1];
-  const int b = blockIdx.x, t = threadIdx.x;
-  float acc[MOM_F];
-#pragma unroll
-  for (int c = 0; c < MOM_F; ++c) acc[c] = 0.f;
-  for (int w = t; w < nblk; w += 256) {
-    const float* row = partials + ((size_t) w * M + b) * MOM_F;
-#pragma unroll
-    for (int c = 0; c < MOM_F; ++c) acc[c] += row[c];
-  }
-#pragma unroll
-  for (int c = 0; c < MOM_F; ++c) s_red[t][c] = acc[c];
-  __syncthreads();
-  for (int d = 128; d > 0; d >>= 1) {
-    if (t < d) {
-#pragma unroll
-      for (int c = 0; c < MOM_F; ++c) s_red[t][c] += s_red[t + d][c];
-    }
-    __syncthreads();
-  }
-  if (t != 0) return;
-  float m[MOM_F];
-  for (int i = 0; i < MOM_F; ++i) m[i] = s_red[0][i];
-  const float q0 = bone_T[7 * b + 3], q1 = bone_T[7 * b + 4], q2 = bone_T[7 * b + 5], q3 = bone_T[7 * b + 6];
-  const float qn = sqrtf(q0 * q0 + q1 * q1 + q2 * q2 + q3 * q3);
-  const float vq[4] = {q0 / qn, q1 / qn, q2 / qn, q3 / qn};
-  const float* S = m + 3;
-#define SM(a, c) S[3 * (a) + (c)]
-  const float pxg[3] = {SM(2, 1) - SM(1, 2), SM(0, 2) - SM(2, 0), SM(1, 0) - SM(0, 1)};
-  const float tr     = SM(0, 0) + SM(1, 1) + SM(2, 2);
-  float gqh[4];
-  for (int i = 0; i < 3; ++i) {
-    const float vdp_g = vq[0] * SM(i, 0) + vq[1] * SM(i, 1) + vq[2] * SM(i, 2);
-    const float gdv_p = vq[0] * SM(0, i) + vq[1] * SM(1, i) + vq[2] * SM(2, i);
-    gqh[i] = 2.0f * vq[3] * pxg[i] + 2.0f * (vdp_g + gdv_p - 2.0f * tr * vq[i]);
-  }
-  gqh[3] = 2.0f * ((vq[1] * SM(0, 2) - vq[2] * SM(0, 1)) + (vq[2] * SM(1, 0) - vq[0] * SM(1, 2)) +
-                   (vq[0] * SM(2, 1) - vq[1] * SM(2, 0)));
-#undef SM
-  const float dotq = vq[0] * gqh[0] + vq[1] * gqh[1] + vq[2] * gqh[2] + vq[3] * gqh[3];
-  g_bone_T[7 * b] = m[0], g_bone_T[7 * b + 1] = m[1], g_bone_T[7 * b + 2] = m[2];
-  for (int i = 0; i < 4; ++i) g_bone_T[7 * b + 3 + i] = (gqh[i] - vq[i] * dotq) / qn;
-  for (int i = 0; i < 4; ++i) g_bone_drot[4 * b + i] = m[12 + i];
-  for (int i = 0; i < 3; ++i) g_bone_dscale[3 * b + i] = m[16 + i];
+  static_assert(FIN_MOM_F == MOM_F && FIN_THREADS == 256, "deform_finalize.h: the moments' row / the reduction's thread map");
+  __shared__ float s_red[FIN_THREADS][FIN_MOM_F + 1];
+  deform_finalize_bone(s_red, blockIdx.x, M, nblk, partials, bone_T, g_bone_T, g_bone_drot, g_bone_dscale, nullptr);
 }
 
 constexpr int KNN_MAXK = 16;
@@ -786,12 +746,13 @@
 
 int launch_deform_backward_finalize(const skgs_deform_inputs& in, void* workspace, float* g_bone_T, float* g_bone_drot,
     float* g_bone_dscale, hipStream_t s) {
-  const int nblk = (in.P + DEFORM_BWD_THREADS - 1) / DEFORM_BWD_THREADS;
+  const int nblk = deform_backward_job_blocks(in.P);
   hipLaunchKernelGGL(deform_backward_finalize_kernel, dim3(in.M), dim3(256), 0, s, in.M, nblk, reinterpret_cast<float*>(workspace),
       in.bone_T, g_bone_T, g_bone_drot, g_bone_dscale);
   SKGS_CHECK_HIP(hipGetLastError());
   return 0;
 }
+int deform_backward_job_blocks(int P) { return (P + DEFORM_BWD_THREADS - 1) / DEFORM_BWD_THREADS; }
 int deform_backward_job_max_bones() { return MOM_MAX_BONES; }
 int deform_backward_job_max_k() { return PREF_K; }
 
diff --git a/sk_gs_amd/csrc/deform_finalize.h b/sk_gs_amd/csrc/deform_finalize.h
--- /dev/null
+++ b/sk_gs_amd/csrc/deform_finalize.h
@@ -0,0 +1,71 @@
+#pragma once
+#include "skgs_common.h"
+
+namespace skgs {
+
+constexpr int FIN_MOM_F   = 19;
+constexpr int FIN_THREADS = 256;
+constexpr int FIN_LDS_FLOATS = FIN_THREADS * (FIN_MOM_F + 1);
+
+__device__ __forceinline__ bool deform_finalize_bone(float (*s_red)[FIN_MOM_F + 1], int b, int M, int nblk,
+    const float* __restrict__ partials, const float* __restrict__ bone_T, float* __restrict__ g_bone_T,
+    float* __restrict__ g_bone_drot, float* __restrict__ g_bone_dscale, float* rec) {
+#pragma clang fp contract(off)
+  constexpr int MOM_F = FIN_MOM_F;
+  const int t = threadIdx.x;
+  if (t < FIN_THREADS) {
+    float acc[MOM_F];
+#pragma unroll
+    for (int c = 0; c < MOM_F; ++c) acc[c] = 0.f;
+    for (int w = t; w < nblk; w += FIN_THREADS) {
+      const float* row = partials + ((size_t) w * M + b) * MOM_F;
+#pragma unroll
+      for (int c = 0; c < MOM_F; ++c) acc[c] += row[c];
+    }
+#pragma unroll
+    for (int c = 0; c < MOM_F; ++c) s_red[t][c] = acc[c];
+  }
+  __syncthreads();
+  for (int d = FIN_THREADS / 2; d > 0; d >>= 1) {
+    if (t < d) {
+#pragma unroll
+      for (int c = 0; c < MOM_F; ++c) s_red[t][c] += s_red[t + d][c];
+    }
+    __syncthreads();
+  }
+  if (t != 0) return false;
+  float m[MOM_F];
+  for (int i = 0; i < MOM_F; ++i) m[i] = s_red[0][i];
+  const float q0 = bone_T[7 * b + 3], q1 = bone_T[7 * b + 4], q2 = bone_T[7 * b + 5], q3 = bone_T[7 * b + 6];
+  const float qn = sqrtf(q0 * q0 + q1 * q1 + q2 * q2 + q3 * q3);
+  const float vq[4] = {q0 / qn, q1 / qn, q2 / qn, q3 / qn};
+  const float* S = m + 3;
+#define SKGS_FIN_SM(a, c) S[3 * (a) + (c)]
+  const float pxg[3] = {SKGS_FIN_SM(2, 1) - SKGS_FIN_SM(1, 2), SKGS_FIN_SM(0, 2) - SKGS_FIN_SM(2, 0),
+      SKGS_FIN_SM(1, 0) - SKGS_FIN_SM(0, 1)};
+  const float tr     = SKGS_FIN_SM(0, 0) + SKGS_FIN_SM(1, 1) + SKGS_FIN_SM(2, 2);
+  float gqh[4];
+  for (int i = 0; i < 3; ++i) {
+    const float vdp_g = vq[0] * SKGS_FIN_SM(i, 0) + vq[1] * SKGS_FIN_SM(i, 1) + vq[2] * SKGS_FIN_SM(i, 2);
+    const float gdv_p = vq[0] * SKGS_FIN_SM(0, i) + vq[1] * SKGS_FIN_SM(1, i) + vq[2] * SKGS_FIN_SM(2, i);
+    gqh[i] = 2.0f * vq[3] * pxg[i] + 2.0f * (vdp_g + gdv_p - 2.0f * tr * vq[i]);
+  }
+  gqh[3] = 2.0f * ((vq[1] * SKGS_FIN_SM(0, 2) - vq[2] * SKGS_FIN_SM(0, 1)) + (vq[2] * SKGS_FIN_SM(1, 0) - vq[0] * SKGS_FIN_SM(1, 2)) +
+                   (vq[0] * SKGS_FIN_SM(2, 1) - vq[1] * SKGS_FIN_SM(2, 0)));
+#undef SKGS_FIN_SM
+  const float dotq = vq[0] * gqh[0] + vq[1] * gqh[1] + vq[2] * gqh[2] + vq[3] * gqh[3];
+  float o[14];
+  o[0] = m[0], o[1] = m[1], o[2] = m[2];
+  for (int i = 0; i < 4; ++i) o[3 + i] = (gqh[i] - vq[i] * dotq) / qn;
+  for (int i = 0; i < 4; ++i) o[7 + i] = m[12 + i];
+  for (int i = 0; i < 3; ++i) o[11 + i] = m[16 + i];
+  for (int i = 0; i < 7; ++i) g_bone_T[7 * b + i] = o[i];
+  for (int i = 0; i < 4; ++i) g_bone_drot[4 * b + i] = o[7 + i];
+  for (int i = 0; i < 3; ++i) g_bone_dscale[3 * b + i] = o[11 + i];
+  if (rec) {
+    for (int i = 0; i < 14; ++i) rec[i] = o[i];
+  }
+  return true;
+}
+
+}
diff --git a/sk_gs_amd/csrc/mlp_fused.hip b/sk_gs_amd/csrc/mlp_fused.hip
--- a/sk_gs_amd/csrc/mlp_fused.hip
+++ b/sk_gs_amd/csrc/mlp_fused.hip
@@ -3,6 +3,7 @@
 
 #include "adam_update.h"
 #include "bone_chain.inl"
+#include "deform_finalize.h"
 #include "skgs_common.h"
 
 namespace skgs {
@@ -58,7 +59,16 @@
   int xcd_mode;
   int side_delay;
   unsigned* census;
+  const float* fin_partials;
+  int fin_nblk, fin_M;
+  const float* fin_bone_T;
+  float *fin_g_T, *fin_g_drot, *fin_g_dscale;
+  float* fin_rec;
+  unsigned* fin_flag;
 };
+constexpr int FIN_MAX_BONES = 48;
+constexpr int FIN_BYTES = FIN_MAX_BONES * (64 + 4) + 64;
+static_assert(FIN_BYTES % 256 == 0, "the workspace's last section keeps the 256-byte grain");
 
 __device__ __forceinline__ FusedLayer get_layer(const FusedArgs& a, int l) {
   return FusedLayer{a.W[l], a.bias[l], a.gW[l], a.gb[l], l ? H : 0, ((a.xmask >> l) & 1u) ? a.IN : 0,
@@ -83,8 +93,8 @@
 }
 
 
-__device__ __forceinline__ void stamp(const FusedArgs& a, const unsigned* s_misc, int& si, unsigned long long t_entry = 0) {
-  if (s_misc[2] && blockIdx.x == 0 && threadIdx.x == 0 && si < 20) {
+__device__ __forceinline__ void stamp(const FusedArgs& a, const unsigned* s_misc, int& si, unsigned long long t_entry = 0, bool first = blockIdx.x == 0) {
+  if (s_misc[2] && first && threadIdx.x == 0 && si < 20) {
     if (t_entry) a.hdr[16 + 46] = (unsigned) t_entry;
     a.hdr[16 + 2 * si]     = (unsigned) __builtin_amdgcn_s_memrealtime();
     a.hdr[16 + 2 * si + 1] = (unsigned) __builtin_amdgcn_s_memtime();
@@ -295,7 +305,10 @@
 };
 __device__ __forceinline__ Role role_of(const FusedArgs& a) {
   const int b = (int) blockIdx.x, n_side = (int) gridDim.x - G_NET;
-  if (!a.xcd_mode) return Role{b < G_NET, b, b - G_NET, n_side};
+  if (!a.xcd_mode) {
+    const int r = a.fin_partials ? a.fin_M : 0;
+    return Role{b >= r && b < r + G_NET, b - r, b < r ? b : b - G_NET, n_side};
+  }
   const bool low = b < 8 * G_NET;
   const bool net = low && (b & 7) == 0;
   const int before = low ? (b >> 3) + 1 : G_NET;
@@ -309,7 +322,15 @@
   const AdamTensorLanes desc = adam_load_descriptors(a.adam_tensors, a.adam_n, lane);
   const int64_t first0 = lane < a.adam_n ? a.adam_tensors[lane].chunk0 : INT64_MAX;
   const int64_t n_chunks = a.adam_c1 - a.adam_c0;
-  const int64_t begin = a.adam_c0 + n_chunks * wg / n_side, end = a.adam_c0 + n_chunks * (wg + 1) / n_side;
+  int64_t begin = a.adam_c0 + n_chunks * wg / n_side, end = a.adam_c0 + n_chunks * (wg + 1) / n_side;
+  if (a.fin_partials) {
+    const int64_t M = a.fin_M, wr = n_chunks > n_side ? n_chunks - n_side : 0, wo = n_chunks;
+    const int64_t total = wr * min(M, (int64_t) n_side) + wo * max((int64_t) n_side - M, (int64_t) 0);
+    if (total > 0) {
+      auto cum = [&](int64_t w) { return w < M ? wr * w : wr * M + wo * (w - M); };
+      begin = a.adam_c0 + n_chunks * cum(wg) / total, end = a.adam_c0 + n_chunks * cum(wg + 1) / total;
+    }
+  }
 #if SKGS_SIDE_CHUNKS == 1
   for (int64_t chunk = begin + half; chunk < end; chunk += 2) {
     const int ti0 = adam_owner(a.adam_tensors, a.adam_n, first0, lane, chunk);
@@ -329,6 +350,48 @@
       adam_update_chunk(T0, (chunk - T0.chunk0) * ADAM_CHUNK, t256, k);
     }
   }
+}
+
+__device__ __forceinline__ void bone_finalize_job(const FusedArgs& a, int b, float* smem) {
+  unsigned cnt = 0;
+  if (threadIdx.x == 0) cnt = __hip_atomic_load(reinterpret_cast<const gu32*>((unsigned long long) a.hdr) + 3, __ATOMIC_RELAXED, __HIP_MEMORY_SCOPE_AGENT);
+  float rec[16];
+  const bool lead = deform_finalize_bone(reinterpret_cast<float(*)[FIN_MOM_F + 1]>(smem), b, a.fin_M, a.fin_nblk, a.fin_partials,
+      a.fin_bone_T, a.fin_g_T, a.fin_g_drot, a.fin_g_dscale, rec);
+  if (lead) {
+    rec[14] = rec[15] = 0.f;
+    float* r = a.fin_rec + 16 * b;
+#pragma unroll
+    for (int q = 0; q < 4; ++q) store16_sc1(r + 4 * q, make_float4(rec[4 * q], rec[4 * q + 1], rec[4 * q + 2], rec[4 * q + 3]));
+    asm volatile("s_waitcnt vmcnt(0)" ::: "memory");
+    __hip_atomic_store(reinterpret_cast<gu32*>((unsigned long long) a.fin_flag) + b, cnt + 1u, __ATOMIC_RELAXED, __HIP_MEMORY_SCOPE_AGENT);
+  }
+  __syncthreads();
+}
+__device__ __forceinline__ bool bone_finalize_wait(const FusedArgs& a, unsigned epoch, float* s_rec) {
+  const int M = a.fin_M, i = min((int) threadIdx.x, M - 1);
+  const gu32* fp = reinterpret_cast<const gu32*>((unsigned long long) a.fin_flag) + i;
+  const unsigned long long t0 = __builtin_amdgcn_s_memrealtime();
+  unsigned polls = 0;
+  for (;;) {
+    const unsigned f = __hip_atomic_load(fp, __ATOMIC_RELAXED, __HIP_MEMORY_SCOPE_AGENT);
+    if (__builtin_amdgcn_ballot_w64(f != epoch) == 0) break;
+    if (++polls > 100000u && __builtin_amdgcn_s_memrealtime() - t0 > 5000000ull) return false;
+  }
+  const float* rp = a.fin_rec + 16 * i;
+  f4 r0, r1, r2, r3;
+  asm volatile(
+      "global_load_dwordx4 %0, %4, off sc1\n\tglobal_load_dwordx4 %1, %4, off offset:16 sc1\n\t"
+      "global_load_dwordx4 %2, %4, off offset:32 sc1\n\tglobal_load_dwordx4 %3, %4, off offset:48 sc1\n\ts_waitcnt vmcnt(0)"
+      : "=&v"(r0), "=&v"(r1), "=&v"(r2), "=&v"(r3)
+      : "v"(rp)
+      : "memory");
+  if ((int) threadIdx.x < M) {
+    float4* d = reinterpret_cast<float4*>(s_rec + 16 * i);
+    d[0] = make_float4(r0.x, r0.y, r0.z, r0.w), d[1] = make_float4(r1.x, r1.y, r1.z, r1.w);
+    d[2] = make_float4(r2.x, r2.y, r2.z, r2.w), d[3] = make_float4(r3.x, r3.y, r3.z, r3.w);
+  }
+  return true;
 }
 
 template <int PASSES>
@@ -531,12 +594,14 @@
   extern __shared__ __attribute__((aligned(16))) float smem[];
   const Role role = role_of(a);
   if (!role.net) {
+    if (a.fin_partials && role.wg < a.fin_M) bone_finalize_job(a, role.wg, smem);
     adam_side_job(a, role.wg, role.n_side);
     return;
   }
   const int tid = threadIdx.x, wave = tid >> 6;
   const int G = G_NET, g = role.g, col0 = g * NC;
   const int B = a.B, nL = a.n_layers, IN = a.IN, nX = nL - 1;
+  const bool fold = a.fin_partials != nullptr;
   const bool want_gx = a.g_x0 != nullptr && col0 < IN;
   float* s_gz   = smem;
   float* s_x0   = s_gz;
@@ -567,14 +632,14 @@
     stamps_on = __hip_atomic_load(h + 2, __ATOMIC_RELAXED, __HIP_MEMORY_SCOPE_AGENT);
   }
   auto pstamp = [&](int slot, unsigned long long t) {
-    if (stamps_on && blockIdx.x == 0 && tid == 0) {
+    if (stamps_on && g == 0 && tid == 0) {
       a.hdr[16 + 2 * slot]     = (unsigned) (t ? t : __builtin_amdgcn_s_memrealtime());
       a.hdr[16 + 2 * slot + 1] = (unsigned) __builtin_amdgcn_s_memtime();
     }
   };
   chain::Prefetch cpf;
   cpf.valid = false;
-  if (a.has_chain) cpf = chain::prefetch(a.chain, true, true);
+  if (a.has_chain) cpf = chain::prefetch(a.chain, true, true, !fold);
   pstamp(18, t_entry);
   const int mrow = tid >> 1, mpart = tid & 1;
   const bool mlive = tid < Bp * 2 && mrow < B;
@@ -627,25 +692,18 @@
     for (int q = 0; q < GZQ; ++q) {
       const int b = (tid >> 6) + q * (NT / 64);
       hgz[q] = 0.f;
-      if (b < B && c < oL_pf && !(a.has_chain && c < 4))
+      if (b < B && c < oL_pf && !(a.has_chain && c < 4) && !fold)
         hgz[q] = *head_elem_sel(a, a.head_gout, a.g_out, b, c, oL_pf);
     }
     const int bo = tid / NC, co = col0 + tid % NC;
-    if (tid < Bp * NC && bo < B && co < oL_pf && !(a.has_chain && co < 4))
+    if (tid < Bp * NC && bo < B && co < oL_pf && !(a.has_chain && co < 4) && !fold)
       hown = *head_elem_sel(a, a.head_gout, a.g_out, bo, co, oL_pf);
   }
   if (stamps_on_all(a)) {
     asm volatile("s_waitcnt vmcnt(0)" ::: "memory");
     pstamp(22, 0);
   }
-  if (a.has_chain) {
-    chain::backward_stage(s_part, a.chain, cpf);
-    pstamp(19, 0);
-    chain::backward_levels(s_part, a.chain, s_graw, g == 0);
-    __syncthreads();
-  }
-  pstamp(21, 0);
-  {
+  auto stage_slabs = [&]() {
     int toff = 0, xoff = t_total;
 #pragma unroll
     for (int l = 0; l < KL; ++l) {
@@ -668,8 +726,40 @@
         if (want_gx && get_layer(a, l).in_x) xoff += NC * OP;
       }
     }
-  }
-  pstamp(20, 0);
+    pstamp(20, 0);
+  };
+  stage_slabs();
+  unsigned fin_failed = 0;
+  if (fold) {
+    float* s_rec = s_gz;
+    if (wave == 0) {
+      const unsigned epoch = (unsigned) __builtin_amdgcn_readfirstlane((int) cnt) + 1u;
+      if (!bone_finalize_wait(a, epoch, s_rec) || !cpf.valid) fin_failed = 1;
+    }
+    __syncthreads();
+    pstamp(17, 0);
+    if (tid < a.chain.M) {
+#pragma unroll
+      for (int e = 0; e < 7; ++e) cpf.g[e] = s_rec[16 * tid + e];
+    }
+    {
+      const int c = tid & 63;
+#pragma unroll
+      for (int q = 0; q < GZQ; ++q) {
+        const int b = (tid >> 6) + q * (NT / 64);
+        if (b < B && c >= 4 && c < oL_pf) hgz[q] = s_rec[16 * b + c + 3];
+      }
+      const int bo = tid / NC, co = col0 + tid % NC;
+      if (tid < Bp * NC && bo < B && co >= 4 && co < oL_pf) hown = s_rec[16 * bo + co + 3];
+    }
+  }
+  if (a.has_chain) {
+    chain::backward_stage(s_part, a.chain, cpf);
+    pstamp(19, 0);
+    chain::backward_levels(s_part, a.chain, s_graw, g == 0);
+    __syncthreads();
+  }
+  pstamp(21, 0);
   {
     const int oL = oL_pf;
     const int c = tid & 63;
@@ -687,7 +777,7 @@
       s_own[(nL - 1) * Bp * NC + tid] = (b < B && cc < oL) ? v : 0.f;
     }
   }
-  if (tid == 0) s_misc[0] = cnt, s_misc[1] = 0, s_misc[2] = stamps_on;
+  if (tid == 0) s_misc[0] = cnt, s_misc[1] = fin_failed, s_misc[2] = stamps_on;
   __syncthreads();
   const unsigned count = s_misc[0];
   const size_t img_floats = (size_t) nX * G * Bp * NC;
@@ -698,7 +788,7 @@
   bool plain = false;
   unsigned census_word = 0;
   int si = 12;
-  stamp(a, s_misc, si);
+  stamp(a, s_misc, si, 0, g == 0);
 
   const int kcol = (H / NW) * wave + 4 * lm.rgl + lm.j;
   f4 gw = {0.f, 0.f, 0.f, 0.f};
@@ -773,7 +863,7 @@
     for (int i = 0; i < 4; ++i)
       if (i < gw_rows) gw_dst[(size_t) i * gw_ld] = gw[i];
   }
-  stamp(a, s_misc, si);
+  stamp(a, s_misc, si, 0, g == 0);
   if (want_gx && !s_misc[1]) {
     mfma_dot<ROUNDS, H / NW / 4>(accx, s_gz, HP, rowc, s_wT + t_total, H + 4, lm.colw, (H / NW) * wave);
     write_partials<ROUNDS>(s_part, accx, lm, wave, Bp, 4 * PASSES);
@@ -788,7 +878,7 @@
       if (c + 3 < IN) d[3] = y.w;
     }
   }
-  stamp(a, s_misc, si);
+  stamp(a, s_misc, si, 0, g == 0);
   if (!s_misc[1]) {
     __syncthreads();
     if (a.x0) {
@@ -845,7 +935,7 @@
       }
     }
   }
-  stamp(a, s_misc, si);
+  stamp(a, s_misc, si, 0, g == 0);
   if (g == 0 && tid == 0) {
     gu32* h = reinterpret_cast<gu32*>((unsigned long long) a.hdr);
     if (s_misc[1]) __hip_atomic_fetch_add(h + 1, 1u, __ATOMIC_RELAXED, __HIP_MEMORY_SCOPE_AGENT);
@@ -958,14 +1048,15 @@
   if (a.adam_tensors && a.adam_c1 > a.adam_c0)
     side = (int) std::max<long long>(1, std::min<long long>((a.adam_c1 - a.adam_c0 + 1) / 2, num_cus() - p.G));
   FusedArgs b = a;
-  int grid = p.G + side;
+  const int fin = a.fin_partials ? a.fin_M : 0;
+  int grid = p.G + std::max(side, fin);
   {
     static const int delay = [] { const char* e = getenv("SKGS_SIDE_DELAY"); return e ? std::max(0, atoi(e)) : 0; }();
     b.side_delay = delay;
   }
   b.xcd_mode = xcd_mode_wanted();
   if (b.xcd_mode) {
-    if (num_cus() != 256 || p.G != G_NET || (side > 0 && grid < 8 * p.G - 7)) b.xcd_mode = 0;
+    if (num_cus() != 256 || p.G != G_NET || (side > 0 && p.G + side < 8 * p.G - 7)) b.xcd_mode = 0;
     else grid = std::max(grid, 8 * p.G - 7);
   }
   hipLaunchKernelGGL(k, dim3(grid), dim3(NT), lds, s, b);
@@ -999,7 +1090,7 @@
 size_t skgs_deform_mlp_workspace_bytes(const skgs_mlp_desc* d) {
   Plan p;
   if (make_plan(d, &p)) return 0;
-  return HDR_BYTES + 2 * p.exch_bytes;
+  return HDR_BYTES + 2 * p.exch_bytes + FIN_BYTES;
 }
 
 int skgs_deform_mlp_workspace_init(void* workspace, size_t workspace_bytes, skgs_stream_t stream) {
@@ -1113,6 +1204,22 @@
     a.chain.g_global_T = bones->g_global_T, a.chain.g_sk_r_raw = const_cast<float*>(d->head_gout[0]);
   }
   if (fill_side(side, &a)) return 1;
+  if (const skgs_deform_backward_job* fj = bones ? bones->finalize_job : nullptr) {
+    SKGS_REQUIRE(fj->in && fj->workspace && fj->in->bone_T, "skeleton_backward: finalize_job: NULL argument");
+    SKGS_REQUIRE(fj->in->M == bones->M && fj->in->M <= FIN_MAX_BONES && fj->in->M <= deform_backward_job_max_bones(),
+        "skeleton_backward: finalize_job: %d bones (the chain has %d)", fj->in->M, bones->M);
+    SKGS_REQUIRE(d->n_heads == 3 && d->head_dim[1] == 4 && d->head_dim[2] == 3, "skeleton_backward: finalize_job needs the heads 4 | 4 | 3");
+    SKGS_REQUIRE(fj->g_bone_T == bones->g_bone_T && fj->g_bone_drot == d->head_gout[1] && fj->g_bone_dscale == d->head_gout[2],
+        "skeleton_backward: finalize_job must write the gradients this launch reads (g_bone_T, head_gout[1], head_gout[2])");
+    SKGS_REQUIRE(fj->workspace_bytes >= deform_backward_workspace_bytes(fj->in->P, fj->in->M), "skeleton_backward: finalize_job: workspace too small");
+    SKGS_REQUIRE(workspace_bytes >= HDR_BYTES + 2 * p.exch_bytes + FIN_BYTES, "skeleton_backward: finalize_job: workspace too small (skgs_deform_mlp_workspace_bytes)");
+    SKGS_REQUIRE(bones->num_levels + 1 <= NT, "skeleton_backward: finalize_job: %d tree levels", bones->num_levels);
+    a.fin_partials = reinterpret_cast<const float*>(fj->workspace);
+    a.fin_nblk = deform_backward_job_blocks(fj->in->P), a.fin_M = fj->in->M, a.fin_bone_T = fj->in->bone_T;
+    a.fin_g_T = fj->g_bone_T, a.fin_g_drot = fj->g_bone_drot, a.fin_g_dscale = fj->g_bone_dscale;
+    a.fin_rec  = reinterpret_cast<float*>(reinterpret_cast<char*>(workspace) + HDR_BYTES + 2 * p.exch_bytes);
+    a.fin_flag = reinterpret_cast<unsigned*>(a.fin_rec + FIN_MAX_BONES * 16);
+  }
   a.hdr  = reinterpret_cast<unsigned*>(workspace);
   a.exch = reinterpret_cast<float*>(reinterpret_cast<char*>(workspace) + HDR_BYTES + p.exch_bytes);
   a.census = reinterpret_cast<unsigned*>(reinterpret_cast<char*>(a.exch) + p.exch_bytes - CENSUS_BYTES);
@@ -1125,6 +1232,7 @@
   a.lds_floats = (int) fl;
   const size_t lds = fl * 4;
   SKGS_REQUIRE(lds <= 160 * 1024, "deform_mlp_backward: %zu bytes of LDS needed", lds);
+  SKGS_REQUIRE(!a.fin_partials || fl >= (size_t) FIN_LDS_FLOATS, "skeleton_backward: finalize_job: the launch's LDS does not hold the reduction");
   SKGS_MLP_DISPATCH(fused_mlp_backward_kernel, K_SKELETON_BWD)
 }
 }
diff --git a/sk_gs_amd/csrc/skgs_common.h b/sk_gs_amd/csrc/skgs_common.h
--- a/sk_gs_amd/csrc/skgs_common.h
+++ b/sk_gs_amd/csrc/skgs_common.h
@@ -393,6 +393,7 @@
 inline bool sp_fix_job(const skgs_sp_skinning_job& j) { return j.image_to_deform_off != 0 && j.g_weights_extra == nullptr; }
 int launch_deform_backward_finalize(const skgs_deform_inputs& in, void* workspace, float* g_bone_T, float* g_bone_drot,
     float* g_bone_dscale, hipStream_t s);
+int deform_backward_job_blocks(int P);
 int deform_backward_job_max_bones();
 int deform_backward_job_max_k();
 int launch_knn_deform_forward(int P, int M, int K, const float* points, const float* joints, const float* sp_W,
diff --git a/sk_gs_amd/deform_net.py b/sk_gs_amd/deform_net.py
--- a/sk_gs_amd/deform_net.py
+++ b/sk_gs_amd/deform_net.py
@@ -198,7 +198,7 @@
                 ('parents', C.c_void_p), ('level_nodes', C.c_void_p), ('level_start', C.c_void_p),
                 ('joints', C.c_void_p), ('global_T', C.c_void_p), ('frame_index', C.c_void_p),
                 ('bone_T', C.c_void_p), ('chain_A', C.c_void_p), ('sk_r_raw', C.c_void_p), ('g_bone_T', C.c_void_p),
-                ('g_joints', C.c_void_p), ('g_global_T', C.c_void_p), ('sk_cache', C.c_void_p)]
+                ('g_joints', C.c_void_p), ('g_global_T', C.c_void_p), ('sk_cache', C.c_void_p), ('finalize_job', C.c_void_p)]
 
 
 def fused_supported(mlp: 'DeformMLP', B: int) -> bool:
diff --git a/sk_gs_amd/fused_step.py b/sk_gs_amd/fused_step.py
--- a/sk_gs_amd/fused_step.py
+++ b/sk_gs_amd/fused_step.py
@@ -40,6 +40,8 @@
         self.deform_in_preprocess = os.environ.get('SKGS_SEPARATE_DEFORM', '0') != '1'
         self.deform_backward_in_preprocess = os.environ.get('SKGS_SEPARATE_DEFORM_BACKWARD', '0') != '1'
         self._rows_backward_done = False
+        self.fold_bone_finalize = os.environ.get('SKGS_BONE_FINALIZE_LAUNCH', '1') == '0'
+        self._deferred_finalize = None
         self.lbs_method = getattr(model, 'lbs_method', 'W')
         assert self.lbs_method == 'W' or (cap is None and spw_logit_grad is None), \
             'the distance-based LBS weightings run without a row capacity / compact-logit exchange'
@@ -361,6 +363,7 @@
             g.stat_xyz_gradient_accum, g.stat_denom = self._acc_store.data_ptr(), self._den_store.data_ptr()
             g.stat_max_radii2D, g.stat_grad_multiplier = self._rad_store.data_ptr(), 1.0 / self._grad_scale_value
         self._rows_backward_done = False
+        self._deferred_finalize = None
         job = self._attach_backward_job(g, d, time_id)
         if job is not None and self._rows_backward_done and not self.keep_raster_grads:
             g.dL_dcolors = g.dL_dopacity = g.dL_dmeans3D = g.dL_dcov3D = g.dL_dscales = g.dL_drotations = None
@@ -386,6 +389,9 @@
         j.workspace, j.workspace_bytes = self.deform_ws.data_ptr(), self.deform_ws.numel()
         g.deform_backward_job = C.cast(C.pointer(j), C.c_void_p)
         self._rows_backward_done = True
+        if self.fold_bone_finalize and self.deform_net is not None and self._mlp_fused is not None:
+            j.defer_finalize = 1
+            self._deferred_finalize = (j, d)
         return j
 
     @torch.no_grad()
@@ -576,8 +582,11 @@
             side = None
             if self.side_optimizer is not None:
                 side = self.side_optimizer[0].side_range(*self.side_optimizer[1:])
+            bones = self._bones_desc(self._time_id)
+            if self._deferred_finalize is not None:
+                bones.finalize_job = C.addressof(self._deferred_finalize[0])
             self._mlp_fused.backward(self.model.joints, self._time_tensor(self._time_id), self._g_heads, grads, self._g_x0,
-                                     side_adam=side, bones=self._bones_desc(self._time_id))
+                                     side_adam=side, bones=bones)
             if self._g_x0 is not None and not self.defer_input_grad:
                 self._mlp.input_grad(self._g_x0, self._mlp_fused.x0, self.model.joints.grad, accumulate=True)
             return
```

Result: no change. 3065 (median of 2 runs) (-0.0%).
